# rosielab/emojivoice

Hardware: AMD Instinct MI355X
Metric: audio_seconds_per_second (higher is better)
Workload: dtype f32 (deep layers: operand = two block-scaled fp16 pieces, product = 3 fp16 products on the fp16 MFMA, f32 accumulate); 1 GPU; config2: batch 64 x 516-frame (5.99 s) utterances per GPU, 10 Euler steps + HiFi-GAN V1, 22.05 kHz; global_batch=64, frames=516, ode_steps=10, parallelism=dp1, collective=none, batch_pipeline=cfm(i+1) || hifigan(i) on two streams, 2 pipeline(s) in flight

## Files before the change

emojivoice_amd/_lib.py:

```python
from __future__ import annotations

import ctypes as C
import os
import subprocess
from typing import Dict, Optional

import numpy as np
import torch

_HERE = os.path.dirname(os.path.abspath(__file__))
LIB_PATH = os.environ.get("EV_LIB_PATH") or os.path.join(_HERE, "lib", "libemojivoice_hip.so")
CSRC = os.path.join(_HERE, "csrc")

EXPORTS = [
    "ev_abi_version", "ev_create", "ev_destroy", "ev_last_error", "ev_load_estimator", "ev_load_vocoder", "ev_load_vocoder_cfg", "ev_load_text_encoder", "ev_text_encoder",
    "ev_text_encoder_status", "ev_stft_magnitude", "ev_denoise", "ev_align", "ev_dbg_conv_bench",
    "ev_workspace_bytes", "ev_cfm_decode", "ev_estimator", "ev_hifigan", "ev_profile_enable", "ev_profile_read", "ev_profile_read_split", "ev_dbg_last_cfg", "ev_set_arithmetic", "ev_get_arithmetic",
    "ev_op_conv1d", "ev_op_groupnorm_mish", "ev_op_layernorm", "ev_op_split_pieces", "ev_op_attention", "ev_op_ln_mlp", "ev_set_mrf_streams_max",
    "ev_cfm_decode2", "ev_reserve", "ev_alloc_count", "ev_dbg_sk_stats", "ev_op_attn_out", "ev_dbg_set_amax", "ev_dbg_set_attn_h16", "ev_dbg_set_chain", "ev_dbg_sk_taken",
    "ev_load_mel_basis", "ev_mel_spectrogram",
    "ev_maximum_path", "ev_log_prior", "ev_mas_align",
    "ev_estimator_rows", "ev_cfm_loss",
    "ev_load_resampler", "ev_resample", "ev_mel_stats",
]


class EvLibraryError(RuntimeError):
    pass


class ev_tensor_index(C.Structure):
    _fields_ = [("name", C.c_char_p), ("offset", C.c_uint64), ("ndim", C.c_int32), ("shape", C.c_int64 * 4)]


class ev_model_dims(C.Structure):
    _fields_ = [("n_feats", C.c_int32), ("spk_emb_dim", C.c_int32), ("channels", C.c_int32), ("heads", C.c_int32),
                ("head_dim", C.c_int32)]


class ev_vocoder_config(C.Structure):
    _fields_ = [("resblock", C.c_int32), ("num_levels", C.c_int32), ("upsample_rates", C.c_int32 * 4), ("upsample_kernel_sizes", C.c_int32 * 4),
                ("resblock_kernel_sizes", C.c_int32 * 3), ("resblock_dilations", (C.c_int32 * 3) * 3)]


def vocoder_config(h) -> ev_vocoder_config:
    c = ev_vocoder_config()
    c.resblock = 1 if str(h["resblock"]) == "1" else 2
    c.num_levels = len(h["upsample_rates"])
    for i, (u, k) in enumerate(zip(h["upsample_rates"], h["upsample_kernel_sizes"])):
        c.upsample_rates[i], c.upsample_kernel_sizes[i] = int(u), int(k)
    for j, (k, ds) in enumerate(zip(h["resblock_kernel_sizes"], h["resblock_dilation_sizes"])):
        c.resblock_kernel_sizes[j] = int(k)
        for m, d in enumerate(ds):
            c.resblock_dilations[j][m] = int(d)
    return c


def vocoder_frame_bytes(h) -> int:
    rates, rb1 = list(h["upsample_rates"]), str(h["resblock"]) == "1"
    widest, prod, p0 = 0, 1, 4
    for i, u in enumerate(rates):
        prod *= u
        widest = max(widest, prod * (h["upsample_initial_channel"] // 2 ** (i + 1)) * 4)
        halo = 3 if i == len(rates) - 1 else 0
        for k, ds in zip(h["resblock_kernel_sizes"], h["resblock_dilation_sizes"]):
            for d in (ds if rb1 else ds[:2]):
                halo = max(halo, (k - 1) * d // 2)
        p0 = max(p0, -(-halo // prod))
    return widest, p0


def build_library(force: bool = False, verbose: bool = False) -> str:
    src = os.path.join(CSRC, "ev_engine.hip")
    deps = [src, os.path.join(CSRC, "ev_kernels.h"), os.path.join(os.path.dirname(_HERE), "include", "emojivoice.h")]
    if not force and os.path.exists(LIB_PATH) and all(os.path.getmtime(LIB_PATH) >= os.path.getmtime(d) for d in deps):
        return LIB_PATH
    os.makedirs(os.path.dirname(LIB_PATH), exist_ok=True)
    hipcc = os.environ.get("HIPCC", "/opt/rocm/bin/hipcc")
    cmd = [hipcc, "--offload-arch=gfx950", "-O3", "-std=c++17", "-fPIC", "-shared", "-Wno-unused-value", src, "-o", LIB_PATH]
    if verbose:
        print(" ".join(cmd))
    subprocess.run(cmd, check=True)
    return LIB_PATH


_lib: Optional[C.CDLL] = None


def load_library() -> C.CDLL:
    global _lib
    if _lib is not None:
        return _lib
    if not os.path.exists(LIB_PATH):
        raise EvLibraryError(
            f"{LIB_PATH} is missing: build it with `python -c 'import __graft_entry__ as g; g.build()'` "
            "(there is no CPU fallback for the EmojiVoice hot path)")
    lib = C.CDLL(LIB_PATH)
    vp, i32, f32, u64 = C.c_void_p, C.c_int, C.c_float, C.c_size_t
    lib.ev_abi_version.restype = C.c_int
    lib.ev_create.argtypes = [C.POINTER(vp), i32, C.POINTER(ev_model_dims)]
    lib.ev_destroy.argtypes = [vp]
    lib.ev_destroy.restype = None
    lib.ev_last_error.argtypes = [vp]
    lib.ev_last_error.restype = C.c_char_p
    for f in (lib.ev_load_estimator, lib.ev_load_vocoder, lib.ev_load_text_encoder):
        f.argtypes = [vp, vp, C.POINTER(ev_tensor_index), u64]
    lib.ev_load_vocoder_cfg.argtypes = [vp, vp, C.POINTER(ev_tensor_index), u64, C.POINTER(ev_vocoder_config)]
    lib.ev_set_mrf_streams_max.argtypes = [vp, i32]
    lib.ev_set_mrf_streams_max.restype = i32
    lib.ev_workspace_bytes.argtypes = [vp, i32, i32, i32]
    lib.ev_workspace_bytes.restype = u64
    lib.ev_cfm_decode.argtypes = [vp, vp, vp, vp, vp, i32, i32, i32, f32, f32, vp, vp]
    lib.ev_cfm_decode2.argtypes = [vp, vp, vp, vp, vp, i32, i32, i32, vp, f32, f32, vp, vp]
    lib.ev_reserve.argtypes = [vp, i32, i32, i32, i32, vp]
    lib.ev_alloc_count.argtypes = [vp]
    lib.ev_alloc_count.restype = C.c_int64
    lib.ev_dbg_sk_stats.argtypes = [vp, C.POINTER(C.c_uint32)]
    lib.ev_estimator.argtypes = [vp, vp, vp, vp, vp, f32, i32, i32, vp, vp]
    lib.ev_estimator_rows.argtypes = [vp, vp, vp, vp, vp, vp, i32, i32, vp, vp]
    lib.ev_cfm_loss.argtypes = [vp, vp, vp, vp, vp, vp, vp, i32, i32, f32, vp, vp, vp]
    lib.ev_hifigan.argtypes = [vp, vp, i32, i32, vp, vp]
    lib.ev_text_encoder.argtypes = [vp, vp, vp, vp, i32, i32, vp, vp, vp]
    lib.ev_text_encoder_status.argtypes = [vp, vp]
    lib.ev_dbg_conv_bench.argtypes = [vp, i32, i32, i32, i32, i32, i32, i32, i32, i32, i32, C.POINTER(C.c_float)]
    lib.ev_stft_magnitude.argtypes = [vp, vp, i32, i32, vp, vp]
    lib.ev_align.argtypes = [vp, vp, vp, vp, vp, i32, i32, i32, vp, vp, vp]
    lib.ev_denoise.argtypes = [vp, vp, i32, i32, vp, f32, vp, vp]
    lib.ev_load_mel_basis.argtypes = [vp, vp, i32, i32]
    lib.ev_mel_spectrogram.argtypes = [vp, vp, i32, i32, f32, f32, vp, vp]
    lib.ev_load_resampler.argtypes = [vp, vp, i32, i32, i32]
    lib.ev_resample.argtypes = [vp, vp, vp, i32, i32, vp, i32, vp]
    lib.ev_mel_stats.argtypes = [vp, vp, vp, i32, i32, i32, vp, vp]
    lib.ev_maximum_path.argtypes = [vp, vp, vp, vp, i32, i32, i32, vp, vp, vp]
    lib.ev_log_prior.argtypes = [vp, vp, vp, i32, i32, i32, vp, vp]
    lib.ev_mas_align.argtypes = [vp, vp, vp, vp, vp, i32, i32, i32, vp, vp, vp, vp, vp]
    lib.ev_profile_enable.argtypes = [vp, i32]
    lib.ev_profile_read.argtypes = [vp, C.POINTER(C.c_double), C.POINTER(C.c_double), C.POINTER(C.c_int64), i32]
    lib.ev_profile_read_split.argtypes = [vp, C.POINTER(C.c_double), C.POINTER(C.c_double), C.POINTER(C.c_int64)]
    lib.ev_dbg_last_cfg.argtypes = [vp]
    lib.ev_set_arithmetic.argtypes = [vp, i32]
    lib.ev_get_arithmetic.argtypes = [vp]
    lib.ev_dbg_set_amax.argtypes = [vp, i32]
    lib.ev_dbg_set_attn_h16.argtypes = [vp, i32]
    lib.ev_dbg_set_chain.argtypes = [vp, i32]
    lib.ev_dbg_sk_taken.argtypes = [vp]
    lib.ev_dbg_sk_taken.restype = C.c_int64
    lib.ev_op_conv1d.argtypes = [vp, vp, vp, vp, i32, i32, i32, i32, i32, i32, i32, i32, i32, f32, vp, vp]
    lib.ev_op_groupnorm_mish.argtypes = [vp, vp, vp, vp, vp, i32, i32, i32, i32, vp, vp]
    lib.ev_op_layernorm.argtypes = [vp, vp, vp, vp, i32, i32, vp, vp]
    lib.ev_op_split_pieces.argtypes = [vp, vp, i32, vp, vp]
    lib.ev_op_attention.argtypes = [vp, vp, vp, i32, i32, i32, vp, vp]
    lib.ev_op_attn_out.argtypes = [vp, vp, vp, i32, i32, vp, vp, vp, vp]
    lib.ev_op_ln_mlp.argtypes = [vp, vp, vp, vp, vp, vp, vp, vp, vp, vp, vp, i32, i32, i32, vp, vp]
    for n in EXPORTS:
        getattr(lib, n)
    _lib = lib
    return lib


def _stream_ptr() -> int:
    return int(torch.cuda.current_stream().cuda_stream)


class Engine:

    def __init__(self, device: int = 0, spk_emb_dim: int = 64, heads: int = 2):
        if not torch.cuda.is_available():
            raise EvLibraryError("no ROCm GPU visible: the EmojiVoice hot path has no CPU fallback")
        self.lib = load_library()
        self.device = device
        dims = ev_model_dims(80, spk_emb_dim, 256, heads, 64)
        h = C.c_void_p()
        rc = self.lib.ev_create(C.byref(h), device, C.byref(dims))
        if rc != 0:
            raise EvLibraryError(f"ev_create failed with code {rc}")
        self.h = h
        self.spk_emb_dim = spk_emb_dim
        env = os.environ.get("EV_MRF_STREAMS_MAX", "")
        if env:
            import re
            m = re.match(r"\s*([+-]?\d+)", env)
            self.mrf_streams_max = int(m.group(1)) if m else 0
        else:
            self.mrf_streams_max = 16384
        self.pipeline_owner = None
        self.voc_frame_bytes, self.voc_pad0 = 256 * 128, 4

    def set_mrf_streams_max(self, max_frames: int) -> None:
        if self.lib.ev_set_mrf_streams_max(self.h, int(max_frames)) != 0:
            raise EvLibraryError(self.lib.ev_last_error(self.h).decode())
        self.mrf_streams_max = int(max_frames)

    def close(self):
        if getattr(self, "h", None):
            self.lib.ev_destroy(self.h)
            self.h = None

    def __del__(self):
        try:
            self.close()
        except Exception:
            pass

    def _check(self, rc: int, what: str):
        if rc != 0:
            raise EvLibraryError(f"{what} failed: {self.lib.ev_last_error(self.h).decode()}")

    def _load(self, fn, tensors: Dict[str, torch.Tensor], what: str, *extra):
        names = list(tensors.keys())
        arrs = [np.ascontiguousarray(tensors[k].detach().to("cpu", torch.float32).numpy()).reshape(-1) for k in names]
        blob = np.concatenate(arrs) if arrs else np.zeros(1, np.float32)
        idx = (ev_tensor_index * len(names))()
        off = 0
        keep = []
        for i, k in enumerate(names):
            b = k.encode()
            keep.append(b)
            shp = tuple(tensors[k].shape)
            idx[i].name = b
            idx[i].offset = off
            idx[i].ndim = len(shp)
            for d, s in enumerate(shp):
                idx[i].shape[d] = s
            off += arrs[i].size
        self._check(fn(self.h, blob.ctypes.data_as(C.c_void_p), idx, len(names), *extra), what)

    def load_estimator(self, tensors: Dict[str, torch.Tensor]):
        self._load(self.lib.ev_load_estimator, tensors, "ev_load_estimator")
# ... 102 lines not shown
        return logp

    def mas_align(self, mu_x, y, x_lengths, y_lengths, want_attn: bool = True, want_dur: bool = True, want_mu_y: bool = True, want_logp: bool = False):
        mu_x, y = self._f32(mu_x), self._f32(y)
        B, F, Tx = mu_x.shape
        Ty = y.shape[2]
        assert y.shape[:2] == (B, F)
        dev = mu_x.device
        xl = x_lengths.to(dev, torch.int32).contiguous()
        yl = y_lengths.to(dev, torch.int32).contiguous()
        attn = torch.empty((B, Tx, Ty), dtype=torch.float32, device=dev) if want_attn else None
        dur = torch.empty((B, Tx), dtype=torch.int32, device=dev) if want_dur else None
        mu_y = torch.empty((B, F, Ty), dtype=torch.float32, device=dev) if want_mu_y else None
        logp = torch.empty((B, Tx, Ty), dtype=torch.float32, device=dev) if want_logp else None
        dp = lambda t: None if t is None else t.data_ptr()
        self._check(self.lib.ev_mas_align(self.h, mu_x.data_ptr(), y.data_ptr(), xl.data_ptr(), yl.data_ptr(), B, Tx, Ty,
                                          dp(attn), dp(dur), dp(mu_y), dp(logp), _stream_ptr()), "ev_mas_align")
        return {"attn": attn, "dur": dur, "mu_y": mu_y, "logp": logp}

    def load_text_encoder(self, tensors: Dict[str, torch.Tensor]):
        self._load(self.lib.ev_load_text_encoder, tensors, "ev_load_text_encoder")

    def text_encoder(self, ids, lengths, spk):
        assert ids.is_cuda and ids.dim() == 2
        ids = ids.to(torch.int64).contiguous()
        B, Tx = ids.shape
        lengths = lengths.to(ids.device, torch.int32).contiguous()
        spk_p = None
        if spk is not None:
            spk = self._f32(spk)
            spk_p = spk.data_ptr()
        mu = torch.empty((B, 80, Tx), dtype=torch.float32, device=ids.device)
        logw = torch.empty((B, 1, Tx), dtype=torch.float32, device=ids.device)
        self._check(self.lib.ev_text_encoder(self.h, ids.data_ptr(), lengths.data_ptr(), spk_p, B, Tx, mu.data_ptr(), logw.data_ptr(), _stream_ptr()),
                    "ev_text_encoder")
        return mu, logw

    def text_encoder_status(self):
        if self.lib.ev_text_encoder_status(self.h, _stream_ptr()) != 0:
            raise IndexError(self.lib.ev_last_error(self.h).decode())

    @staticmethod
    def _f32(t: torch.Tensor) -> torch.Tensor:
        assert t.is_cuda, "tensor must live on the GPU"
        return t.contiguous().float()

    def cfm_decode(self, mu, lengths, spk, z, n_steps: int, out_scale: float = 1.0, out_shift: float = 0.0):
        mu, z = self._f32(mu), self._f32(z)
        B, F, Tp = mu.shape
        assert F == 80 and z.shape == mu.shape
        lengths = lengths.to(mu.device, torch.int32).contiguous()
        spk_p = None
        if spk is not None:
            spk = self._f32(spk)
            spk_p = spk.data_ptr()
        out = torch.empty_like(mu)
        self._check(self.lib.ev_cfm_decode(self.h, mu.data_ptr(), lengths.data_ptr(), spk_p, z.data_ptr(), B, Tp, int(n_steps),
                                           float(out_scale), float(out_shift), out.data_ptr(), _stream_ptr()), "ev_cfm_decode")
        return out

    def cfm_decode2(self, mu, lengths, spk, z, n_steps: int, mel_std: float, mel_mean: float):
        mu, z = self._f32(mu), self._f32(z)
        B, F, Tp = mu.shape
        assert F == 80 and z.shape == mu.shape
        lengths = lengths.to(mu.device, torch.int32).contiguous()
        spk_p = None
        if spk is not None:
            spk = self._f32(spk)
            spk_p = spk.data_ptr()
        dec, mel = torch.empty_like(mu), torch.empty_like(mu)
        self._check(self.lib.ev_cfm_decode2(self.h, mu.data_ptr(), lengths.data_ptr(), spk_p, z.data_ptr(), B, Tp, int(n_steps),
                                            dec.data_ptr(), float(mel_std), float(mel_mean), mel.data_ptr(), _stream_ptr()), "ev_cfm_decode2")
        return dec, mel

    def reserve(self, B: int, Tx_max: int = 0, Tp_max: int = 0, T_voc_max: int = 0) -> None:
        self._check(self.lib.ev_reserve(self.h, int(B), int(Tx_max), int(Tp_max), int(T_voc_max), _stream_ptr()), "ev_reserve")

    def alloc_count(self) -> int:
        return int(self.lib.ev_alloc_count(self.h))

    def sk_taken(self) -> int:
        return int(self.lib.ev_dbg_sk_taken(self.h))

    def sk_stats(self):
        out = (C.c_uint32 * 3)()
        self._check(self.lib.ev_dbg_sk_stats(self.h, out), "ev_dbg_sk_stats")
        return tuple(int(v) for v in out)

    def estimator(self, x, mu, lengths, spk, t: float):
        x, mu = self._f32(x), self._f32(mu)
        B, F, Tp = mu.shape
        lengths = lengths.to(mu.device, torch.int32).contiguous()
        spk_p = None
        if spk is not None:
            spk = self._f32(spk)
            spk_p = spk.data_ptr()
        out = torch.empty_like(mu)
        self._check(self.lib.ev_estimator(self.h, x.data_ptr(), mu.data_ptr(), lengths.data_ptr(), spk_p, float(t), B, Tp,
                                          out.data_ptr(), _stream_ptr()), "ev_estimator")
        return out

    @staticmethod
    def _host_times(t, B: int) -> np.ndarray:
        tv = np.ascontiguousarray(torch.as_tensor(t).detach().to("cpu", torch.float32).numpy().reshape(-1))
        if tv.shape[0] != B:
            raise ValueError(f"t must hold one time per utterance: {B} expected, got {tv.shape[0]}")
        return tv

    def estimator_rows(self, x, mu, lengths, spk, t):
        x, mu = self._f32(x), self._f32(mu)
        B, F, Tp = mu.shape
        assert F == 80 and x.shape == mu.shape
        lengths = lengths.to(mu.device, torch.int32).contiguous()
        tv = self._host_times(t, B)
        spk_p = None
        if spk is not None:
            spk = self._f32(spk)
            spk_p = spk.data_ptr()
        out = torch.empty_like(mu)
        self._check(self.lib.ev_estimator_rows(self.h, x.data_ptr(), mu.data_ptr(), lengths.data_ptr(), spk_p, tv.ctypes.data_as(C.c_void_p), B, Tp,
                                               out.data_ptr(), _stream_ptr()), "ev_estimator_rows")
        return out

    def cfm_loss(self, x1, mu_y, y_lengths, spk, z, t, sigma_min: float, want_v: bool = False):
        x1, mu_y, z = self._f32(x1), self._f32(mu_y), self._f32(z)
        B, F, Ty = x1.shape
        assert F == 80 and mu_y.shape == x1.shape and z.shape == x1.shape
        yl = y_lengths.to(x1.device, torch.int32).contiguous()
        tv = self._host_times(t, B)
        spk_p = None
        if spk is not None:
            spk = self._f32(spk)
            spk_p = spk.data_ptr()
        sums = torch.empty((B, 2), dtype=torch.float64, device=x1.device)
        v = torch.empty_like(x1) if want_v else None
        self._check(self.lib.ev_cfm_loss(self.h, x1.data_ptr(), mu_y.data_ptr(), yl.data_ptr(), spk_p, z.data_ptr(), tv.ctypes.data_as(C.c_void_p), B, Ty,
                                         float(sigma_min), sums.data_ptr(), v.data_ptr() if want_v else None, _stream_ptr()), "ev_cfm_loss")
        return sums, v

    def hifigan(self, mel):
        mel = self._f32(mel)
        B, F, T = mel.shape
        assert F == 80
        wav = torch.empty((B, 1, T * 256), dtype=torch.float32, device=mel.device)
        per_utt = (T + 2 * self.voc_pad0) * self.voc_frame_bytes
        bmax = max(1, int((2**32 - 2**20) // per_utt))
        for b0 in range(0, B, bmax):
            b1 = min(B, b0 + bmax)
            self._check(self.lib.ev_hifigan(self.h, mel[b0:b1].data_ptr(), b1 - b0, T, wav[b0:b1].data_ptr(), _stream_ptr()), "ev_hifigan")
        return wav

    def workspace_bytes(self, B: int, Tp: int, Tv: int) -> int:
        return int(self.lib.ev_workspace_bytes(self.h, B, Tp, Tv))

    def profile_enable(self, on: bool):
        self._check(self.lib.ev_profile_enable(self.h, int(on)), "ev_profile_enable")

    def op_split_pieces(self, x):
        x = self._f32(x).reshape(-1)
        out = torch.empty((3, x.numel()), dtype=torch.float32, device=x.device)
        self._check(self.lib.ev_op_split_pieces(self.h, x.data_ptr(), x.numel(), out.data_ptr(), _stream_ptr()), "ev_op_split_pieces")
        return out

    def set_arithmetic(self, bf16_products: int):
        self._check(self.lib.ev_set_arithmetic(self.h, int(bf16_products)), "ev_set_arithmetic")

# ... 98 lines not shown
```

emojivoice_amd/csrc/ev_engine.hip:

```cpp
#include "ev_kernels.h"
#include "../../include/emojivoice.h"

#include <math.h>
#include <stdlib.h>
#include <stdarg.h>
#include <stdio.h>
#include <string.h>

#include <algorithm>
#include <atomic>
#include <mutex>
#include <numeric>
#include <string>
#include <unordered_map>
#include <vector>

namespace {

struct HostTensor {
    const float* p = nullptr;
    int ndim = 0;
    int64_t shape[4] = {0, 0, 0, 0};
    int64_t numel() const { int64_t n = 1; for (int i = 0; i < ndim; ++i) n *= shape[i]; return n; }
};
typedef std::unordered_map<std::string, HostTensor> TensorMap;

struct Geom { int nrows, S, P, T; };

struct ConvLayer {
    float* W = nullptr;
    unsigned short* Wh = nullptr; float wh_scale = 1.f;
    unsigned short* Wx = nullptr;
    unsigned short* Wq = nullptr;
    float* bias = nullptr;
    int2* taplist[3] = {nullptr, nullptr, nullptr};
    int* nact[3] = {nullptr, nullptr, nullptr};
    bool sparse_taps = false;
    bool tile128_exact = true;
    int kstack_mt = 0, kstack_tap = 0;
    int ntaps = 0, off[EV_MAX_TAPS] = {0};
    int halo_lo = 0, halo_hi = 0;
    bool wide = false;
    int Cin = 0, Cout = 0, Mpad = 0, Kpad = 0;
    double macs_per_row = 0;
};

struct Epi {
    int act = ACT_NONE; float act_slope = 0.f; const float* act_a = nullptr; const float* act_b = nullptr;
    int mask1 = 0; float scale = 1.f; const float* R = nullptr; int ldr = 0; int accum = 0; int div3 = 0;
    int act2_lrelu = 0; float act2_slope = 0.f; int mask2 = 0; const float* rowmask = nullptr; int mmul = 1;
    float* Y2 = nullptr; int ldy2 = 0;
    float pro_slope = -1.f;
    int dbg = 0; int force_cfg = -1; int stagger = -1; unsigned long long* stamps = nullptr;
    float* gn_part = nullptr;
    int isplit_log2 = 31, isstride = 0;
    unsigned* ymax = nullptr; int ymax_mul = 1; const unsigned* rmax = nullptr; const unsigned* yold = nullptr; const unsigned* xmax = nullptr; int xmax_n = 0;
    int osplit_log2 = 31, osstride = 0;
};

struct ResnetW { ConvLayer c1r, c2; float *g1, *b1, *g2, *b2; };
struct TransW {
    ConvLayer qkv, out, ff1, ff2; float *ln1g, *ln1b, *ln3g, *ln3b, *alpha, *binv;
    float qkv_scale[3] = {0.f, 0.f, 0.f};
};

struct EstimatorW {
    bool loaded = false;
    int in_ch = 0;
    ConvLayer t1, t2, tmlp;
    ResnetW rn[6];
    ConvLayer rn0_c1r_x, rn0_c1r_ms;
    TransW tr[6];
    ConvLayer down0, down1, up0, up1, fin_conv, fin_proj;
    float *fin_g, *fin_b;
};

struct VocoderW {
    bool loaded = false;
    int rb = 1;
    int nl = 4;
    int rates[4] = {8, 8, 2, 2};
    int P0 = 4;
    ConvLayer pre, post, ups[4];
    ConvLayer c1[12][3], c2[12][3];
    ConvLayer lo[12][2], hi[12][2];
    int ch[5];
    float* post_w = nullptr; float post_b = 0.f; int post_k = 0;
};

struct EncLayerW { ConvLayer qkv, out, ff1, ff2; float *g1, *b1, *g2, *b2; };
struct TextEncW {
    bool loaded = false;
    int nvocab = 0, nch = 0, C = 0, heads = 0, nlayers = 0, ffc = 0;
    float* emb = nullptr; float* theta = nullptr;
    ConvLayer pre[3], pre_proj; float *pre_g[3], *pre_b[3];
    std::vector<EncLayerW> layers;
    ConvLayer proj_m, dp1, dp2, dp_proj; float *dp_g1, *dp_b1, *dp_g2, *dp_b2;
};

struct DenoiserW { bool ready = false; ConvLayer fwd, inv; float* win2 = nullptr; };

struct MelBasisW { bool loaded = false; int n_mels = 0, nb = 0; int* span = nullptr; float* wts = nullptr; };
struct ResamplerW { bool loaded = false; int up = 0, down = 0, n_taps = 0, W = 0, Wp = 0, tab_floats = 0; float* table = nullptr; };

}

struct ev_handle {
    int device = 0;
    ev_model_dims dims;
    std::string err;
    std::vector<void*> owned;
    EstimatorW est;
    VocoderW voc;
    TextEncW enc;
    DenoiserW dn;
    MelBasisW melb;
    ResamplerW rs;
    struct Scratch { char* p = nullptr; size_t bytes = 0; hipStream_t last = nullptr; bool last_valid = false; };
    Scratch dn_ws, enc_ws, mas_ws;
    Scratch stat_ws;
    float* zeros = nullptr;
    int max_steps = 64;
    int* bad_ids_host = nullptr; int* bad_ids_dev = nullptr;
    char* ws = nullptr; size_t ws_bytes = 0; size_t ws_used = 0; size_t ws_bytes_last = 0;
    int ws_B = -1, ws_Tp = -1, ws_Tv = -1;
    bool prof = false;
    bool fuse_pairs = true;
    bool fuse_attn = true;
    bool attn_h16 = true;
    bool use_chain = true;
    bool fuse_mlp = true;
    int gn_stats_tiles = 0;
    int fuse_mlp_min_tiles = 96;
    std::vector<hipEvent_t> ev_pool; size_t ev_used = 0;
    hipStream_t ws_stream = nullptr; bool ws_stream_valid = false;
    float* temb_host[2] = {nullptr, nullptr}; size_t temb_cap[2] = {0, 0}; hipEvent_t temb_ev[2] = {nullptr, nullptr}; int temb_slot = 0;
    float* cap_pool = nullptr; size_t cap_stride = 0; int cap_used = 0; int cap_nt[8] = {0};
    struct TprojEntry { int nt; float* d; };
    std::vector<TprojEntry> tproj_cache;
    bool captured = false; int cap_B = 0, cap_Tp = 0;
    int64_t n_allocs = 0;
    double prof_flops = 0; int64_t prof_launches = 0;
    struct ProfRec { int kind, Cin, Cout, ntaps, nrows, cfg, lean; double flops; bool split = false; };
    std::vector<ProfRec> prof_recs;
    hipStream_t stream = nullptr;
    hipStream_t mrf_stream[2] = {nullptr, nullptr};
    hipEvent_t mrf_ev[4] = {nullptr, nullptr, nullptr, nullptr};
    int ncu = 0;
    unsigned* sk_ctrl = nullptr;
    unsigned sk_seq = 0;
    float* sk_part = nullptr;
    int split_terms = 16;
    bool use_amax = true;
    bool amax_emitted = false;
    int n_fp32_only_layers = 0;
    int last_cfg = -1;
    bool sk_balance = true;
    int sk_wgs = 2;
    int sk_spin = 3000;
    int mrf_max_frames = 16384;
    int force_cfg = -1;
    bool lean = true;
    bool small_sk = true;
    bool sk32_lean = true;
    bool gn_stats = true;
    bool qkv_h16 = true;
    bool attn_sk = true;
    int attn_tpw = 2;
    bool full_rezero = false;
    int rb2_minkeep = 4;
};

namespace {

int fail(ev_handle* h, const char* fmt, ...) {
    char buf[512];
    va_list ap; va_start(ap, fmt); vsnprintf(buf, sizeof buf, fmt, ap); va_end(ap);
    if (h) h->err = buf;
    return 1;
}
#define HIPCHK(h, x) do { hipError_t e_ = (x); if (e_ != hipSuccess) return fail(h, "%s failed: %s (%s:%d)", #x, hipGetErrorString(e_), __FILE__, __LINE__); } while (0)

template <typename T>
int dev_upload(ev_handle* h, const std::vector<T>& v, T** out) {
    void* d = nullptr;
    HIPCHK(h, hipMalloc(&d, v.size() * sizeof(T) + 16));
    HIPCHK(h, hipMemcpy(d, v.data(), v.size() * sizeof(T), hipMemcpyHostToDevice));
    h->owned.push_back(d);
    *out = (T*)d;
    return 0;
}

int round_up(int x, int m) { return (x + m - 1) / m * m; }

int scratch_acquire(ev_handle* h, ev_handle::Scratch& s, size_t need) {
    if (s.last_valid && s.last != h->stream) HIPCHK(h, hipStreamSynchronize(s.last));
    if (need > s.bytes) {
        if (s.last_valid) HIPCHK(h, hipStreamSynchronize(h->stream));
        if (s.p) HIPCHK(h, hipFree(s.p));
        const size_t want = std::max(need, s.bytes + s.bytes / 2);
        s.p = nullptr; s.bytes = 0;
        if (hipMalloc((void**)&s.p, want) == hipSuccess) s.bytes = want;
        else { (void)hipGetLastError(); HIPCHK(h, hipMalloc((void**)&s.p, need)); s.bytes = need; }
        ++h->n_allocs;
    }
    s.last = h->stream; s.last_valid = true;
    return 0;
}

int finish_layer(ev_handle* h, ConvLayer& L, const std::vector<float>& Wh, const std::vector<float>* bias) {
    int lo = 0, hi = 0;
    for (int i = 0; i < L.ntaps; ++i) { if (-L.off[i] > lo) lo = -L.off[i]; if (L.off[i] > hi) hi = L.off[i]; }
    L.halo_lo = lo; L.halo_hi = hi;
    if (lo + hi > EV_HALO && !L.wide) return fail(h, "conv halo %d exceeds EV_HALO", lo + hi);
    {
        std::vector<float> Wf(Wh.size());
        const int MT32 = L.Mpad / 32, KG8 = L.Kpad / 8;
        for (int tap = 0; tap < L.ntaps; ++tap)
            for (int mt = 0; mt < MT32; ++mt)
                for (int kg = 0; kg < KG8; ++kg)
                    for (int lane = 0; lane < 64; ++lane)
                        for (int e = 0; e < 4; ++e) {
                            const int row = mt * 32 + (lane & 31), k = kg * 8 + 4 * (lane >> 5) + e;
                            Wf[((((size_t)tap * MT32 + mt) * KG8 + kg) * 64 + lane) * 4 + e] = Wh[((size_t)tap * L.Mpad + row) * L.Kpad + k];
                        }
        if (dev_upload(h, Wf, &L.W)) return 1;
    }
    if (L.Kpad % 16 == 0) {
        float mx = 0.f;
        for (float w : Wh) if (std::isfinite(w)) mx = std::max(mx, std::fabs(w));
        int k = 0;
        if (mx > 0.f) { int ex; std::frexp(mx, &ex); k = 14 - ex; }
        k = std::max(-40, std::min(40, k));
        L.wh_scale = std::ldexp(1.0f, k);
        const int MT32 = L.Mpad / 32, KG16 = L.Kpad / 16;
        std::vector<unsigned short> Whp(Wh.size() * 2);
        auto hbits = [](_Float16 v) { unsigned short u; memcpy(&u, &v, 2); return u; };
        for (int tap = 0; tap < L.ntaps; ++tap)
            for (int mt = 0; mt < MT32; ++mt)
                for (int kg = 0; kg < KG16; ++kg)
                    for (int lane = 0; lane < 64; ++lane)
                        for (int e = 0; e < 8; ++e) {
                            const int row = mt * 32 + (lane & 31), kk = kg * 16 + 8 * (lane >> 5) + e;
                            const float w = Wh[((size_t)tap * L.Mpad + row) * L.Kpad + kk] * L.wh_scale;
                            const _Float16 h0 = (_Float16)w, h1 = (_Float16)(w - (float)h0);
                            const size_t base = ((((size_t)tap * MT32 + mt) * KG16 + kg) * 2) * 512 + (size_t)lane * 8 + e;
                            Whp[base] = hbits(h0); Whp[base + 512] = hbits(h1);
                        }
// ... 250 lines not shown
    h->prof_recs.push_back(r);
    return 0;
}
inline double valid_rows(const Geom& g) { return (double)(g.nrows / g.S) * g.T; }

inline bool over_4gib(const Geom& g, int ld) { return (double)g.nrows * ld * 4.0 >= 4294967296.0; }

template <int BM, int BN, int WM, int WN, bool PF = false>
void launch_cfg(const ConvParams& p, hipStream_t st, const LaunchOpts& lo) {
    const size_t xs = (size_t)(BN + ((lo.halo + 7) & ~7)) * 36;
    constexpr size_t es = (size_t)4 * 32 * (BM / WM + 4);
    size_t smem = (xs > es ? xs : es) * sizeof(float);
    if (lo.wgs_per_cu > 0) { size_t cap = (size_t)(160 * 1024 / lo.wgs_per_cu) & ~(size_t)255; if (cap > smem) smem = cap; }
    dispatch<1, 2, 3, 0, EPI_FULL>(epi_flavour(p, lo.lean && lean_ok(p)), [&](auto E) {
        launch<conv_gemm_kernel<BM, BN, WM, WN, PF, E == EPI_FULL, (E > 0 ? E : 0)>>(lo.device, dim3(p.mtiles * p.ntiles), dim3(256), smem, st, p);
    });
}

template <int BM, int BN, int WM, int WN, int TERMS = 6>
void launch_split(const ConvParams& p, hipStream_t st, const LaunchOpts& lo) {
    const size_t xs = (size_t)(BN + ((lo.halo + 7) & ~7)) * EVX_RSB;
    constexpr size_t es = (size_t)4 * 32 * (BM / WM + 4) * sizeof(float);
    const size_t smem = xs > es ? xs : es;
    dispatch<1, 2, 3>(epi_flavour(p, true), [&](auto E) {
        launch<conv_split_kernel<BM, BN, WM, WN, E, TERMS>>(lo.device, dim3(p.mtiles * p.ntiles), dim3(256), smem, st, p);
    });
}
template <int BM, int BN, int WM, int WN>
void launch_h16(const ConvParams& p, hipStream_t st, const LaunchOpts& lo) {
    const size_t xs = (size_t)(BN + EV_HALO) * EVH_RSB + 16;
    constexpr size_t es = (size_t)4 * 32 * (BM / WM + 4) * sizeof(float);
    const size_t smem = xs > es ? xs : es;
    const dim3 grid(p.mtiles * p.ntiles);
    if (p.Wq && p.act != ACT_SNAKE)
        dispatch<1, 3>(epi_flavour(p, true), [&](auto E) { launch<conv_h16_kernel<BM, BN, WM, WN, E, 1>>(lo.device, grid, dim3(256), smem, st, p); });
    else dispatch<1, 2, 3>(epi_flavour(p, true), [&](auto E) { launch<conv_h16_kernel<BM, BN, WM, WN, E>>(lo.device, grid, dim3(256), smem, st, p); });
}
inline bool split_ok(const ConvLayer& L, const ConvParams& p0) {
    ConvParams p = p0;
    p.dbg &= ~4;
    return L.Wx && lean_ok(p) && (p.isplit_log2 >= 31 || (p.isplit_log2 >= 6 && p.isplit_log2 < 31)) && L.Cin % EVX_KC == 0 && L.Cin == L.Kpad && L.Mpad % 128 == 0 && ((size_t)p.bias & 15) == 0;
}

template <int TW>
void launch_sk(const ConvParams& p, hipStream_t st, const LaunchOpts& lo) {
    constexpr int KS = TW == 4 ? 4 : 8, BN = TW == 4 ? 64 : 32;
    const int nchunks = p.Kpad / EV_BK, rows = BN + ((lo.halo + 7) & ~7);
    int kbs = nchunks < (TW == 4 ? 8 : 32) ? nchunks : (TW == 4 ? 8 : 32);
    while (kbs > 8 && ((size_t)rows * (32 * kbs + 4) * 4 > 150 * 1024 || rows * kbs * 8 > EV_SK_MAXF4(TW))) kbs = (kbs - 1) & ~7;
    const size_t xs = 2 * EV_MAX_TAPS + (size_t)rows * (32 * kbs + 4);
    const size_t red = (size_t)(KS - 1) * TW * 16 * 64, es = (size_t)TW * 32 * 36;
    size_t smem = std::max(xs, std::max(red, es)) * sizeof(float);
    ConvParams q = p;
    q.sk_kb = kbs;
    dispatch<1, 2, 3, 0, EPI_FULL>(epi_flavour(p, lo.lean && lean_ok(p)), [&](auto E) {
        launch<conv_gemm_sk_kernel<KS, E == EPI_FULL, (E > 0 ? E : 0), TW>>(lo.device, dim3(p.mtiles * p.ntiles), dim3(64 * TW * KS), smem, st, q);
    });
}

constexpr int EV_CAPTURE_SLOTS = 8;
constexpr int EV_SK_MAXWG = 1024;
constexpr int EV_SK_PART_FLOATS = 16384;
int ensure_sk(ev_handle* h, bool hot_path = true) {
    if (h->sk_ctrl) return 0;
    if (hot_path) ++h->n_allocs;
    const size_t words = 16 + 2 * EV_SK_MAXWG;
    HIPCHK(h, hipMalloc((void**)&h->sk_ctrl, words * sizeof(unsigned)));
    HIPCHK(h, hipMemset(h->sk_ctrl, 0, words * sizeof(unsigned)));
    HIPCHK(h, hipMalloc((void**)&h->sk_part, (size_t)EV_SK_MAXWG * 2 * EV_SK_PART_FLOATS * sizeof(float)));
    return 0;
}
int sk_setup(ev_handle* h, SkCtl& sk, long U, int G, bool claims) {
    if (ensure_sk(h)) return 1;
    sk.ctrl = h->sk_ctrl; sk.flags = h->sk_ctrl + 16; sk.part = h->sk_part; sk.part_floats = EV_SK_PART_FLOATS;
    sk.q = (int)(U / G); sk.r = (int)(U % G); sk.spin_limit = h->sk_spin;
    if (claims) { sk.claims = h->sk_ctrl + 16 + EV_SK_MAXWG; sk.seq = ++h->sk_seq; }
    return 0;
}

enum { PIPE_FP32, PIPE_BF16, PIPE_H16 };
template <int PIPE, int BM, int BN, int WM, int WN>
int launch_bal(ev_handle* h, ConvParams p, const LaunchOpts& lo, int wpc) {
    static_assert((size_t)BM * BN <= EV_SK_PART_FLOATS, "hand-off slot");
    const int G = wpc * h->ncu;
    if (sk_setup(h, p.sk, (long)p.mtiles * p.ntiles * (p.Kpad / (PIPE == PIPE_FP32 ? EV_BK : EVX_KC)), G, PIPE == PIPE_H16)) return 1;
    const size_t rsb = PIPE == PIPE_FP32 ? 36 * sizeof(float) : PIPE == PIPE_BF16 ? EVX_RSB : EVH_RSB;
    const size_t xs = (size_t)(BN + ((lo.halo + 7) & ~7)) * rsb;
    constexpr size_t es = (size_t)4 * 32 * (BM / WM + 4) * sizeof(float);
    size_t smem = xs > es ? xs : es;
    p.sk.lds_word = (int)smem;
    smem += PIPE == PIPE_H16 ? 16 + 3 * 4 * sizeof(float) + 16 : 16;
    const int lean = lean_acc(p) ? 3 : 1;
    const dim3 grid(G), block(256);
    if constexpr (PIPE == PIPE_FP32)
        dispatch<1, 3>(lean, [&](auto E) { launch<conv_gemm_bal_kernel<BM, BN, WM, WN, E>>(lo.device, grid, block, smem, h->stream, p); });
    else if constexpr (PIPE == PIPE_BF16)
        dispatch<1, 3>(lean, [&](auto E) { launch<conv_split_bal_kernel<BM, BN, WM, WN, E>>(lo.device, grid, block, smem, h->stream, p); });
    else if (BN + p.halo_lo + p.halo_hi <= 16 * 9)
        dispatch<1, 3>(lean, [&](auto E) { launch<conv_h16_bal_kernel<BM, BN, WM, WN, E, 9>>(lo.device, grid, block, smem, h->stream, p); });
    else dispatch<1, 3>(lean, [&](auto E) { launch<conv_h16_bal_kernel<BM, BN, WM, WN, E>>(lo.device, grid, block, smem, h->stream, p); });
    return 0;
}
inline bool split_bal_ok(const ev_handle* h, const ConvLayer& L, const ConvParams& p, long nwg, int wpc) {
    return h->sk_balance && h->ncu > 0 && split_ok(L, p) && p.act != ACT_SNAKE && !p.dbg && !p.stamps && !p.gn_part &&
           nwg * 2 >= h->ncu && wpc * h->ncu <= EV_SK_MAXWG && (long)nwg * (p.Kpad / EVX_KC) >= (long)wpc * h->ncu;
}
inline bool bal_ok(const ev_handle* h, const ConvLayer& L, const ConvParams& p, long nwg, int wpc) {
    if (L.sparse_taps) return false;
    return h->sk_balance && h->ncu > 0 && lean_ok(p) && p.act != ACT_SNAKE && !p.dbg && !p.stamps && !p.gn_part &&
           nwg >= h->ncu && nwg < 4L * wpc * h->ncu && wpc * h->ncu <= EV_SK_MAXWG && (long)nwg * (p.Kpad / EV_BK) >= (long)wpc * h->ncu;
}

enum : int {
    CFG_128x128 = 0, CFG_64x128 = 1, CFG_32x256 = 2, CFG_64x192 = 5, CFG_64x64 = 6,
    CFG_64x64_PF = 8,
    CFG_SK64 = 9, CFG_SK32 = 19,
    CFG_SPLIT = 40, CFG_SPLIT64 = 41, CFG_SPLIT3 = 43, CFG_SPLIT9 = 49,
    CFG_H16 = 46,
    CFG_SPLIT_BAL = 60,
    CFG_H16_64 = 47, CFG_BAL64 = 56, CFG_H16_BAL = 66,
};
struct ConvTile { int cfg, bm, bn, slots; bool split; };
constexpr ConvTile EV_TILES[] = {
    {CFG_128x128, 128, 128, 3, false}, {CFG_64x128, 64, 128, 4, false}, {CFG_32x256, 32, 256, 3, false}, {CFG_64x192, 64, 192, 4, false},
    {CFG_64x64, 64, 64, 5, false}, {CFG_64x64_PF, 64, 64, 5, false}, {CFG_SK64, 64, 64, 0, false}, {CFG_SK32, 32, 32, 0, false},
    {CFG_SPLIT, 128, 128, 0, true}, {CFG_SPLIT64, 64, 128, 0, true}, {CFG_SPLIT3, 128, 128, 0, true}, {CFG_H16, 128, 128, 0, true},
    {CFG_SPLIT9, 128, 128, 0, true}, {CFG_SPLIT_BAL, 128, 128, 0, true},
};
inline const ConvTile* conv_tile(int cfg) {
    for (const ConvTile& t : EV_TILES) if (t.cfg == cfg) return &t;
    return nullptr;
}
inline int tile_list(const ConvTile& t) { return t.bm == 128 ? 0 : t.bm == 64 ? 1 : 2; }
inline int tile_mtiles(const ConvTile& t, const ConvLayer& L) { return t.bm == 128 ? L.Mpad / 128 : (L.Cout + t.bm - 1) / t.bm; }
inline long tile_count(const ConvTile& t, const ConvLayer& L, const Geom& g) { return (long)tile_mtiles(t, L) * ((g.nrows + t.bn - 1) / t.bn); }

int pick_cfg(const ev_handle* h, const ConvLayer& L, const ConvParams& p, const Geom& g) {
    auto tiles = [&](int cfg) { return tile_count(*conv_tile(cfg), L, g); };
    int cfg;
    if (L.Cout <= 32) cfg = CFG_32x256;
    else {
        double best = 1e30;
        cfg = CFG_64x128;
        for (int c : {CFG_64x128, CFG_64x192, CFG_64x64}) {
            const ConvTile& k = *conv_tile(c);
            const long nwg = tiles(c);
            const double w = (double)(k.bm / 32) * (k.bn / 32);
            double t;
            if (nwg <= 256L * k.slots) t = (double)((nwg + 255) / 256) * w;
            else t = (double)nwg * w / 256.0 + (nwg < 256L * k.slots * 3 ? w : 0.0);
            t *= (c == CFG_64x64 ? 1.08 : 1.0);
            if (t < best - 1e-9) { best = t; cfg = c; }
        }
    }
    if (L.sparse_taps && L.Cout > 32 && tiles(CFG_64x64) <= 256L * 5 * 2) cfg = CFG_64x64;
    if (cfg == CFG_64x64 && tiles(CFG_64x64) <= 320) cfg = CFG_64x64_PF;
    if (cfg == CFG_64x128 && L.Cout % 128 == 0 && !L.sparse_taps && tiles(CFG_64x128) >= 256L * 4 * 6)
        cfg = (L.Cin > 128 && L.ntaps >= 7) ? CFG_64x192 : CFG_128x128;
    if (h->small_sk) {
        const long wg64 = tiles(CFG_64x64);
        if ((cfg == CFG_64x64 || cfg == CFG_64x64_PF) && wg64 <= 192 && (L.Kpad / EV_BK) * L.ntaps >= 8) cfg = CFG_SK64;
        if ((cfg == CFG_64x64 || cfg == CFG_64x64_PF) && wg64 <= 96 && L.Kpad == 128 && L.Cin == 128 && !L.sparse_taps) cfg = CFG_SK64;
        if (cfg == CFG_SK64 && wg64 <= 192 && L.Cout >= 32) cfg = CFG_SK32;
    }
    {
        const int split_terms = h->split_terms;
        const bool fp32_tile = cfg == CFG_128x128 || cfg == CFG_64x128 || cfg == CFG_64x192 || cfg == CFG_64x64;
        const long nwg128 = tiles(CFG_128x128);
        if (split_terms > 0 && fp32_tile && split_ok(L, p) && L.Cout % 128 == 0 && (!L.sparse_taps || (L.tile128_exact && L.kstack_mt == 0)) && nwg128 >= 2L * 2 * h->ncu && h->ncu > 0)
            cfg = split_terms == 3 ? CFG_SPLIT3 : split_terms == 9 ? CFG_SPLIT9 : split_terms == 16 ? CFG_H16 : CFG_SPLIT;
        else if ((split_terms == 6 || split_terms == 3 || split_terms == 16) && fp32_tile && split_ok(L, p) && L.Cout % 64 == 0 && L.kstack_mt == 0 && h->ncu > 0 &&
                 (L.sparse_taps || L.Cout % 128 != 0) && tiles(CFG_64x128) >= 2L * 3 * h->ncu) cfg = CFG_SPLIT64;
        else if ((split_terms == 6 || split_terms == 16) && fp32_tile && L.Cout == L.Mpad && split_bal_ok(h, L, p, nwg128, 2)) cfg = CFG_SPLIT_BAL;
    }
    return cfg;
}

constexpr int EV_GN_MAXTILES = 256;
int launch_conv(ev_handle* h, const ConvLayer& L, const float* X, int ldx, float* Y, int ldy, const Geom& g, const Epi& e) {
    ConvParams p;
    memset(&p, 0, sizeof p);
    h->gn_stats_tiles = 0;
    if (L.halo_lo + L.halo_hi > EV_HALO) return fail(h, "launch_conv: conv halo %d exceeds EV_HALO", L.halo_lo + L.halo_hi);
    p.X = X; p.ldx = ldx; p.Cin = L.Cin; p.isplit_log2 = e.isplit_log2; p.isstride = e.isstride;
    p.W = L.W; p.Wx = L.Wx; p.Wh = L.Wh; p.Wq = L.Wq; p.wh_scale = L.wh_scale; p.Mpad = L.Mpad; p.Kpad = L.Kpad; p.bias = L.bias;
    p.Y = Y; p.ldy = ldy; p.Cout = L.Cout; p.osplit_log2 = e.osplit_log2; p.osstride = e.osstride; p.mmul = e.mmul;
    p.nrows = g.nrows; p.S = g.S; p.P = g.P; p.T = g.T;
    p.ntaps = L.ntaps; for (int i = 0; i < L.ntaps; ++i) p.off[i] = L.off[i];
    if (!L.sparse_taps || L.kstack_mt > 0) {
        bool even = true;
        const int d = L.ntaps > 1 ? L.off[1] - L.off[0] : 0;
        for (int i = 2; i < L.ntaps; ++i) even = even && (L.off[i] - L.off[i - 1] == d);
        if (even) {
            p.plane_bytes = (L.Mpad / 32) * (L.Kpad / 8) * 1024; p.koff0 = L.off[0]; p.kdoff = d;
            if (!L.sparse_taps) p.ktaps_n = L.ntaps;
            else { p.kstack_mt = L.kstack_mt; p.kstack_tap = L.kstack_tap; }
        }
    }
    p.halo_lo = L.halo_lo; p.halo_hi = L.halo_hi;
    p.pro_lrelu = e.pro_slope >= 0.f; p.pro_slope = e.pro_slope;
    p.act = e.act; p.act_slope = e.act_slope; p.act_a = e.act_a; p.act_b = e.act_b;
    p.mask1 = e.mask1; p.scale = e.scale; p.R = e.R; p.ldr = e.ldr; p.accum = e.accum; p.div3 = e.div3;
    p.act2_lrelu = e.act2_lrelu; p.act2_slope = e.act2_slope; p.mask2 = e.mask2; p.rowmask = e.rowmask;
    p.Y2 = e.Y2; p.ldy2 = e.ldy2; p.dbg = e.dbg; p.stamps = e.stamps;
    p.xmax = e.xmax; p.xmax_n = e.xmax_n; p.rmax = e.rmax; p.yold = e.yold; p.ymax_mul = e.ymax_mul; h->amax_emitted = false;
    if ((ldx & 3) || (L.Cin & 3)) return fail(h, "conv input must be float4-aligned (ldx %d Cin %d)", ldx, L.Cin);
    if (over_4gib(g, ldx) || over_4gib(g, ldy) || (e.R && over_4gib(g, e.ldr)) || (e.Y2 && over_4gib(g, e.ldy2)))
        return fail(h, "tensor of %.1f GiB exceeds the 4 GiB buffer-addressing limit: split the batch", (double)g.nrows * std::max(ldx, ldy) * 4.0 / 1073741824.0);

    int cfg = pick_cfg(h, L, p, g);
    LaunchOpts lo;
    lo.device = h->device; lo.lean = h->lean; lo.halo = L.halo_lo + L.halo_hi;
    if (h->force_cfg >= 0) cfg = h->force_cfg;
    if (e.force_cfg >= 0) { cfg = e.force_cfg < 1000 ? e.force_cfg % 100 : -1; lo.wgs_per_cu = (e.force_cfg / 100) % 10; }
    if ((h->force_cfg >= 0 || e.force_cfg >= 0) && !conv_tile(cfg))
        return fail(h, "launch_conv: forced tile configuration %d is not one launch_conv selects", e.force_cfg >= 0 ? e.force_cfg : h->force_cfg);
    if (prof_begin(h)) return 1;
    {
        const ConvTile& s = *conv_tile(cfg == CFG_SK64 ? CFG_32x256 : cfg);
        p.stagger_slots = tile_count(s, L, g) >= 256L * s.slots * 3 ? s.slots : 0;
        if (e.stagger >= 0) p.stagger_slots = e.stagger;
    }
    if (conv_tile(cfg)->split && !split_ok(L, p)) cfg = CFG_128x128;
    if (cfg == CFG_H16 && !L.Wh) cfg = CFG_SPLIT;
    const bool fp16 = h->split_terms == 16 && L.Wh;
    {
        const bool lean1or3 = lean_ok(p) && p.act != ACT_SNAKE && h->lean;
        const bool h16 = cfg == CFG_H16 || (cfg == CFG_SPLIT64 && fp16);
        const bool gemm = (cfg == CFG_128x128 || cfg == CFG_64x128 || cfg == CFG_64x192 || cfg == CFG_64x64) && lean1or3;
        const bool no_amax = !h->use_amax;
        if (!no_amax && e.ymax && lean1or3 && (h16 || gemm) && (!e.R || e.rmax) && (!e.accum || e.yold)) { p.ymax = e.ymax; h->amax_emitted = true; }
        if (no_amax) p.xmax = nullptr;
    }
    const ConvTile& t = *conv_tile(cfg);
    p.mtiles = tile_mtiles(t, L); p.ntiles = (g.nrows + t.bn - 1) / t.bn;
    p.taplist = L.taplist[tile_list(t)]; p.nact_tab = L.nact[tile_list(t)]; p.tl_stride = L.sparse_taps ? EV_MAX_TAPS : 0;
    switch (cfg) {
    case CFG_H16: launch_h16<128, 128, 2, 2>(p, h->stream, lo); break;
    case CFG_SPLIT64:
        if (fp16) { launch_h16<64, 128, 2, 2>(p, h->stream, lo); cfg = CFG_H16_64; }
        else if (h->split_terms == 3) launch_split<64, 128, 2, 2, 3>(p, h->stream, lo);
        else launch_split<64, 128, 2, 2, 6>(p, h->stream, lo);
        break;
    case CFG_SPLIT_BAL:
        if (fp16) { if (launch_bal<PIPE_H16, 128, 128, 2, 2>(h, p, lo, 2)) return 1; cfg = CFG_H16_BAL; }
        else if (launch_bal<PIPE_BF16, 128, 128, 2, 2>(h, p, lo, 2)) return 1;
        break;
    case CFG_SPLIT: launch_split<128, 128, 2, 2, 6>(p, h->stream, lo); break;
    case CFG_SPLIT3: launch_split<128, 128, 2, 2, 3>(p, h->stream, lo); break;
    case CFG_SPLIT9: launch_split<128, 128, 2, 2, 9>(p, h->stream, lo); break;
    case CFG_128x128: launch_cfg<128, 128, 2, 2>(p, h->stream, lo); break;
    case CFG_64x128: launch_cfg<64, 128, 2, 2>(p, h->stream, lo); break;
    case CFG_64x192: launch_cfg<64, 192, 2, 2>(p, h->stream, lo); break;
    case CFG_64x64_PF: launch_cfg<64, 64, 2, 2, true>(p, h->stream, lo); break;
    case CFG_SK64: launch_sk<4>(p, h->stream, lo); break;
    case CFG_SK32: {
        const int xr = 32 + p.halo_lo + p.halo_hi;
        const bool fast = h->sk32_lean && h->lean && lean_ok(p) && (p.ktaps_n > 0 || p.kstack_mt > 0) && p.isplit_log2 >= 31 && !p.pro_lrelu && p.Cin == p.Kpad &&
                          (p.Kpad == 128 || p.Kpad == 256 || p.Kpad == 512 || p.Kpad == 1024) && (ldx % 4) == 0 && xr <= 16 * (512 / (p.Kpad / 4)) && (size_t)g.nrows * ldx * 4 < ((size_t)1 << 31) &&
                          (size_t)xr * (p.Kpad + 4) * 4 <= 150 * 1024;
        if (!fast) { launch_sk<1>(p, h->stream, lo); break; }
        if (h->gn_stats && e.gn_part && g.nrows == g.S && p.ntiles <= EV_GN_MAXTILES && p.act == ACT_NONE && !p.R && !lean_acc(p) && !p.mask1 && !p.mask2 &&
            (p.kstack_mt == 8 || (p.kstack_mt == 0 && L.Cout == 256))) {
            p.gn_part = e.gn_part;
            h->gn_stats_tiles = p.ntiles;
        }
        const size_t smem = std::max((size_t)xr * (p.Kpad + 4), (size_t)7 * 16 * 64) * sizeof(float);
        dispatch<1, 2, 3>(epi_flavour(p, true), [&](auto E) { launch<conv_sk32_kernel<E>>(h->device, dim3(p.mtiles, p.ntiles), dim3(512), smem, h->stream, p); });
        break;
    }
    case CFG_64x64:
        if (bal_ok(h, L, p, (long)p.mtiles * p.ntiles, 4)) {
            p.ymax = nullptr; h->amax_emitted = false;
            if (launch_bal<PIPE_FP32, 64, 64, 2, 2>(h, p, lo, 4)) return 1;
            cfg = CFG_BAL64;
        }
        else launch_cfg<64, 64, 2, 2>(p, h->stream, lo);
        break;
    default: launch_cfg<32, 256, 1, 4>(p, h->stream, lo);
    }
    HIPCHK(h, hipGetLastError());
    h->last_cfg = cfg;
    return h->prof ? prof_end(h, {0, L.Cin, L.Cout, L.ntaps, g.nrows, cfg, (int)lean_ok(p), 2.0 * L.macs_per_row * valid_rows(g), t.split}) : 0;
}

void resblock_params(ev_handle* h, ConvParams& p, const ConvLayer& Lc, const float* X, float* Y, int C, const Geom& g, const Epi& e, int out_rows) {
    p.X = X; p.ldx = C; p.Cin = C; p.isplit_log2 = 31;
    p.Mpad = Lc.Mpad; p.Kpad = Lc.Kpad;
    p.Y = Y; p.ldy = C; p.Cout = C; p.osplit_log2 = 31; p.mmul = 1;
    p.nrows = g.nrows; p.S = g.S; p.P = g.P; p.T = g.T;
    p.pro_lrelu = 1; p.pro_slope = 0.1f;
    p.scale = 1.f; p.ldr = C; p.accum = e.accum; p.div3 = e.div3; p.act2_lrelu = e.act2_lrelu; p.act2_slope = e.act2_slope;
    p.yold = e.yold; p.ymax_mul = 1; h->amax_emitted = false;
    p.mtiles = 1; p.ntiles = (g.nrows + out_rows - 1) / out_rows;
}
inline void resblock_bounds(ev_handle* h, ConvParams& p, const Epi& e) {
    if (e.ymax && (!e.accum || e.yold) && h->use_amax) { p.ymax = e.ymax; h->amax_emitted = true; }
}

int launch_pair(ev_handle* h, const ConvLayer& L1, const ConvLayer& L2, const float* X, float* Y, int C, const Geom& g, const Epi& e) {
    if (over_4gib(g, C)) return fail(h, "tensor exceeds the 4 GiB buffer-addressing limit: split the batch");
    if (L1.sparse_taps || L2.sparse_taps || L1.Kpad != C || L2.Kpad != C || L1.Kpad != L2.Kpad || L1.Mpad != L2.Mpad || L1.halo_lo != L1.halo_hi ||
        L2.halo_lo != L2.halo_hi || 2 * L2.halo_lo > 16 || !L1.bias || !L2.bias)
        return fail(h, "launch_pair: unsupported layer pair");
    if (C != 32 && C != 64 && C != 128) return fail(h, "launch_pair: C must be 32, 64 or 128");
    PairParams pp;
    memset(&pp, 0, sizeof pp);
    ConvParams& p = pp.c2;
    const int NT = 8192 / C;
    pp.h1 = L1.halo_lo; pp.h2 = L2.halo_lo; pp.mid_slope = 0.1f; pp.out_rows = NT - 2 * pp.h2;
    resblock_params(h, p, L2, X, Y, C, g, e, pp.out_rows);
    p.W = L2.W; p.bias = L2.bias; p.ntaps = L2.ntaps; p.taplist = L2.taplist[0];
    p.R = X;
    pp.W1 = L1.W; pp.W1x = L1.Wx; p.Wx = L2.Wx; pp.W1h = L1.Wh; pp.w1h_scale = L1.wh_scale; p.Wh = L2.Wh; p.wh_scale = L2.wh_scale; pp.b1 = L1.bias; pp.taplist1 = L1.taplist[0]; pp.ntaps1 = L1.ntaps;
    if (prof_begin(h)) return 1;
    const int lean = epi_flavour(p, h->lean);
    const int split_terms = h->split_terms;
    const bool split = split_terms > 0 && lean != 0 && L1.Wx && L2.Wx && !(e.force_cfg == 0);
    const bool h16 = split && split_terms == 16 && L1.Wh && L2.Wh;
    const dim3 grid(p.ntiles), block(256);
    dispatch<32, 64, 128>(C, [&](auto CC) {
        constexpr int WM = CC / 32, WN = 4 / WM;
        if (h16) {
            resblock_bounds(h, p, e);
            const size_t smem = std::max((size_t)(NT + EV_HALO) * (4 * C + 16) + 64, (size_t)4 * 32 * 36 * sizeof(float));
            dispatch<1, 3>(lean, [&](auto E) { launch<resblock_pair_h16_kernel<WM, WN, E>>(h->device, grid, block, smem, h->stream, pp); });
        } else if (split) {
            const size_t rsb = 6 * C + 16;
// ... 37 lines not shown
    for (int m = 0; m < 3; ++m) {
        cp.W1h[m] = L1[m].Wh; cp.W2h[m] = L2[m].Wh; cp.w1_scale[m] = L1[m].wh_scale; cp.w2_scale[m] = L2[m].wh_scale;
        cp.b1[m] = L1[m].bias; cp.b2[m] = L2[m].bias; cp.tl1[m] = L1[m].taplist[0]; cp.tl2[m] = L2[m].taplist[0];
        hb = std::max(hb, std::max(L1[m].halo_lo, L2[m].halo_lo));
        macs += L1[m].macs_per_row + L2[m].macs_per_row;
    }
    cp.ntaps1 = L1[0].ntaps; cp.ntaps2 = L2[0].ntaps; cp.hb = hb; cp.halo = chain_halo(L1, L2); cp.mid_slope = 0.1f;
    const int NT = 8192 / C;
    cp.out_rows = NT - 2 * cp.halo;
    resblock_params(h, p, L2[2], X, Y, C, g, e, cp.out_rows);
    resblock_bounds(h, p, e);
    if (prof_begin(h)) return 1;
    const int lean = epi_flavour(p, true);
    const size_t smem = std::max((size_t)(NT + EV_HALO) * (4 * C + 16) + 64, (size_t)4 * 32 * 36 * sizeof(float));
    dispatch<32, 64>(C, [&](auto CC) {
        constexpr int WM = CC / 32, WN = 4 / WM;
        dispatch<1, 3>(lean, [&](auto E) { launch<resblock_chain_h16_kernel<WM, WN, E>>(h->device, dim3(p.ntiles), dim3(256), smem, h->stream, cp); });
    });
    HIPCHK(h, hipGetLastError());
    h->last_cfg = 180 + L2[0].ntaps;
    return h->prof ? prof_end(h, {1, C, C, L1[0].ntaps, g.nrows, 180 + L2[0].ntaps, lean, 2.0 * macs * valid_rows(g), true}) : 0;
}

inline int rb2_halo(const ConvLayer* L) { return L[0].halo_lo + L[1].halo_lo; }
inline bool rb2_ok(const ev_handle* h, const ConvLayer* L, int C) {
    if (!h->use_chain || h->split_terms != 16 || (C != 32 && C != 64 && C != 128)) return false;
    for (int m = 0; m < 2; ++m) {
        const ConvLayer& a = L[m];
        if (!a.Wh || !a.bias || a.sparse_taps || a.Kpad != C || a.Mpad != L[0].Mpad || a.halo_lo != a.halo_hi || a.ntaps != L[0].ntaps || a.ntaps > 64) return false;
    }
    const int NT = C == 32 ? 256 : C == 64 ? 128 : 64;
    return 8 * (NT - 2 * rb2_halo(L)) >= h->rb2_minkeep * NT && NT - 2 * rb2_halo(L) > 0;
}
int launch_rb2(ev_handle* h, const ConvLayer* L, const float* X, float* Y, int C, const Geom& g, const Epi& e) {
    if (over_4gib(g, C)) return fail(h, "tensor exceeds the 4 GiB buffer-addressing limit: split the batch");
    Rb2Params cp;
    memset(&cp, 0, sizeof cp);
    ConvParams& p = cp.c2;
    int hb = 0;
    for (int m = 0; m < 2; ++m) {
        cp.Wh[m] = L[m].Wh; cp.w_scale[m] = L[m].wh_scale; cp.b[m] = L[m].bias; cp.tl[m] = L[m].taplist[0];
        hb = std::max(hb, L[m].halo_lo);
    }
    cp.ntaps = L[0].ntaps; cp.hb = hb; cp.halo = rb2_halo(L);
    const int NT = 8192 / C;
    cp.out_rows = NT - 2 * cp.halo;
    if (cp.out_rows <= 0) return fail(h, "launch_rb2: halo %d leaves no row of a %d-frame tile", cp.halo, NT);
    resblock_params(h, p, L[1], X, Y, C, g, e, cp.out_rows);
    resblock_bounds(h, p, e);
    if (prof_begin(h)) return 1;
    const int lean = epi_flavour(p, true);
    const size_t smem = std::max((size_t)(NT + 2 * hb) * (4 * C + 16) + 64, (size_t)4 * 32 * 36 * sizeof(float));
    dispatch<32, 64, 128>(C, [&](auto CC) {
        constexpr int WM = CC / 32, WN = 4 / WM;
        dispatch<1, 3>(lean, [&](auto E) { launch<resblock2_h16_kernel<WM, WN, E>>(h->device, dim3(p.ntiles), dim3(256), smem, h->stream, cp); });
    });
    HIPCHK(h, hipGetLastError());
    h->last_cfg = 200 + L[0].ntaps;
    return h->prof ? prof_end(h, {1, C, C, L[0].ntaps, g.nrows, 200 + L[0].ntaps, lean, 2.0 * (L[0].macs_per_row + L[1].macs_per_row) * valid_rows(g), true}) : 0;
}

int launch_gn(ev_handle* h, const float* X, int ldx, float* Y, int ldy, const float* gamma, const float* beta, const float* rowmask,
              const float* temb, const float* R, int ldr, const Geom& g, int C, int mode, const float* part = nullptr, int temb_stride = 0) {
    GNParams p;
    p.X = X; p.ldx = ldx; p.Y = Y; p.ldy = ldy; p.gamma = gamma; p.beta = beta; p.rowmask = rowmask; p.temb = temb; p.R = R; p.ldr = ldr;
    p.S = g.S; p.P = g.P; p.T = g.T; p.CG = C / 8; p.mode = mode; p.eps = 1e-5f; p.temb_stride = temb_stride;
    if (p.CG != 32) return fail(h, "groupnorm kernel expects 32 channels per group, got %d", p.CG);
    if (part && h->gn_stats_tiles > 0 && g.nrows == g.S && h->gn_stats_tiles == (g.nrows + 31) / 32)
        hipLaunchKernelGGL(groupnorm_apply_kernel, dim3(h->gn_stats_tiles, 8), dim3(256), 0, h->stream, p, part, h->gn_stats_tiles);
    else if (g.nrows / g.S < 32) hipLaunchKernelGGL(groupnorm_mish_kernel<1024>, dim3(g.nrows / g.S, 8), dim3(1024), 0, h->stream, p);
    else hipLaunchKernelGGL(groupnorm_mish_kernel<512>, dim3(g.nrows / g.S, 8), dim3(512), 0, h->stream, p);
    HIPCHK(h, hipGetLastError());
    return 0;
}

int launch_ln(ev_handle* h, const float* X, int ldx, float* Y, int ldy, const float* gamma, const float* beta, const Geom& g) {
    LNParams p;
    p.X = X; p.ldx = ldx; p.Y = Y; p.ldy = ldy; p.gamma = gamma; p.beta = beta; p.nrows = g.nrows; p.S = g.S; p.P = g.P; p.T = g.T; p.eps = 1e-5f;
    hipLaunchKernelGGL(layernorm256_kernel, dim3((g.nrows + 3) / 4), dim3(256), 0, h->stream, p);
    HIPCHK(h, hipGetLastError());
    return 0;
}

int launch_mlp(ev_handle* h, int mode, const float* X, const float* ln_g, const float* ln_b, const ConvLayer& L1, const ConvLayer* L2,
               const float* alpha, const float* binv, const float* R, const float* rowmask, float* Y, int ldy, const Geom& g,
               const float* qkv_scale = nullptr, int* qkv_packed = nullptr) {
    if (qkv_packed) *qkv_packed = 0;
    MlpParams mp;
    memset(&mp, 0, sizeof mp);
    ConvParams& p = mp.ep;
    const ConvLayer& Lout = mode == 0 ? *L2 : L1;
    p.Y = Y; p.ldy = ldy; p.Cout = Lout.Cout; p.bias = mode == 0 ? Lout.bias : nullptr; p.osplit_log2 = 31; p.isplit_log2 = 31; p.mmul = 1;
    p.nrows = g.nrows; p.S = g.S; p.P = g.P; p.T = g.T; p.scale = 1.f;
    p.R = R; p.ldr = 256; p.rowmask = rowmask; p.mask2 = (mode == 0 && rowmask) ? 1 : 0;
    mp.X = X; mp.ldx = 256; mp.ln_g = ln_g; mp.ln_b = ln_b; mp.ln_eps = 1e-5f;
    if (!L1.bias && !h->zeros) {
        HIPCHK(h, hipMalloc((void**)&h->zeros, 4096 * sizeof(float)));
        HIPCHK(h, hipMemsetAsync(h->zeros, 0, 4096 * sizeof(float), h->stream));
        h->owned.push_back(h->zeros);
    }
    if (L1.Mpad > 4096) return fail(h, "launch_mlp: hidden width %d > 4096", L1.Mpad);
    mp.W1 = L1.W; mp.b1 = L1.bias ? L1.bias : h->zeros; mp.M1 = L1.Mpad; mp.alpha = alpha; mp.binv = binv; mp.W2 = L2 ? L2->W : nullptr;
    if (L1.Cin != 256 || L1.Kpad != 256 || L1.ntaps != 1 || (L1.Mpad % 128) || L1.Cout != L1.Mpad || (ldy & 3))
        return fail(h, "launch_mlp: first linear must be 256 -> multiple of 128 (got %d -> %d)", L1.Cin, L1.Cout);
    if (mode == 0 && (!L2 || L2->Cout != 256 || L2->Mpad != 256 || L2->Cin != L1.Cout || L2->Kpad != L1.Mpad || L2->ntaps != 1 || !L2->bias || !alpha || !binv))
        return fail(h, "launch_mlp: second linear must be %d -> 256 with bias", L1.Cout);
    if (over_4gib(g, std::max(ldy, 256))) return fail(h, "tensor exceeds the 4 GiB buffer-addressing limit: split the batch");
    if (g.S < 4 && g.nrows > 1) return fail(h, "launch_mlp: utterance stride %d < 4 rows is not supported by the lean row walk", g.S);
    const int nchunk = L1.Mpad / 128;
    const double flops = 2.0 * (L1.macs_per_row + (L2 ? L2->macs_per_row : 0.0)) * valid_rows(g);
    {
        const int split_terms = h->split_terms;
        const int nt64 = (g.nrows + 63) / 64;
        if (mode == 0 && (split_terms == 6 || split_terms == 16) && L1.Wx && L2->Wx && h->sk_balance && h->ncu > 0 && h->ncu <= EV_SK_MAXWG && nt64 >= h->ncu) {
            const int grid = h->ncu;
            const bool h16 = split_terms == 16 && L1.Wh && L2->Wh;
            mp.W1x = L1.Wx; mp.W2x = L2->Wx; mp.ntiles = nt64;
            mp.W1h = L1.Wh; mp.W2h = L2->Wh; mp.w1_scale = L1.wh_scale; mp.w2_scale = L2->wh_scale;
            if (sk_setup(h, mp.sk, (long)nt64 * nchunk, grid, h16)) return 1;
            if (L1.Mpad > 1024) return fail(h, "launch_mlp: hidden width %d > 1024 (LDS table of the SnakeBeta vectors)", L1.Mpad);
            const size_t smem = h16 ? (size_t)64 * (4 * 256 + 16) + (size_t)64 * (4 * 128 + 16) + 16 + (size_t)2 * L1.Mpad * sizeof(float) + 64
                                    : (size_t)64 * (6 * 256 + 16) + (size_t)64 * (6 * 128 + 16) + 16 + (size_t)2 * L1.Mpad * sizeof(float);
            if (prof_begin(h)) return 1;
            if (h16) launch<ln_mlp_h16_kernel<0>>(h->device, dim3(grid), dim3(256), smem, h->stream, mp);
            else launch<ln_mlp_split_kernel<6>>(h->device, dim3(grid), dim3(256), smem, h->stream, mp);
            HIPCHK(h, hipGetLastError());
            return h->prof ? prof_end(h, {2, 256, Lout.Cout, 1, g.nrows, h16 ? 121 : 120, 1, flops, true}) : 0;
        }
    }
    {
        const int nt64 = (g.nrows + 63) / 64;
        if (mode == 1 && h->split_terms == 16 && h->qkv_h16 && L1.Wh && L1.Mpad == 384 && !R && !rowmask && h->ncu > 0 && nt64 >= h->ncu) {
            mp.W1h = L1.Wh; mp.w1_scale = L1.wh_scale; mp.ntiles = nt64;
            if (qkv_scale && qkv_packed && qkv_scale[0] > 0.f && qkv_scale[1] > 0.f && qkv_scale[2] > 0.f) {
                mp.qkv_pack = 1; *qkv_packed = 1;
                for (int i = 0; i < 3; ++i) mp.qkv_scale[i] = qkv_scale[i];
            }
            const size_t smem = (size_t)64 * (4 * 256 + 16) + 32;
            if (prof_begin(h)) return 1;
            launch<ln_qkv_h16_kernel<0>>(h->device, dim3(nt64), dim3(256), smem, h->stream, mp);
            HIPCHK(h, hipGetLastError());
            h->last_cfg = 122;
            return h->prof ? prof_end(h, {3, 256, Lout.Cout, 1, g.nrows, 122, 1, flops, true}) : 0;
        }
    }
    const int ntiles = (g.nrows + 31) / 32;
    size_t smem = (size_t)(32 * 260 + 4 * 32 * 36 + 4) * sizeof(float);
    int grid = ntiles;
    mp.ntiles = ntiles;
    mp.sk.q = nchunk; mp.sk.r = 0; mp.sk.spin_limit = h->sk_spin;
    const int wpc = h->sk_wgs;
    const bool big = ntiles >= h->ncu && (long)ntiles * nchunk >= (long)wpc * h->ncu;
    if (h->sk_balance && h->ncu > 0 && wpc * h->ncu <= EV_SK_MAXWG && big) {
        const long U = (long)ntiles * nchunk;
        grid = (int)std::min<long>((long)wpc * h->ncu, U);
        if (sk_setup(h, mp.sk, U, grid, false)) return 1;
        if (wpc != 2) smem = std::max(smem, (size_t)((160 * 1024 / wpc) & ~255));
    }
    if (prof_begin(h)) return 1;
    const bool two = (mp.sk.ctrl != nullptr && wpc == 2) || (mp.sk.ctrl == nullptr && h->ncu > 0 && ntiles <= 2 * h->ncu);
    dispatch<0, 1>(mode != 0, [&](auto M) {
        if (two) launch<ln_mlp_kernel<M, 2>>(h->device, dim3(grid), dim3(256), smem, h->stream, mp);
        else launch<ln_mlp_kernel<M, 3>>(h->device, dim3(grid), dim3(256), smem, h->stream, mp);
    });
    HIPCHK(h, hipGetLastError());
    return h->prof ? prof_end(h, {2 + mode, 256, Lout.Cout, 1, g.nrows, 20 + mode, 1, flops}) : 0;
}

constexpr int EV_ATTN_MAXPARTS = 16;
constexpr int EV_ATTN_MAXROWS = 8192;
int launch_attn(ev_handle* h, const float* QKV, int ld, float* O, int ldo, const float* rowmask, const Geom& g, int H, float* part = nullptr) {
    AttnParams p;
    p.QKV = QKV; p.ld = ld; p.O = O; p.ldo = ldo; p.rowmask = rowmask; p.S = g.S; p.P = g.P; p.T = g.T; p.H = H; p.scale = 0.125f;
    const int nwg = ((g.T + 127) / 128) * H * (g.nrows / g.S), nkt = (g.T + 31) / 32;
    if (h->attn_sk && part && nwg <= 64 && nkt >= 4 && g.nrows <= EV_ATTN_MAXROWS) {
        AttnPartParams pp;
        pp.a = p; pp.rows = g.nrows;
        pp.KS = std::min(EV_ATTN_MAXPARTS, (nkt + h->attn_tpw - 1) / h->attn_tpw);
        pp.PO = part; pp.PML = part + (size_t)EV_ATTN_MAXPARTS * g.nrows * H * 64;
        hipLaunchKernelGGL(attention_part_kernel, dim3((g.T + 127) / 128, H, (g.nrows / g.S) * pp.KS), dim3(256), 0, h->stream, pp);
        const long tot = (long)g.nrows * H * 16;
        hipLaunchKernelGGL(attention_merge_kernel, dim3((unsigned)((tot + 255) / 256)), dim3(256), 0, h->stream, pp);
    } else {
        hipLaunchKernelGGL(attention_kernel, dim3((g.T + 127) / 128, H, g.nrows / g.S), dim3(256), 0, h->stream, p);
    }
    HIPCHK(h, hipGetLastError());
    return 0;
}

bool attn_mask_split(const float* qkv_scale, float* mask_a, float* mask_b) {
    int eq = 0, ek = 0;
    if (!(qkv_scale[0] > 0.f) || !(qkv_scale[1] > 0.f) || std::frexp(qkv_scale[0], &eq) != 0.5f || std::frexp(qkv_scale[1], &ek) != 0.5f) return false;
    const int e = 3 + (eq - 1) + (ek - 1);
    const int ea = std::min(15, std::max(-14, e / 2)), eb = e - ea;
    if (eb < -14 || eb > 15) return false;
    *mask_a = (float)std::ldexp(1.0, ea); *mask_b = (float)std::ldexp(1.0, eb);
    return true;
}

void qkv_pack_scales(const HostTensor* g, const HostTensor* b, std::initializer_list<const HostTensor*> ws, float* out) {
    out[0] = out[1] = out[2] = 0.f;
    if (!g || !b) return;
    float tmp[3]; int t = 0;
    for (const HostTensor* W : ws) {
        if (!W || W->ndim != 2 || t >= 3) return;
        const int M = (int)W->shape[0], C = (int)W->shape[1];
        if ((int)g->shape[0] != C || (int)b->shape[0] != C) return;
        const double rc = std::sqrt((double)(C - 1));
        double worst = 0.0;
        for (int j = 0; j < M; ++j) {
            double acc = 0.0;
            for (int c = 0; c < C; ++c) acc += std::fabs((double)W->p[(size_t)j * C + c]) * (rc * std::fabs((double)g->p[c]) + std::fabs((double)b->p[c]));
            worst = std::max(worst, acc);
        }
        if (!(worst > 0.0) || !std::isfinite(worst)) return;
        int e = (int)std::floor(std::log2(32768.0 / worst));
        e = std::min(40, std::max(-40, e));
        tmp[t++] = (float)std::ldexp(1.0, e);
    }
    float ma, mb;
    if (t == 3 && attn_mask_split(tmp, &ma, &mb)) for (int i = 0; i < 3; ++i) out[i] = tmp[i];
}

inline bool attn_out_ok(const ev_handle* h, const ConvLayer& Lo, const Geom& g, int H) {
    const long wgs = (long)((g.T + 31) / 32) * (g.nrows / g.S);
    return h->fuse_attn && H == 2 && Lo.Cin == 128 && Lo.Kpad == 128 && Lo.Cout == 256 && Lo.Mpad == 256 && Lo.ntaps == 1 && !Lo.sparse_taps && Lo.bias &&
           g.S >= 4 && h->ncu > 0 && wgs >= h->ncu / 2;
}
int launch_attn_out(ev_handle* h, const float* QKV, int ld, const ConvLayer& Lo, float* Hid, int ldh, const float* rowmask, const Geom& g, int H,
                    const float* qkv_scale = nullptr) {
    AttnOutParams p;
    memset(&p, 0, sizeof p);
    const bool h16 = qkv_scale != nullptr;
    if (h16) {
        p.inv_sq = 1.0f / qkv_scale[0]; p.inv_sk = 1.0f / qkv_scale[1]; p.inv_sv = 1.0f / qkv_scale[2]; p.Wouth = Lo.Wh; p.wo_scale = Lo.wh_scale;
        if (!attn_mask_split(qkv_scale, &p.mask_a, &p.mask_b) || !Lo.Wh) return fail(h, "launch_attn_out: q / k scales %g, %g outside the fp16 form's range", qkv_scale[0], qkv_scale[1]);
    }
    const int B = g.nrows / g.S;
    p.QKV = QKV; p.ld = ld; p.rowmask = rowmask; p.Wout = Lo.W; p.S = g.S; p.P = g.P; p.T = g.T; p.B = B; p.nq = (g.T + 31) / 32; p.scale = 0.125f;
    p.xcd_map = (B % 8 == 0) ? 1 : 0;
    {
        const int last = g.T - 32 * (p.nq - 1);
        if (p.nq >= 2 && last <= AO_TAILQ) { p.ntail = last; p.nq -= 1; }
    }
    ConvParams& e = p.ep;
    e.Y = Hid; e.ldy = ldh; e.Cout = Lo.Cout; e.bias = Lo.bias; e.R = Hid; e.ldr = ldh; e.osplit_log2 = 31; e.isplit_log2 = 31; e.mmul = 1; e.scale = 1.f;
    e.nrows = g.nrows; e.S = g.S; e.P = g.P; e.T = g.T;
    if ((ldh & 3) || (ld & 3) || ((size_t)Lo.bias & 15)) return fail(h, "launch_attn_out: unaligned operand");
    if (over_4gib(g, std::max(ld, ldh))) return fail(h, "tensor exceeds the 4 GiB buffer-addressing limit: split the batch");
    const size_t smem = h16 ? (size_t)4 * AOH_WB : (size_t)4 * 2 * 32 * AO_LDK * sizeof(float);
    if (prof_begin(h)) return 1;
    const dim3 grid((unsigned)(p.nq * B + (p.ntail > 0 ? B : 0)));
    if (h16) launch<attn_out_h16_kernel>(h->device, grid, dim3(256), smem, h->stream, p);
    else launch<attn_out_kernel>(h->device, grid, dim3(256), smem, h->stream, p);
    HIPCHK(h, hipGetLastError());
    const double fl = (double)B * ((double)H * 4.0 * g.T * (double)g.T * 64.0 + 2.0 * Lo.macs_per_row * g.T);
    return h->prof ? prof_end(h, {4, 128, 256, 1, g.nrows, h16 ? 31 : 30, 1, fl, h16}) : 0;
}

struct Bump {
    char* base; size_t off = 0; size_t cap;
    float* take(size_t nfloats) {
        size_t bytes = (nfloats * sizeof(float) + 255) & ~(size_t)255;
        float* p = (float*)(base ? base + off : nullptr);
        off += bytes;
        return p;
    }
};

struct EstBufs {
    Geom g0, g1, gt;
    float *rm0, *rm1, *X0, *state, *A0, *B0, *R0, *H0, *LN0, *QKV0, *ATT0, *FF0, *CAT1, *U1, *F0, *G0, *V0;
    float *A1, *B1, *R1, *H1, *LN1, *QKV1, *ATT1, *FF1, *CAT0, *D1, *D2, *M1, *UU;
    float *tv, *temb_in, *temb_a, *temb_b, *tproj;
    float *LOSSP; int32_t* elen;
    float *GNP;
    float *ATTP;
    float *C1RMS;
    float *AR0, *AR1;
};

void plan_est(Bump& b, int B, int Tp, int in_ch, int nsteps, EstBufs& e) {
    e.g0 = {B * (Tp + 4), Tp + 4, 2, Tp};
    e.g1 = {B * (Tp / 2 + 2), Tp / 2 + 2, 1, Tp / 2};
    e.gt = {nsteps, nsteps, 0, nsteps};
    const size_t n0 = e.g0.nrows, n1 = e.g1.nrows;
    e.rm0 = b.take(n0); e.rm1 = b.take(n1);
    e.X0 = b.take(n0 * in_ch); e.state = b.take(n0 * 80);
    e.A0 = b.take(n0 * 256); e.B0 = b.take(n0 * 256); e.R0 = b.take(n0 * 256); e.H0 = b.take(n0 * 256); e.LN0 = b.take(n0 * 256);
    e.QKV0 = b.take(n0 * 384); e.ATT0 = b.take(n0 * 128); e.FF0 = b.take(n0 * 1024); e.CAT1 = b.take(n0 * 512);
    e.U1 = b.take(n0 * 256); e.F0 = b.take(n0 * 256); e.G0 = b.take(n0 * 256); e.V0 = b.take(n0 * 80);
    e.A1 = b.take(n1 * 256); e.B1 = b.take(n1 * 256); e.R1 = b.take(n1 * 256); e.H1 = b.take(n1 * 256); e.LN1 = b.take(n1 * 256);
    e.QKV1 = b.take(n1 * 384); e.ATT1 = b.take(n1 * 128); e.FF1 = b.take(n1 * 1024); e.CAT0 = b.take(n1 * 512);
    e.D1 = b.take(n1 * 256); e.D2 = b.take(n1 * 256); e.M1 = b.take(n1 * 256); e.UU = b.take(n1 * 256);
    const size_t ns = nsteps;
    e.C1RMS = b.take(n0 * 512); e.AR0 = b.take(n0 * 512); e.AR1 = b.take(n1 * 512);
    e.ATTP = b.take(std::min<size_t>(n0, EV_ATTN_MAXROWS) * EV_ATTN_MAXPARTS * (128 + 4));
    e.GNP = b.take((size_t)EV_GN_MAXTILES * 8 * 4);
    e.tv = b.take(ns); e.temb_in = b.take(ns * in_ch); e.temb_a = b.take(ns * 1024); e.temb_b = b.take(ns * 1024); e.tproj = b.take(ns * 1536);
    e.LOSSP = b.take((size_t)B * (Tp / 32 + 1) * 4); e.elen = (int32_t*)b.take(B);
}

struct VocBufs {
    Geom g[5] = {};
    float *M0 = nullptr, *C0 = nullptr;
    float *U[5] = {}, *XS[5] = {}, *T1[5] = {}, *Pa[5] = {}, *Pb[5] = {};
    float *T1x[2][5] = {}, *Pax[2][5] = {}, *Pbx[2][5] = {};
    struct { float* p; int C, l; unsigned* amax[2]; int amax_n; } zl[64]; int nz = 0;
    unsigned* slots = nullptr; size_t slot_words = 0;
    int index_of(const float* q) const { for (int k = 0; k < nz; ++k) if (zl[k].p == q) return k; return -1; }
};

void plan_voc(Bump& b, int B, int T, const int* ch, const int* rates, int nl, int P0, VocBufs& v, bool mrf_streams = false) {
    int Tl = T, Pl = P0;
    v.g[0] = {B * (Tl + 2 * Pl), Tl + 2 * Pl, Pl, Tl};
    for (int l = 1; l <= nl; ++l) {
        Tl *= rates[l - 1]; Pl *= rates[l - 1];
        v.g[l] = {B * (Tl + 2 * Pl), Tl + 2 * Pl, Pl, Tl};
    }
    v.nz = 0;
    auto take = [&](size_t n, int C, int l) { float* q = b.take(n); v.zl[v.nz].p = q; v.zl[v.nz].C = C; v.zl[v.nz].l = l; ++v.nz; return q; };
    v.M0 = take((size_t)v.g[0].nrows * 80, 80, 0);
    v.C0 = take((size_t)v.g[0].nrows * ch[0], ch[0], 0);
    for (int l = 1; l <= nl; ++l) {
        const size_t n = (size_t)v.g[l].nrows * ch[l];
        v.U[l] = take(n, ch[l], l); v.XS[l] = take(n, ch[l], l); v.T1[l] = take(n, ch[l], l); v.Pa[l] = take(n, ch[l], l); v.Pb[l] = take(n, ch[l], l);
        for (int c = 0; c < 2; ++c) {
            v.T1x[c][l] = mrf_streams ? take(n, ch[l], l) : nullptr; v.Pax[c][l] = mrf_streams ? take(n, ch[l], l) : nullptr;
            v.Pbx[c][l] = mrf_streams ? take(n, ch[l], l) : nullptr;
        }
    }
    v.slot_words = 0;
    for (int k = 0; k < v.nz; ++k) { v.zl[k].amax_n = (v.g[v.zl[k].l].nrows >> 7) + 2; v.slot_words += 2 * (size_t)v.zl[k].amax_n; }
    v.slots = (unsigned*)b.take(v.slot_words);
    size_t off = 0;
    for (int k = 0; k < v.nz; ++k)
        for (int c = 0; c < 2; ++c) { v.zl[k].amax[c] = v.slots ? v.slots + off : nullptr; off += (size_t)v.zl[k].amax_n; }
}
inline bool mrf_streams_for(const ev_handle* h, int B, int Tv) { return h->mrf_max_frames > 0 && (long)B * Tv <= h->mrf_max_frames; }


size_t plan_all(ev_handle* h, char* base, int B, int Tp, int Tv, EstBufs* eb, VocBufs* vb, size_t* voc_off = nullptr) {
    Bump b{base, 0, 0};
    EstBufs e; VocBufs v;
    if (Tp > 0) plan_est(b, B, Tp, h->est.loaded ? h->est.in_ch : 2 * h->dims.n_feats + h->dims.spk_emb_dim, h->max_steps, e);
    if (voc_off) *voc_off = b.off;
    if (Tv > 0) {
        const int ch[5] = {512, 256, 128, 64, 32}, rates[4] = {8, 8, 2, 2};
        const VocoderW& w = h->voc;
        plan_voc(b, B, Tv, w.loaded ? w.ch : ch, w.loaded ? w.rates : rates, w.loaded ? w.nl : 4, w.loaded ? w.P0 : 4, v, mrf_streams_for(h, B, Tv));
    }
    if (eb) *eb = e;
    if (vb) *vb = v;
    return b.off;
}

int grow_ws(ev_handle* h, size_t need, bool geometric) {
    if (h->ws_stream_valid) HIPCHK(h, hipStreamSynchronize(h->ws_stream));
    if (h->stream && (!h->ws_stream_valid || h->stream != h->ws_stream)) HIPCHK(h, hipStreamSynchronize(h->stream));
    if (h->ws) HIPCHK(h, hipFree(h->ws));
    h->ws = nullptr; h->ws_bytes = 0; h->ws_B = -1;
    const size_t want = geometric ? std::max(need, h->ws_bytes_last + h->ws_bytes_last / 2) : need;
    if (want > need && hipMalloc((void**)&h->ws, want) == hipSuccess) h->ws_bytes = want;
    else { (void)hipGetLastError(); HIPCHK(h, hipMalloc((void**)&h->ws, need)); h->ws_bytes = need; }
    h->ws_bytes_last = h->ws_bytes;
    ++h->n_allocs;
    return 0;
}

int ensure_ws(ev_handle* h, int B, int Tp, int Tv, EstBufs* eb, VocBufs* vb) {
    if (!h->captured) {
        if (Tp <= 0) Tp = h->ws_Tp > 0 && h->ws_B == B ? h->ws_Tp : 0;
        if (Tv <= 0) Tv = h->ws_Tv > 0 && h->ws_B == B ? h->ws_Tv : 0;
    }
    if (h->ws_stream_valid && h->ws_stream != h->stream) HIPCHK(h, hipStreamSynchronize(h->ws_stream));
    h->ws_stream = h->stream; h->ws_stream_valid = true;
    const size_t need = plan_all(h, nullptr, B, Tp, Tv, nullptr, nullptr);
    bool rezero = h->captured || B != h->ws_B || Tp != h->ws_Tp || Tv != h->ws_Tv;
    if (need > h->ws_bytes) {
        if (h->captured) return fail(h, "this handle holds a captured ev_cfm_decode: its workspace cannot be replaced (needs %zu bytes, has %zu); "
                                        "use ev_reserve before capturing, or another handle", need, h->ws_bytes);
        if (grow_ws(h, need, true)) return 1;
        rezero = true;
    }
    size_t voc_off = 0;
    VocBufs vplan;
    plan_all(h, h->ws, B, Tp, Tv, eb, &vplan, &voc_off);
    if (vb) *vb = vplan;
    if (rezero) {
        const size_t zbytes = (h->full_rezero || Tv <= 0) ? need : voc_off;
        if (zbytes) {
            hipStreamCaptureStatus cst = hipStreamCaptureStatusNone;
            const bool capturing = h->stream && hipStreamIsCapturing(h->stream, &cst) == hipSuccess && cst == hipStreamCaptureStatusActive;
            if (capturing || h->captured) {
                const size_t n16 = (zbytes + 15) / 16;
                hipLaunchKernelGGL(zero_fill_kernel, dim3((unsigned)std::min<size_t>((n16 + 255) / 256, 2048)), dim3(256), 0, h->stream, (f32x4*)h->ws, n16);
                HIPCHK(h, hipGetLastError());
            } else HIPCHK(h, hipMemsetAsync(h->ws, 0, zbytes, h->stream));
        }
        if (!h->full_rezero && Tv > 0 && vplan.nz > 0) {
            ZeroPadParams zp;
            memset(&zp, 0, sizeof zp);
            zp.B = B; zp.n = vplan.nz;
            for (int k = 0; k < vplan.nz; ++k) { zp.p[k] = vplan.zl[k].p; zp.C[k] = vplan.zl[k].C; zp.lvl[k] = vplan.zl[k].l; }
            long most = 0;
            for (int l = 0; l < 5; ++l) {
                zp.S[l] = vplan.g[l].S; zp.P[l] = vplan.g[l].P; zp.T[l] = vplan.g[l].T;
            }
            for (int k = 0; k < vplan.nz; ++k) most = std::max(most, (long)B * (zp.S[zp.lvl[k]] - zp.T[zp.lvl[k]]) * (zp.C[k] / 4));
            const unsigned gx = (unsigned)std::min<long>((most + 255) / 256, 512);
            hipLaunchKernelGGL(zero_pads_kernel, dim3(gx ? gx : 1, vplan.nz), dim3(256), 0, h->stream, zp);
            HIPCHK(h, hipGetLastError());
        }
        h->ws_B = B; h->ws_Tp = Tp; h->ws_Tv = Tv;
    }
    return 0;
}

struct LevelBufs { float *A, *Bf, *R, *H, *LN, *QKV, *ATT, *FF; const float* rm; Geom g; float* AR; float* ATTP; float* GNP; };
inline int g_rows32(const Geom& g) { return (g.nrows + 31) / 32; }

int run_resnet(ev_handle* h, const ResnetW& w, const float* X, int ldx, const LevelBufs& L, const float* temb, int tstride) {
    Epi e; e.gn_part = L.GNP;
    if (launch_conv(h, w.c1r, X, ldx, L.AR, 512, L.g, e)) return 1;
    if (launch_gn(h, L.AR, 512, L.Bf, 256, w.g1, w.b1, L.rm, temb, nullptr, 0, L.g, 256, 1, L.GNP, tstride)) return 1;
    if (launch_conv(h, w.c2, L.Bf, 256, L.A, 256, L.g, e)) return 1;
    return launch_gn(h, L.A, 256, L.H, 256, w.g2, w.b2, L.rm, nullptr, L.AR + 256, 512, L.g, 256, 2, L.GNP);
}

int run_resnet0(ev_handle* h, const EstimatorW& W, const float* X, int ldx, const LevelBufs& L, const float* temb, int tstride, const float* C1RMS) {
    const ResnetW& w = W.rn[0];
    Epi e;
    { Epi e1; e1.R = C1RMS; e1.ldr = 512; if (launch_conv(h, W.rn0_c1r_x, X, ldx, L.AR, 512, L.g, e1)) return 1; }
    if (launch_gn(h, L.AR, 512, L.Bf, 256, w.g1, w.b1, L.rm, temb, nullptr, 0, L.g, 256, 1, nullptr, tstride)) return 1;
    e.gn_part = L.GNP;
    if (launch_conv(h, w.c2, L.Bf, 256, L.A, 256, L.g, e)) return 1;
    return launch_gn(h, L.A, 256, L.H, 256, w.g2, w.b2, L.rm, nullptr, L.AR + 256, 512, L.g, 256, 2, L.GNP);
}

int run_transformer(ev_handle* h, const TransW& w, const LevelBufs& L, float* Z, int ldz, int heads) {
    Epi e;
    const bool fuse = h->fuse_mlp && g_rows32(L.g) >= h->fuse_mlp_min_tiles;
    const bool aok = attn_out_ok(h, w.out, L.g, heads);
    int packed = 0;
    if (fuse) {
        if (launch_mlp(h, 1, L.H, w.ln1g, w.ln1b, w.qkv, nullptr, nullptr, nullptr, nullptr, nullptr, L.QKV, 384, L.g,
                       (aok && h->attn_h16 && w.out.Wh) ? w.qkv_scale : nullptr, &packed)) return 1;
    } else {
        if (launch_ln(h, L.H, 256, L.LN, 256, w.ln1g, w.ln1b, L.g)) return 1;
        if (launch_conv(h, w.qkv, L.LN, 256, L.QKV, 384, L.g, e)) return 1;
    }
    if (aok) {
        if (launch_attn_out(h, L.QKV, 384, w.out, L.H, 256, L.rm, L.g, heads, packed ? w.qkv_scale : nullptr)) return 1;
    } else {
        if (launch_attn(h, L.QKV, 384, L.ATT, 128, L.rm, L.g, heads, L.ATTP)) return 1;
        Epi eo; eo.R = L.H; eo.ldr = 256;
        if (launch_conv(h, w.out, L.ATT, 128, L.H, 256, L.g, eo)) return 1;
    }
    if (fuse) return launch_mlp(h, 0, L.H, w.ln3g, w.ln3b, w.ff1, &w.ff2, w.alpha, w.binv, L.H, L.rm, Z, ldz, L.g);
    if (launch_ln(h, L.H, 256, L.LN, 256, w.ln3g, w.ln3b, L.g)) return 1;
    Epi e1; e1.act = ACT_SNAKE; e1.act_a = w.alpha; e1.act_b = w.binv;
    if (launch_conv(h, w.ff1, L.LN, 256, L.FF, 1024, L.g, e1)) return 1;
    Epi e2; e2.R = L.H; e2.ldr = 256; e2.mask2 = 1; e2.rowmask = L.rm;
    return launch_conv(h, w.ff2, L.FF, 1024, Z, ldz, L.g, e2);
}

int run_estimator(ev_handle* h, EstBufs& b, int step, float dt, bool euler, const float* tproj = nullptr, int tstride = 0) {
    const EstimatorW& w = h->est;
    const int heads = h->dims.heads;
    LevelBufs L0{b.A0, b.B0, b.R0, b.H0, b.LN0, b.QKV0, b.ATT0, b.FF0, b.rm0, b.g0, b.AR0, b.ATTP, b.GNP};
    LevelBufs L1{b.A1, b.B1, b.R1, b.H1, b.LN1, b.QKV1, b.ATT1, b.FF1, b.rm1, b.g1, b.AR1, b.ATTP, b.GNP};
    const float* tp = (tproj ? tproj : b.tproj) + (size_t)step * 1536;
    if (run_resnet0(h, w, b.X0, w.in_ch, L0, tp + 0 * 256, tstride, b.C1RMS)) return 1;
    if (run_transformer(h, w.tr[0], L0, b.CAT1 + 256, 512, heads)) return 1;
    {
        Epi e; e.isplit_log2 = 8; e.isstride = 512; e.mask1 = 1; e.rowmask = b.rm1;
        if (launch_conv(h, w.down0, b.CAT1 + 256, 1024, b.D1, 256, b.g1, e)) return 1;
    }
    if (run_resnet(h, w.rn[1], b.D1, 256, L1, tp + 1 * 256, tstride)) return 1;
    if (run_transformer(h, w.tr[1], L1, b.CAT0 + 256, 512, heads)) return 1;
    { Epi e; e.mask1 = 1; e.rowmask = b.rm1; if (launch_conv(h, w.down1, b.CAT0 + 256, 512, b.D2, 256, b.g1, e)) return 1; }
    if (run_resnet(h, w.rn[2], b.D2, 256, L1, tp + 2 * 256, tstride)) return 1;
    if (run_transformer(h, w.tr[2], L1, b.M1, 256, heads)) return 1;
    if (run_resnet(h, w.rn[3], b.M1, 256, L1, tp + 3 * 256, tstride)) return 1;
    if (run_transformer(h, w.tr[3], L1, b.CAT0, 512, heads)) return 1;
    if (run_resnet(h, w.rn[4], b.CAT0, 512, L1, tp + 4 * 256, tstride)) return 1;
    if (run_transformer(h, w.tr[4], L1, b.UU, 256, heads)) return 1;
    {
        Epi e; e.osplit_log2 = 8; e.osstride = 512; e.mask1 = 1; e.rowmask = b.rm0; e.mmul = 2;
        if (launch_conv(h, w.up0, b.UU, 256, b.CAT1, 1024, b.g1, e)) return 1;
    }
    if (run_resnet(h, w.rn[5], b.CAT1, 512, L0, tp + 5 * 256, tstride)) return 1;
    if (run_transformer(h, w.tr[5], L0, b.U1, 256, heads)) return 1;
    { Epi e; e.mask1 = 1; e.rowmask = b.rm0; if (launch_conv(h, w.up1, b.U1, 256, b.F0, 256, b.g0, e)) return 1; }
    { Epi e; if (launch_conv(h, w.fin_conv, b.F0, 256, b.A0, 256, b.g0, e)) return 1; }
    if (launch_gn(h, b.A0, 256, b.G0, 256, w.fin_g, w.fin_b, b.rm0, nullptr, nullptr, 0, b.g0, 256, 0)) return 1;
    if (euler) {
        Epi e; e.mask1 = 1; e.rowmask = b.rm0; e.scale = dt; e.R = b.state; e.ldr = 80; e.Y2 = b.X0; e.ldy2 = w.in_ch;
        return launch_conv(h, w.fin_proj, b.G0, 256, b.state, 80, b.g0, e);
    }
    Epi e; e.mask1 = 1; e.rowmask = b.rm0;
    return launch_conv(h, w.fin_proj, b.G0, 256, b.V0, 80, b.g0, e);
}

int run_time_mlp(ev_handle* h, EstBufs& b, const std::vector<float>& ts) {
    const EstimatorW& w = h->est;
    const int nt = (int)ts.size(), dim = w.in_ch, half = dim / 2;
    std::vector<float> emb((size_t)nt * dim);
    const float ne = -(float)(log(10000.0) / (double)(half - 1));
    for (int i = 0; i < nt; ++i) {
        const float st = 1000.0f * ts[i];
        for (int k = 0; k < half; ++k) {
            const float f = expf((float)k * ne);
            const float a = st * f;
            emb[(size_t)i * dim + k] = sinf(a);
            emb[(size_t)i * dim + half + k] = cosf(a);
        }
    }
    {
        const size_t bytes = emb.size() * sizeof(float);
        hipStreamCaptureStatus cst = hipStreamCaptureStatusNone;
        const bool capturing = h->stream && hipStreamIsCapturing(h->stream, &cst) == hipSuccess && cst == hipStreamCaptureStatusActive;
        const float* src = nullptr;
        if (capturing) {
            if (!h->cap_pool || bytes > h->cap_stride) return fail(h, "ev_cfm_decode under stream capture: %d Euler steps exceed the capture staging (%zu bytes per call)", nt, h->cap_stride);
            int slot = -1;
            for (int k = 0; k < h->cap_used; ++k) if (h->cap_nt[k] == nt) slot = k;
            if (slot < 0) {
                if (h->cap_used >= EV_CAPTURE_SLOTS) return fail(h, "ev_cfm_decode under stream capture: this handle has already captured calls with %d different step counts (their staging is never recycled)", EV_CAPTURE_SLOTS);
                slot = h->cap_used++;
                h->cap_nt[slot] = nt;
                memcpy((char*)h->cap_pool + (size_t)slot * h->cap_stride, emb.data(), bytes);
            }
            src = (const float*)((const char*)h->cap_pool + (size_t)slot * h->cap_stride);
        } else {
            const int slot = (h->temb_slot ^= 1);
            if (h->temb_cap[slot] < bytes) {
                if (h->temb_host[slot]) { HIPCHK(h, hipEventSynchronize(h->temb_ev[slot])); HIPCHK(h, hipHostFree(h->temb_host[slot])); h->temb_host[slot] = nullptr; h->temb_cap[slot] = 0; }
                const size_t want = std::max(bytes, (size_t)64 * dim * sizeof(float));
                HIPCHK(h, hipHostMalloc((void**)&h->temb_host[slot], want, hipHostMallocDefault));
                h->temb_cap[slot] = want;
                ++h->n_allocs;
                if (!h->temb_ev[slot]) HIPCHK(h, hipEventCreateWithFlags(&h->temb_ev[slot], hipEventDisableTiming));
            } else {
                HIPCHK(h, hipEventSynchronize(h->temb_ev[slot]));
            }
            memcpy(h->temb_host[slot], emb.data(), bytes);
            src = h->temb_host[slot];
        }
        HIPCHK(h, hipMemcpyAsync(b.temb_in, src, bytes, hipMemcpyHostToDevice, h->stream));
        if (!capturing) HIPCHK(h, hipEventRecord(h->temb_ev[h->temb_slot], h->stream));
    }
    Geom gt{nt, nt, 0, nt};
    Epi e1; e1.act = ACT_SILU;
    if (launch_conv(h, w.t1, b.temb_in, dim, b.temb_a, 1024, gt, e1)) return 1;
    Epi e2; e2.act = ACT_MISH;
    if (launch_conv(h, w.t2, b.temb_a, 1024, b.temb_b, 1024, gt, e2)) return 1;
    Epi e3;
    return launch_conv(h, w.tmlp, b.temb_b, 1024, b.tproj, 1536, gt, e3);
}

void prep_masks(ev_handle* h, EstBufs& b, const int32_t* d_len) {
    hipStream_t st = h->stream;
    hipLaunchKernelGGL(rowmask_kernel, dim3((b.g0.nrows + 255) / 256), dim3(256), 0, st, b.rm0, d_len, b.g0.nrows, b.g0.S, b.g0.P, b.g0.T, 1);
    hipLaunchKernelGGL(rowmask_kernel, dim3((b.g1.nrows + 255) / 256), dim3(256), 0, st, b.rm1, d_len, b.g1.nrows, b.g1.S, b.g1.P, b.g1.T, 2);
}

int prep_rest(ev_handle* h, EstBufs& b, const float* d_spk) {
    const EstimatorW& w = h->est;
    hipStream_t st = h->stream;
    if (w.in_ch > 160) {
        const int C = w.in_ch - 160;
        const long tot = (long)b.g0.nrows * C;
        hipLaunchKernelGGL(bcast_rows_kernel, dim3((unsigned)((tot + 255) / 256)), dim3(256), 0, st, d_spk, b.X0, w.in_ch, 160, C, b.g0.nrows, b.g0.S, b.g0.P, b.g0.T, (const float*)b.rm0);
    }
    HIPCHK(h, hipGetLastError());
// ... 205 lines not shown
        hipLaunchKernelGGL(mel_project_kernel, dim3((T + 31) / 32, B), dim3(256), smem, st, (const float*)SPEC, (const int*)mb.span, (const float*)mb.wts, d_mel,
                           mb.n_mels, mb.nb, T, S, P, out_scale, out_shift);
    }
    HIPCHK(h, hipGetLastError());
    return 0;
}

int run_mas(ev_handle* h, bool fused, const float* d_value, const float* d_mu_x, const float* d_y, const int32_t* d_xlen, const int32_t* d_ylen,
            int B, int Tx, int Ty, float* d_attn, int32_t* d_dur, float* d_mu_y, float* d_logp) {
    constexpr size_t LDS_MAX = 160 * 1024;
    const int C = h->dims.n_feats;
    if (B <= 0 || B > 65535 || Tx <= 0 || Ty <= 0 || Tx > 4096 || !d_xlen || !d_ylen || (fused ? (!d_mu_x || !d_y || C <= 0) : !d_value))
        return fail(h, "bad arguments B=%d Tx=%d Ty=%d (1 <= B <= 65535, 1 <= Tx <= 4096, 1 <= Ty)", B, Tx, Ty);
    MasParams p{};
    p.value = d_value; p.mu_x = d_mu_x; p.y = d_y; p.xlen = d_xlen; p.ylen = d_ylen; p.logp = fused ? d_logp : nullptr; p.dur = d_dur;
    p.C = C; p.Tx = Tx; p.Ty = Ty; p.TxP = round_up(Tx, 2) + 1; p.nxw = (Tx + 63) / 64;
    p.cst = (float)(-0.5 * log(2.0 * 3.14159265358979323846) * C);
    int W = 16;
    auto plan = [&](int w) {
        p.off_col = fused ? round_up(C * w, 4) : 0;
        p.off_tile = p.off_col + round_up(2 * p.TxP, 4);
        p.off_bits = p.off_tile + round_up(w * p.TxP, 4);
        return (size_t)p.off_bits * sizeof(float);
    };
    if (plan(16) > LDS_MAX) W = 4;
    size_t smem = plan(W);
    if (smem > LDS_MAX) return fail(h, "alignment search: Tx=%d does not fit the LDS plan", Tx);
    const size_t bit_bytes = (size_t)Ty * p.nxw * sizeof(unsigned long long);
    const bool bits_in_lds = smem + bit_bytes <= LDS_MAX;
    if (bits_in_lds) smem += bit_bytes;
    const size_t idx_bytes = ((size_t)B * Ty * sizeof(int32_t) + 255) / 256 * 256;
    if (scratch_acquire(h, h->mas_ws, idx_bytes + (bits_in_lds ? 0 : (size_t)B * bit_bytes))) return 1;
    p.idx = (int32_t*)h->mas_ws.p;
    p.gbits = bits_in_lds ? nullptr : (unsigned long long*)(h->mas_ws.p + idx_bytes);
    const int NT = std::min(1024, std::max(256, round_up(Tx, 64)));
    hipStream_t st = h->stream;
    auto go = [&](auto kernel_tag) {
        constexpr int w = decltype(kernel_tag)::value;
        if (fused) launch<mas_search_kernel<w, true>>(h->device, dim3(B), dim3(NT), smem, st, p);
        else launch<mas_search_kernel<w, false>>(h->device, dim3(B), dim3(NT), smem, st, p);
    };
    dispatch<16, 4>(W, go);
    HIPCHK(h, hipGetLastError());
    if (d_attn || d_mu_y) {
        hipLaunchKernelGGL(mas_fill_kernel, dim3((Ty + 255) / 256, B, d_attn ? (Tx + 63) / 64 : 1), dim3(256), 0, st, (const int32_t*)p.idx, d_mu_x, d_attn, d_mu_y, C, Tx, Ty);
        HIPCHK(h, hipGetLastError());
    }
    return 0;
}

}

extern "C" {

int ev_abi_version(void) { return EV_ABI_VERSION; }

int ev_create(ev_handle** out, int device, const ev_model_dims* dims) {
    if (!out || !dims) return 1;
    *out = nullptr;
    int ndev = 0;
    if (hipGetDeviceCount(&ndev) != hipSuccess || device < 0 || device >= ndev) return 2;
    if (hipSetDevice(device) != hipSuccess) return 3;
    ev_handle* h = new ev_handle();
    h->device = device;
    h->dims = *dims;
    { const char* fp = getenv("EV_FUSE_PAIRS"); if (fp && *fp == '0') h->fuse_pairs = false; }
    { const char* fp = getenv("EV_FUSE_MLP"); if (fp && *fp == '0') h->fuse_mlp = false; }
    { const char* fp = getenv("EV_FUSE_ATTN"); if (fp && *fp == '0') h->fuse_attn = false; }
    if (getenv("EV_NO_ATTN_H16")) h->attn_h16 = false;
    if (getenv("EV_NO_CHAIN")) h->use_chain = false;
    { const char* fp = getenv("EV_FUSE_MLP_MIN"); if (fp && *fp) h->fuse_mlp_min_tiles = atoi(fp); }
    { const char* fp = getenv("EV_MRF_STREAMS_MAX"); if (fp && *fp) h->mrf_max_frames = atoi(fp); }
    if (getenv("EV_NO_AMAX")) h->use_amax = false;
    { const char* sp = getenv("EV_SPLIT"); if (sp && *sp) { const int t = atoi(sp); h->split_terms = (t == 0 || t == 3 || t == 6 || t == 9 || t == 16) ? t : 16; } }
    { const char* fp = getenv("EV_NO_SK_BALANCE"); if (fp && *fp && *fp != '0') h->sk_balance = false; }
    { const char* fp = getenv("EV_SK_SPIN"); if (fp && *fp) h->sk_spin = atoi(fp); }
    { const char* fp = getenv("EV_SK_WGS"); if (fp && *fp) h->sk_wgs = std::min(3, std::max(1, atoi(fp))); }
    { const char* fp = getenv("EV_FORCE_CFG"); if (fp && *fp) h->force_cfg = atoi(fp); }
    if (getenv("EV_NO_LEAN")) h->lean = false;
    if (getenv("EV_NO_SK")) h->small_sk = false;
    if (getenv("EV_NO_SK32_LEAN")) h->sk32_lean = false;
    if (getenv("EV_NO_GN_STATS")) h->gn_stats = false;
    if (getenv("EV_NO_QKV_H16")) h->qkv_h16 = false;
    if (getenv("EV_NO_ATTN_SK")) h->attn_sk = false;
    { const char* fp = getenv("EV_ATTN_TPW"); if (fp) h->attn_tpw = std::max(1, atoi(fp)); }
    if (getenv("EV_FULL_REZERO")) h->full_rezero = true;
    { const char* fp = getenv("EV_RB2_MINKEEP"); if (fp) h->rb2_minkeep = atoi(fp); }
    if (hipDeviceGetAttribute(&h->ncu, hipDeviceAttributeMultiprocessorCount, device) != hipSuccess) h->ncu = 0;
    if (dims->n_feats != 80 || dims->channels != 256 || dims->head_dim != 64 || dims->heads != 2) {
        delete h;
        return 4;
    }
    *out = h;
    return 0;
}

void ev_destroy(ev_handle* h) {
    if (!h) return;
    hipSetDevice(h->device);
    hipDeviceSynchronize();
    for (void* p : h->owned) hipFree(p);
    if (h->ws) hipFree(h->ws);
    if (h->cap_pool) hipHostFree(h->cap_pool);
    for (auto& c : h->tproj_cache) hipFree(c.d);
    h->tproj_cache.clear();
    if (h->sk_ctrl) hipFree(h->sk_ctrl);
    if (h->sk_part) hipFree(h->sk_part);
    for (hipEvent_t e : h->ev_pool) hipEventDestroy(e);
    if (h->enc_ws.p) hipFree(h->enc_ws.p);
    if (h->mas_ws.p) hipFree(h->mas_ws.p);
    if (h->stat_ws.p) hipFree(h->stat_ws.p);
    if (h->dn_ws.p) hipFree(h->dn_ws.p);
    if (h->bad_ids_host) hipHostFree(h->bad_ids_host);
    for (int i = 0; i < 2; ++i) { if (h->temb_ev[i]) hipEventDestroy(h->temb_ev[i]); if (h->temb_host[i]) hipHostFree(h->temb_host[i]); }
    for (int i = 0; i < 2; ++i) if (h->mrf_stream[i]) hipStreamDestroy(h->mrf_stream[i]);
    for (int i = 0; i < 4; ++i) if (h->mrf_ev[i]) hipEventDestroy(h->mrf_ev[i]);
    delete h;
}

const char* ev_last_error(ev_handle* h) { return h ? h->err.c_str() : "null handle"; }

static int build_map(ev_handle* h, const float* blob, const ev_tensor_index* index, size_t n, TensorMap& m) {
    if (!blob || !index) return fail(h, "null blob/index");
    for (size_t i = 0; i < n; ++i) {
        HostTensor t;
        t.p = blob + index[i].offset;
        t.ndim = index[i].ndim;
        if (t.ndim < 0 || t.ndim > 4) return fail(h, "bad ndim for %s", index[i].name);
        for (int d = 0; d < t.ndim; ++d) t.shape[d] = index[i].shape[d];
        m[index[i].name] = t;
    }
    return 0;
}

int ev_load_estimator(ev_handle* h, const float* blob, const ev_tensor_index* index, size_t n) {
    if (!h) return 1;
    HIPCHK(h, hipSetDevice(h->device));
    TensorMap m;
    if (build_map(h, blob, index, n, m)) return 1;
    if (ensure_sk(h, false)) return 1;
    if (!h->tproj_cache.empty()) {
        HIPCHK(h, hipDeviceSynchronize());
        for (auto& c : h->tproj_cache) hipFree(c.d);
        h->tproj_cache.clear();
    }
    EstimatorW& w = h->est;
    w.loaded = false;
#define T_(k) find(h, m, k)
#define REQ(x) do { if (x) return 1; } while (0)
    const HostTensor* l1 = T_("time_mlp.linear_1.weight");
    if (!l1) return 1;
    w.in_ch = (int)l1->shape[1];
    if (w.in_ch != 2 * h->dims.n_feats + h->dims.spk_emb_dim) return fail(h, "estimator in_channels %d != 2*n_feats + spk_emb_dim", w.in_ch);
    {
        const HostTensor *b1 = T_("time_mlp.linear_1.bias"), *l2 = T_("time_mlp.linear_2.weight"), *b2 = T_("time_mlp.linear_2.bias");
        if (!b1 || !l2 || !b2) return 1;
        REQ(pack_linear_stack(h, w.t1, {l1}, {b1}));
        REQ(pack_linear_stack(h, w.t2, {l2}, {b2}));
    }
    const char* rn_names[6] = {"down_blocks.0.0", "down_blocks.1.0", "mid_blocks.0.0", "mid_blocks.1.0", "up_blocks.0.0", "up_blocks.1.0"};
    const char* tr_names[6] = {"down_blocks.0.1.0", "down_blocks.1.1.0", "mid_blocks.0.1.0", "mid_blocks.1.1.0", "up_blocks.0.1.0", "up_blocks.1.1.0"};
    std::vector<const HostTensor*> mw, mb;
    for (int i = 0; i < 6; ++i) {
        const std::string p = rn_names[i];
        const HostTensor *c1w = T_(p + ".block1.block.0.weight"), *c1b = T_(p + ".block1.block.0.bias");
        const HostTensor *c2w = T_(p + ".block2.block.0.weight"), *c2b = T_(p + ".block2.block.0.bias");
// ... 393 lines not shown
            if (hipMalloc((void**)&d, bytes) == hipSuccess) {
                ++h->n_allocs;
                HIPCHK(h, hipMemcpyAsync(d, b.tproj, bytes, hipMemcpyDeviceToDevice, h->stream));
                h->tproj_cache.push_back({n_steps, d});
            } else (void)hipGetLastError();
        }
    }
    for (int s = 0; s < n_steps; ++s)
        if (run_estimator(h, b, s, dts[s], true, tproj)) return 1;
    dim3 grid((Tp + 31) / 32, (80 + 31) / 32, B);
    if (d_dec) hipLaunchKernelGGL(fm_to_cm_kernel, grid, dim3(256), 0, h->stream, (const float*)b.state, 80, 0, d_dec, 80, Tp, b.g0.S, b.g0.P, 1.0f, 0.0f);
    if (d_out) hipLaunchKernelGGL(fm_to_cm_kernel, grid, dim3(256), 0, h->stream, (const float*)b.state, 80, 0, d_out, 80, Tp, b.g0.S, b.g0.P, out_scale, out_shift);
    HIPCHK(h, hipGetLastError());
    return 0;
}

int ev_cfm_decode(ev_handle* h, const float* d_mu, const int32_t* d_lengths, const float* d_spk, const float* d_z,
                  int B, int Tp, int n_steps, float out_scale, float out_shift, float* d_out, void* stream) {
    if (h && !d_out) return fail(h, "null tensor argument");
    return cfm_decode_impl(h, d_mu, d_lengths, d_spk, d_z, B, Tp, n_steps, nullptr, out_scale, out_shift, d_out, stream);
}

int ev_cfm_decode2(ev_handle* h, const float* d_mu, const int32_t* d_lengths, const float* d_spk, const float* d_z,
                   int B, int Tp, int n_steps, float* d_dec, float mel_std, float mel_mean, float* d_mel, void* stream) {
    return cfm_decode_impl(h, d_mu, d_lengths, d_spk, d_z, B, Tp, n_steps, d_dec, mel_std, mel_mean, d_mel, stream);
}

int ev_reserve(ev_handle* h, int B, int Tx_max, int Tp_max, int T_voc_max, void* stream) {
    if (!h) return 1;
    HIPCHK(h, hipSetDevice(h->device));
    if (B <= 0 || Tx_max < 0 || Tp_max < 0 || T_voc_max < 0 || (Tp_max & 3)) return fail(h, "ev_reserve: bad shape B=%d Tx=%d Tp=%d (multiple of 4) T_voc=%d", B, Tx_max, Tp_max, T_voc_max);
    h->stream = (hipStream_t)stream;
    if (ensure_sk(h, false)) return 1;
    if (Tp_max > 0 || T_voc_max > 0) {
        size_t need = plan_all(h, nullptr, B, Tp_max, T_voc_max, nullptr, nullptr);
        if (T_voc_max > 0 && h->mrf_max_frames > 0) {
            const int tv_ms = (int)std::min<long>(T_voc_max, h->mrf_max_frames / B);
            if (tv_ms > 0) need = std::max(need, plan_all(h, nullptr, B, Tp_max, tv_ms, nullptr, nullptr));
        }
        if (need > h->ws_bytes) {
            if (h->captured) return fail(h, "ev_reserve: this handle holds a captured ev_cfm_decode, its workspace cannot be replaced");
            if (grow_ws(h, need, false)) return 1;
        }
    }
    if (Tx_max > 0 && h->enc.loaded) {
        const size_t n = (size_t)B * (Tx_max + 4);
        const TextEncW& w = h->enc;
        const size_t need = (n * (1 + 3 * w.nch + 3 * w.C + 2 * w.dp1.Cout + 3 * w.C + w.C + w.ffc + 80 + 4) + 1024) * sizeof(float);
        if (scratch_acquire(h, h->enc_ws, need)) return 1;
    }
    if (T_voc_max > 0) {
        const size_t n = (size_t)B * (T_voc_max + 4 + 8);
        const size_t need = (n * (256 + 1032 + 256) + 1024) * sizeof(float);
        if (scratch_acquire(h, h->dn_ws, need)) return 1;
        if (denoiser_init(h)) return 1;
    }
    if (h->est.loaded) {
        const size_t bytes = (size_t)std::max(64, h->max_steps) * h->est.in_ch * sizeof(float);
        for (int slot = 0; slot < 2; ++slot) {
            if (h->temb_cap[slot] >= bytes) continue;
            if (h->temb_host[slot]) { HIPCHK(h, hipEventSynchronize(h->temb_ev[slot])); HIPCHK(h, hipHostFree(h->temb_host[slot])); h->temb_host[slot] = nullptr; h->temb_cap[slot] = 0; }
            HIPCHK(h, hipHostMalloc((void**)&h->temb_host[slot], bytes, hipHostMallocDefault));
            h->temb_cap[slot] = bytes;
            if (!h->temb_ev[slot]) HIPCHK(h, hipEventCreateWithFlags(&h->temb_ev[slot], hipEventDisableTiming));
            HIPCHK(h, hipEventRecord(h->temb_ev[slot], h->stream));
        }
    }
    if (h->voc.loaded && h->mrf_max_frames > 0 && !h->mrf_stream[0]) {
        for (int c = 0; c < 2; ++c) HIPCHK(h, hipStreamCreateWithFlags(&h->mrf_stream[c], hipStreamNonBlocking));
        for (int c = 0; c < 4; ++c) HIPCHK(h, hipEventCreateWithFlags(&h->mrf_ev[c], hipEventDisableTiming));
    }
    return 0;
}

int64_t ev_alloc_count(ev_handle* h) { return h ? h->n_allocs : -1; }

int ev_dbg_sk_stats(ev_handle* h, uint32_t* out3) {
    if (!h || !out3) return 1;
    out3[0] = out3[1] = out3[2] = 0;
    if (!h->sk_ctrl) return 0;
    HIPCHK(h, hipSetDevice(h->device));
    HIPCHK(h, hipDeviceSynchronize());
    HIPCHK(h, hipMemcpy(out3, h->sk_ctrl, 3 * sizeof(uint32_t), hipMemcpyDeviceToHost));
    return 0;
}

int64_t ev_dbg_sk_taken(ev_handle* h) {
    if (!h) return -1;
    if (!h->sk_ctrl) return 0;
    uint32_t v = 0;
    if (hipSetDevice(h->device) != hipSuccess || hipDeviceSynchronize() != hipSuccess || hipMemcpy(&v, h->sk_ctrl + 3, sizeof v, hipMemcpyDeviceToHost) != hipSuccess) { (void)hipGetLastError(); return -1; }
    return (int64_t)v;
}

int ev_estimator(ev_handle* h, const float* d_x, const float* d_mu, const int32_t* d_lengths, const float* d_spk, float t,
                 int B, int Tp, float* d_v, void* stream) {
    if (!h) return 1;
    HIPCHK(h, hipSetDevice(h->device));
    if (check_cfm_args(h, B, Tp)) return 1;
    h->stream = (hipStream_t)stream;
    EstBufs b;
    if (ensure_ws(h, B, Tp, 0, &b, nullptr)) return 1;
    if (prep_inputs(h, b, d_x, d_mu, d_lengths, d_spk, B, Tp)) return 1;
    if (run_time_mlp(h, b, std::vector<float>(1, t))) return 1;
    if (run_estimator(h, b, 0, 0.f, false)) return 1;
    dim3 grid((Tp + 31) / 32, (80 + 31) / 32, B);
    hipLaunchKernelGGL(fm_to_cm_kernel, grid, dim3(256), 0, h->stream, (const float*)b.V0, 80, 0, d_v, 80, Tp, b.g0.S, b.g0.P, 1.0f, 0.0f);
    HIPCHK(h, hipGetLastError());
    return 0;
}

static int rows_begin(ev_handle* h, const char* who, int B, int Tp, void* stream, EstBufs* b) {
    if (check_cfm_args(h, B, Tp)) return 1;
    h->stream = (hipStream_t)stream;
    hipStreamCaptureStatus cst = hipStreamCaptureStatusNone;
    if (h->stream && hipStreamIsCapturing(h->stream, &cst) == hipSuccess && cst == hipStreamCaptureStatusActive)
        return fail(h, "%s is eager-only: under stream capture its host-to-device copy of the B times would replay from recycled staging "
                       "(see run_time_mlp); call it outside the capture", who);
    const int64_t before = h->n_allocs;
    if (B > h->max_steps) {
        if (h->captured) return fail(h, "%s: %d rows exceed the %d time slots the workspace is planned for and the handle holds a captured call: "
                                        "its workspace cannot be re-planned", who, B, h->max_steps);
        while (B > h->max_steps) h->max_steps *= 2;
        h->ws_B = -1;
    }
    bool ring_grew = false;
    const size_t bytes = (size_t)std::max(64, h->max_steps) * h->est.in_ch * sizeof(float);
    for (int slot = 0; slot < 2; ++slot) {
        if (h->temb_cap[slot] >= (size_t)B * h->est.in_ch * sizeof(float)) continue;
        if (h->temb_host[slot]) { HIPCHK(h, hipEventSynchronize(h->temb_ev[slot])); HIPCHK(h, hipHostFree(h->temb_host[slot])); h->temb_host[slot] = nullptr; h->temb_cap[slot] = 0; }
        HIPCHK(h, hipHostMalloc((void**)&h->temb_host[slot], bytes, hipHostMallocDefault));
        h->temb_cap[slot] = bytes;
        if (!h->temb_ev[slot]) HIPCHK(h, hipEventCreateWithFlags(&h->temb_ev[slot], hipEventDisableTiming));
        HIPCHK(h, hipEventRecord(h->temb_ev[slot], h->stream));
        ring_grew = true;
    }
    if (ensure_ws(h, B, Tp, 0, b, nullptr)) return 1;
    if (ring_grew && h->n_allocs == before) ++h->n_allocs;
    return 0;
}

int ev_estimator_rows(ev_handle* h, const float* d_x, const float* d_mu, const int32_t* d_lengths, const float* d_spk, const float* t,
                      int B, int Tp, float* d_v, void* stream) {
    if (!h) return 1;
    HIPCHK(h, hipSetDevice(h->device));
    EstBufs b;
    if (rows_begin(h, "ev_estimator_rows", B, Tp, stream, &b)) return 1;
    if (!d_x || !d_mu || !t || !d_v || (h->dims.spk_emb_dim > 0 && !d_spk)) return fail(h, "null tensor argument");
    if (prep_inputs(h, b, d_x, d_mu, d_lengths, d_spk, B, Tp)) return 1;
    if (run_time_mlp(h, b, std::vector<float>(t, t + B))) return 1;
    if (run_estimator(h, b, 0, 0.f, false, nullptr, 1536)) return 1;
    dim3 grid((Tp + 31) / 32, (80 + 31) / 32, B);
    hipLaunchKernelGGL(fm_to_cm_kernel, grid, dim3(256), 0, h->stream, (const float*)b.V0, 80, 0, d_v, 80, Tp, b.g0.S, b.g0.P, 1.0f, 0.0f);
    HIPCHK(h, hipGetLastError());
    return 0;
}

int ev_cfm_loss(ev_handle* h, const float* d_x1, const float* d_mu_y, const int32_t* d_ylen, const float* d_spk, const float* d_z, const float* t,
                int B, int Ty, float sigma_min, double* d_row_sums, float* d_v, void* stream) {
    if (!h) return 1;
    HIPCHK(h, hipSetDevice(h->device));
    if (Ty < 1 || Ty > (1 << 30)) return fail(h, "ev_cfm_loss: bad shape B=%d Ty=%d", B, Ty);
    const int Tp = (Ty + 3) / 4 * 4;
    EstBufs b;
    if (rows_begin(h, "ev_cfm_loss", B, Tp, stream, &b)) return 1;
    if (!d_x1 || !d_mu_y || !d_ylen || !d_z || !t || !d_row_sums || (h->dims.spk_emb_dim > 0 && !d_spk)) return fail(h, "null tensor argument");
// ... 723 lines not shown
```

emojivoice_amd/csrc/ev_kernels.h:

```cpp
#pragma once
#include <hip/hip_runtime.h>
#include <stdint.h>
#include <type_traits>

typedef float f32x16 __attribute__((ext_vector_type(16)));
typedef float f32x4 __attribute__((ext_vector_type(4)));
typedef int i32x4 __attribute__((ext_vector_type(4)));

#define EV_MAX_TAPS 16
#define EV_BK 32
#define EV_LDK 36
#define EV_WROWS 128
#define EV_SK_MAXF4(TW) ((TW) == 4 ? (64 + 64) * 8 * 8 : 16 * 512)
#define EV_HALO 64

enum { ACT_NONE = 0, ACT_LRELU = 1, ACT_TANH = 2, ACT_SILU = 3, ACT_MISH = 4, ACT_SNAKE = 5 };

struct SkCtl {
    unsigned* ctrl;
    unsigned* flags;
    float* part;
    int part_floats;
    int q, r;
    int spin_limit;
    unsigned* claims;
    unsigned seq;
    int lds_word;
};

struct ConvParams {
    const float* X; int ldx; int Cin;
    int isplit_log2, isstride;
    const float* W; int Mpad; int Kpad;
    const void* Wh; float wh_scale;
    const void* Wq;
    const void* Wx;
    const float* bias;
    float* Y; int ldy; int Cout;
    int osplit_log2, osstride;
    int mmul;
    int nrows;
    int S, P, T;
    int ntaps; int off[EV_MAX_TAPS];
    int halo_lo, halo_hi;
    const int2* taplist; int tl_stride;
    const int* nact_tab;
    int mtiles, ntiles;
    float pro_slope; int pro_lrelu;
    int act; float act_slope; const float* act_a; const float* act_b;
    int mask1; float scale; const float* R; int ldr; int accum; int div3;
    int act2_lrelu; float act2_slope; int mask2;
    const float* rowmask;
    float* Y2; int ldy2;
    int ktaps_n, plane_bytes, koff0, kdoff;
    float* gn_part;
    int kstack_mt, kstack_tap;
    int sk_kb;
    unsigned* ymax; int ymax_mul;
    const unsigned* rmax;
    const unsigned* yold;
    const unsigned* xmax; int xmax_n;
    int stagger_slots;
    unsigned long long* stamps;
    int dbg;
    SkCtl sk;
};


__device__ __forceinline__ __amdgpu_buffer_rsrc_t ev_rsrc(const void* p) {
    return __builtin_amdgcn_make_buffer_rsrc((void*)p, 0, 0xffffffff, 0x00020000);
}
__device__ __forceinline__ f32x4 ev_bload4(__amdgpu_buffer_rsrc_t r, unsigned voff_bytes, unsigned soff_bytes) {
    return __builtin_bit_cast(f32x4, __builtin_amdgcn_raw_buffer_load_b128(r, (int)voff_bytes, (int)soff_bytes, 0));
}
__device__ __forceinline__ float ev_bload1(__amdgpu_buffer_rsrc_t r, unsigned voff_bytes, unsigned soff_bytes) {
    return __builtin_bit_cast(float, __builtin_amdgcn_raw_buffer_load_b32(r, (int)voff_bytes, (int)soff_bytes, 0));
}
__device__ __forceinline__ void ev_bstore4(__amdgpu_buffer_rsrc_t r, unsigned voff_bytes, f32x4 v) {
    __builtin_amdgcn_raw_buffer_store_b128(__builtin_bit_cast(i32x4, v), r, (int)voff_bytes, 0, 0);
}
__device__ __forceinline__ void ev_bstore1(__amdgpu_buffer_rsrc_t r, unsigned voff_bytes, float v) {
    __builtin_amdgcn_raw_buffer_store_b32(__builtin_bit_cast(int, v), r, (int)voff_bytes, 0, 0);
}

__device__ __forceinline__ int2 ev_uniform(int2 v) {
    return make_int2(__builtin_amdgcn_readfirstlane(v.x), __builtin_amdgcn_readfirstlane(v.y));
}
__device__ __forceinline__ int2 ev_tap_at(int2 tlv, int i) {
    return make_int2(__builtin_amdgcn_readlane(tlv.x, i), __builtin_amdgcn_readlane(tlv.y, i));
}

__device__ __forceinline__ float ev_lrelu(float v, float s) {
    float r;
    asm("v_max_f32 %0, %1, %2" : "=v"(r) : "v"(v), "v"(v * s));
    return r;
}
__device__ __forceinline__ float ev_mish(float x) {
    const float w = expf(fminf(x, 20.f));
    const float n = w * (w + 2.f);
    return x > 20.f ? x : x * __fdividef(n, n + 2.f);
}
__device__ __forceinline__ float ev_silu(float x) { return x / (1.f + expf(-x)); }

__device__ __forceinline__ float ev_sin2(float u) {
#ifdef EV_SIN2_HW
    const float kk = rintf(u * 0.318309886183790672f);
    float rr = fmaf(kk, -3.1415927410125732421875f, u);
    rr = fmaf(kk, 8.742277657347586e-8f, rr);
    return fmaf(__builtin_amdgcn_cosf(rr * 0.318309886183790672f), -0.5f, 0.5f);
#endif
    const float k = rintf(u * 0.63661977236758134f);
    float r = fmaf(k, -1.57079637050628662109375f, u);
    r = fmaf(k, 4.371138828673793e-8f, r);
    r = fmaf(k, 1.7763568394002505e-15f, r);
    const float z = r * r;
    const float q = fmaf(fmaf(-1.9515295891e-4f, z, 8.3321608736e-3f), z, -1.6666654611e-1f);
    const float sn = fmaf(q * z, r, r);
    const float s2 = sn * sn;
    return ((int)k & 1) ? 1.f - s2 : s2;
}

__device__ __forceinline__ float ev_act(float v, int act, float slope, const float* a, const float* b, int co) {
    switch (act) {
        case ACT_LRELU: return ev_lrelu(v, slope);
        case ACT_TANH: return tanhf(v);
        case ACT_SILU: return ev_silu(v);
        case ACT_MISH: return ev_mish(v);
        case ACT_SNAKE: return fmaf(b[co], ev_sin2(v * a[co]), v);
        default: return v;
    }
}

__device__ __forceinline__ int ev_xcd_remap(int id, int nwg) {
    int q = nwg >> 3, r = nwg & 7, xcd = id & 7, within = id >> 3;
    int base = (xcd < r) ? xcd * (q + 1) : r * (q + 1) + (xcd - r) * q;
    return base + within;
}

// ... 33 lines not shown
            bool ok[NB];
#pragma unroll
            for (int q = 0; q < NB; ++q) {
                const int n = nw0 + j * 32 + (pb + q) * RPP + er;
                const int t = (n % p.S) - p.P;
                ok[q] = co_ok && n < p.nrows && t >= 0 && t < p.T && n >= win_lo && n < win_hi;
                f32x4 z = {0.f, 0.f, 0.f, 0.f};
                rr[q] = z; yo[q] = z;
                if (ok[q]) {
                    if (full) {
                        if (p.R) rr[q] = ev_bload4(rR, ((unsigned)n * p.ldr + col) * 4u, 0);
                        if (p.accum) yo[q] = ev_bload4(rY, ((unsigned)n * p.ldy + col) * 4u, 0);
                    } else {
#pragma unroll
                        for (int e = 0; e < 4; ++e) {
                            if (co + e < p.Cout) {
                                if (p.R) rr[q][e] = ev_bload1(rR, ((unsigned)n * p.ldr + col + e) * 4u, 0);
                                if (p.accum) yo[q][e] = ev_bload1(rY, ((unsigned)n * p.ldy + col + e) * 4u, 0);
                            }
                        }
                    }
                }
            }
            if (pb == 0) {
                ev_lds_barrier();
#pragma unroll
                for (int i = 0; i < TM; ++i)
#pragma unroll
                    for (int g = 0; g < 4; ++g) {
                        f32x4 q4 = {acc[i][j][4 * g], acc[i][j][4 * g + 1], acc[i][j][4 * g + 2], acc[i][j][4 * g + 3]};
                        *(f32x4*)(Es + li * ELD + i * 32 + 8 * g + 4 * lh) = q4;
                    }
                ev_lds_barrier();
            }
#pragma unroll
            for (int q = 0; q < NB; ++q) {
                if (!ok[q]) continue;
                const int rl = (pb + q) * RPP + er;
                const int n = nw0 + j * 32 + rl;
                const f32x4 a = *(const f32x4*)(Es + rl * ELD + ec);
                float v[4] = {a[0], a[1], a[2], a[3]};
                const float rm = p.rowmask ? p.rowmask[(size_t)n * p.mmul + sp] : 1.f;
#pragma unroll
                for (int e = 0; e < 4; ++e) {
                    const int c = (co + e < p.Cout) ? co + e : p.Cout - 1;
                    float x = v[e] + bs[e];
                    if constexpr (FULL_ACT) { if (p.act) x = ev_act(x, p.act, p.act_slope, p.act_a, p.act_b, c); }
                    else { if (p.act == ACT_LRELU) x = ev_lrelu(x, p.act_slope); }
                    if (p.mask1) x *= rm;
                    x *= p.scale;
                    if (p.R) x += rr[q][e];
                    if (p.accum) x += yo[q][e];
                    if (p.div3) x = x / 3.0f;
                    if (p.act2_lrelu) x = ev_lrelu(x, p.act2_slope);
                    if (p.mask2) x *= rm;
                    v[e] = x;
                }
                if (full) {
                    f32x4 o = {v[0], v[1], v[2], v[3]};
                    ev_bstore4(rY, ((unsigned)n * p.ldy + col) * 4u, o);
                    if (p.Y2) { f32x4 o2 = {v[0] * rm, v[1] * rm, v[2] * rm, v[3] * rm}; ev_bstore4(rY2, ((unsigned)n * p.ldy2 + col) * 4u, o2); }
                } else {
#pragma unroll
                    for (int e = 0; e < 4; ++e) {
                        if (co + e < p.Cout) {
                            ev_bstore1(rY, ((unsigned)n * p.ldy + col + e) * 4u, v[e]);
                            if (p.Y2) ev_bstore1(rY2, ((unsigned)n * p.ldy2 + col + e) * 4u, v[e] * rm);
                        }
                    }
                }
            }
        }
    }
}

#ifndef EV_CONV_MIN_WAVES
#define EV_CONV_MIN_WAVES 1
#endif
__device__ __forceinline__ float ev_div3(float x) {
    const float q = x * 0.333333343267440796f;
    return fmaf(fmaf(-3.f, q, x), 0.333333343267440796f, q);
}
struct EvNoHook { __device__ __forceinline__ void operator()() const {} };
template <int TM, int TN, int MODE, class Hook, class PutSlab>
__device__ __forceinline__ void conv_epilogue_lean_impl(const ConvParams& p, PutSlab put_slab, float* Es, int mw0, int nw0, int lane,
                                                        int win_lo, int win_hi, Hook after_issue) {
    constexpr int EC = TM * 32, ELD = EC + 4, C4 = EC / 4, RPP = 64 / C4, NP = 32 / RPP;
    asm volatile("" : "+v"(lane));
    const int er = lane / C4, ec = (lane % C4) * 4;
    const int co = mw0 + ec;
    const bool co_ok = co < p.Cout;
    const __amdgpu_buffer_rsrc_t rY = ev_rsrc(p.Y), rR = ev_rsrc(p.R);
    const bool has_r = p.R != nullptr;
    const bool do_act = p.act == ACT_LRELU;
    constexpr bool SNAKE = MODE == 2, ACC = MODE == 3;
    f32x4 sa = {0.f, 0.f, 0.f, 0.f}, sb = sa;
    if constexpr (SNAKE) {
        if (co_ok) { sa = *(const f32x4*)(p.act_a + co); sb = *(const f32x4*)(p.act_b + co); }
    }
    const int n0l = nw0 + er;
    int t = n0l % p.S;
    if (t < 0) t += p.S;
    t -= p.P;
    const int sp = (p.osplit_log2 >= 31) ? 0 : (co >> p.osplit_log2);
    const unsigned col = (p.osplit_log2 >= 31) ? (unsigned)co : (unsigned)sp * (unsigned)p.osstride + (unsigned)(co & ((1 << p.osplit_log2) - 1));
    unsigned yoff = ((unsigned)n0l * p.ldy + col) * 4u, roff = ((unsigned)n0l * p.ldr + col) * 4u;
    const unsigned ystep = (unsigned)(RPP * p.ldy) * 4u, rstep = (unsigned)(RPP * p.ldr) * 4u;
    f32x4 rr[NP], ra[ACC ? NP : 1];
    float rmk[NP];
    const bool mk = p.mask1 || p.mask2;
    const __amdgpu_buffer_rsrc_t rM = ev_rsrc(p.rowmask);
    const __amdgpu_buffer_rsrc_t rRe = has_r ? rR : rY, rMe = mk ? rM : rY;
    const bool use_acc = ACC && p.accum;
    int nn = n0l;
    unsigned ro = roff, ao = yoff;
    auto issue_one = [&](int q) {
        const bool inr = co_ok && nn >= 0 && nn < p.nrows;
        rr[q] = ev_bload4(rRe, (has_r && inr) ? ro : 0u, 0);
        rmk[q] = ev_bload1(rMe, (mk && inr) ? ((unsigned)nn * (unsigned)p.mmul + (unsigned)sp) * 4u : 0u, 0);
        if constexpr (ACC) {
            ra[q] = ev_bload4(rY, (use_acc && inr) ? ao : 0u, 0);
            ao += ystep;
        }
        nn += RPP;
        ro += rstep;
    };
    const int lim = p.S - p.P;
#pragma unroll
    for (int q = 0; q < NP; ++q) issue_one(q);
    after_issue();
    ev_lds_barrier();
#pragma unroll
    for (int j = 0; j < TN; ++j) {
        put_slab(j);
        asm volatile("s_waitcnt lgkmcnt(0)" ::: "memory");
#pragma unroll
        for (int q = 0; q < NP; ++q) {
            const int rl = q * RPP + er;
            const int n = n0l + (j * NP + q) * RPP;
            f32x4 v = *(const f32x4*)(Es + rl * ELD + ec);
            const bool ok = co_ok && t >= 0 && t < p.T && n < p.nrows && n >= win_lo && n < win_hi;
            if constexpr (SNAKE) {
#pragma unroll
                for (int e = 0; e < 4; ++e) v[e] = fmaf(sb[e], ev_sin2(v[e] * sa[e]), v[e]);
            } else if (do_act) {
                v[0] = fmaxf(v[0], v[0] * p.act_slope); v[1] = fmaxf(v[1], v[1] * p.act_slope);
                v[2] = fmaxf(v[2], v[2] * p.act_slope); v[3] = fmaxf(v[3], v[3] * p.act_slope);
            }
            if (p.mask1) v *= rmk[q];
            if (has_r) v += rr[q];
            if (p.mask2) v *= rmk[q];
            if constexpr (ACC) {
                if (use_acc) v += ra[q];
                if (p.div3) { v[0] = ev_div3(v[0]); v[1] = ev_div3(v[1]); v[2] = ev_div3(v[2]); v[3] = ev_div3(v[3]); }
                if (p.act2_lrelu) {
                    v[0] = fmaxf(v[0], v[0] * p.act2_slope); v[1] = fmaxf(v[1], v[1] * p.act2_slope);
                    v[2] = fmaxf(v[2], v[2] * p.act2_slope); v[3] = fmaxf(v[3], v[3] * p.act2_slope);
                }
            }
            if (ok) ev_bstore4(rY, yoff, v);
            if (j + 1 < TN) issue_one(q);
            t += RPP; t -= (t >= lim) ? p.S : 0; t -= (t >= lim) ? p.S : 0;
            yoff += ystep;
        }
        asm volatile("s_waitcnt lgkmcnt(0)" ::: "memory");
    }
}
template <int TM, int TN, int MODE = 1, class Hook = EvNoHook>
__device__ __forceinline__ void conv_epilogue_lean(const ConvParams& p, f32x16 (&acc)[TM][TN], float* Es, int mw0, int nw0, int lane,
                                                   int win_lo = -0x7fffffff, int win_hi = 0x7fffffff, Hook after_issue = Hook()) {
    auto put = [&](int j) {
        constexpr int ELD = TM * 32 + 4;
        const int li = lane & 31, lh = lane >> 5;
#pragma unroll
        for (int i = 0; i < TM; ++i)
#pragma unroll
            for (int g = 0; g < 4; ++g) {
                f32x4 q4 = {acc[i][j][4 * g], acc[i][j][4 * g + 1], acc[i][j][4 * g + 2], acc[i][j][4 * g + 3]};
                *(f32x4*)(Es + li * ELD + i * 32 + 8 * g + 4 * lh) = q4;
            }
    };
    conv_epilogue_lean_impl<TM, TN, MODE>(p, put, Es, mw0, nw0, lane, win_lo, win_hi, after_issue);
}
template <int TM, int TN, int MODE = 1>
__device__ __forceinline__ void conv_epilogue_lean_q(const ConvParams& p, f32x4 (&acc)[2 * TM][2 * TN], float* Es, int mw0, int nw0, int lane,
                                                     int win_lo = -0x7fffffff, int win_hi = 0x7fffffff) {
    auto put = [&](int j) {
        constexpr int ELD = TM * 32 + 4;
        const int f = lane & 15, kg = lane >> 4;
#pragma unroll
        for (int b2 = 0; b2 < 2; ++b2)
#pragma unroll
            for (int a = 0; a < 2 * TM; ++a) *(f32x4*)(Es + (b2 * 16 + f) * ELD + a * 16 + 4 * kg) = acc[a][2 * j + b2];
    };
    conv_epilogue_lean_impl<TM, TN, MODE>(p, put, Es, mw0, nw0, lane, win_lo, win_hi, EvNoHook());
}

typedef __attribute__((address_space(1))) unsigned ev_gu32;
__device__ __forceinline__ int sk_start(const SkCtl& c, int x) {
    return x * c.q + (x < c.r ? x : c.r);
}
__device__ __forceinline__ unsigned sk_tag(const SkCtl& c) {
    return c.ctrl ? (unsigned)__builtin_amdgcn_readfirstlane((int)__hip_atomic_load((ev_gu32*)c.ctrl, __ATOMIC_RELAXED, __HIP_MEMORY_SCOPE_AGENT)) + 1u : 0u;
}
__device__ __forceinline__ f32x4 ev_bload4_sc1(__amdgpu_buffer_rsrc_t r, unsigned voff_bytes) {
    return __builtin_bit_cast(f32x4, __builtin_amdgcn_raw_buffer_load_b128(r, (int)voff_bytes, 0, 16));
}
__device__ __forceinline__ void ev_bstore4_sc1(__amdgpu_buffer_rsrc_t r, unsigned voff_bytes, f32x4 v) {
    __builtin_amdgcn_raw_buffer_store_b128(__builtin_bit_cast(i32x4, v), r, (int)voff_bytes, 0, 16);
}
__device__ __forceinline__ f32x4 ev_bload4_sc1(__amdgpu_buffer_rsrc_t r, unsigned voff_bytes, unsigned soff_bytes) {
    return __builtin_bit_cast(f32x4, __builtin_amdgcn_raw_buffer_load_b128(r, (int)voff_bytes, (int)soff_bytes, 16));
}
__device__ __forceinline__ void ev_bstore4_sc1(__amdgpu_buffer_rsrc_t r, unsigned voff_bytes, unsigned soff_bytes, f32x4 v) {
    __builtin_amdgcn_raw_buffer_store_b128(__builtin_bit_cast(i32x4, v), r, (int)voff_bytes, (int)soff_bytes, 16);
}
__device__ __forceinline__ void sk_publish(const SkCtl& c, int g, unsigned tag, int tid) {
    asm volatile("s_waitcnt vmcnt(0) lgkmcnt(0)\n\ts_barrier" ::: "memory");
    asm volatile("" : "+s"(tag));
    if (tid == 0) __hip_atomic_store((ev_gu32*)(c.flags + g), tag, __ATOMIC_RELAXED, __HIP_MEMORY_SCOPE_AGENT);
}
__device__ __forceinline__ bool sk_wait(const SkCtl& c, int gi, unsigned tag, int tid, int* word) {
    if (tid == 0) {
        int ok = 0;
        for (int spins = 0; spins < c.spin_limit; ++spins) {
            if (__hip_atomic_load((ev_gu32*)(c.flags + gi), __ATOMIC_RELAXED, __HIP_MEMORY_SCOPE_AGENT) == tag) { ok = 1; break; }
            __builtin_amdgcn_s_sleep(16);
        }
        __builtin_amdgcn_fence(__ATOMIC_ACQUIRE, "agent");
        if (!ok) atomicAdd(c.ctrl + 2, 1u);
        *word = ok;
    }
    asm volatile("s_waitcnt vmcnt(0) lgkmcnt(0)\n\ts_barrier" ::: "memory");
    const bool ok = __builtin_amdgcn_readfirstlane(*word) != 0;
    asm volatile("s_waitcnt lgkmcnt(0)\n\ts_barrier" ::: "memory");
    return ok;
}
__device__ __forceinline__ unsigned sk_claim_start(const SkCtl& c, int g, int tid) {
    unsigned prev = 0;
    if (c.claims && tid == 0) prev = __hip_atomic_fetch_max((ev_gu32*)(c.claims + g), 2u * c.seq, __ATOMIC_RELAXED, __HIP_MEMORY_SCOPE_AGENT);
    return prev;
}
__device__ __forceinline__ bool sk_claim_taken(const SkCtl& c, unsigned prev, int tid, int* word) {
    if (!c.claims) return false;
    if (tid == 0) *word = (prev == 2u * c.seq + 1u) ? 1 : 0;
    asm volatile("s_waitcnt vmcnt(0) lgkmcnt(0)\n\ts_barrier" ::: "memory");
    const bool taken = __builtin_amdgcn_readfirstlane(*word) != 0;
    asm volatile("s_waitcnt lgkmcnt(0)\n\ts_barrier" ::: "memory");
    return taken;
}
__device__ __forceinline__ int sk_wait_many(const SkCtl& c, int gi, int n, unsigned tag, int tid, int* word) {
    if (tid < 64) {
        unsigned long long up = 0, taken = 0;
        const unsigned long long want = n >= 64 ? ~0ull : ((1ull << n) - 1ull);
        if (c.claims) {
            bool mine = false;
            if (tid < n) {
                ev_gu32* w = (ev_gu32*)(c.claims + gi + tid);
                const unsigned started = 2u * c.seq, stolen = started + 1u;
                unsigned v = __hip_atomic_load(w, __ATOMIC_RELAXED, __HIP_MEMORY_SCOPE_AGENT);
                if (v == stolen) mine = true;
                else if (v != started) {
                    unsigned expect = v;
                    mine = __hip_atomic_compare_exchange_strong(w, &expect, stolen, __ATOMIC_RELAXED, __ATOMIC_RELAXED, __HIP_MEMORY_SCOPE_AGENT) || expect == stolen;
                }
            }
            taken = __ballot(mine);
        }
        for (int spins = 0; spins < c.spin_limit; ++spins) {
            const unsigned v = tid < n ? __hip_atomic_load((ev_gu32*)(c.flags + gi + tid), __ATOMIC_RELAXED, __HIP_MEMORY_SCOPE_AGENT) : tag;
            up = __ballot(v == tag) & ~taken;
            const unsigned long long miss = ~up & want;
            if (!miss || ((taken >> __builtin_ctzll(miss)) & 1ull)) break;
            __builtin_amdgcn_s_sleep(16);
        }
        __builtin_amdgcn_fence(__ATOMIC_ACQUIRE, "agent");
        const unsigned long long miss = ~up & want;
        const int ready = miss ? __builtin_ctzll(miss) : n;
// ... 1474 lines not shown
                ldB(B0, brow, 0);
                for (int ti = 0; ti < nact; ++ti) {
                    const bool last_tap = (ti + 1 == nact);
                    const int2 ntv = last_tap ? tv_first : ev_tap_at(tlv, ti + 1);
                    const char* nbrow = bbase + ntv.y * EVH_RSB;
                    const bool have_next = !(last_tap && ch + 1 == cB);
                    const unsigned nap = have_next ? a_off(ntv.x, last_tap ? ch * 4 + 4 : ch * 4) : a_off(tv_first.x, cA * 4);
                    ldB(B1, brow, 1);
                    __builtin_amdgcn_sched_barrier(0);
                    evh_mma<TM, TN>(acc, A0, B0);
                    __builtin_amdgcn_sched_barrier(0);
                    ldAp(A0, nap);
                    ldB(B0, brow, 2);
                    __builtin_amdgcn_sched_barrier(0);
                    evh_mma<TM, TN>(acc, A1, B1);
                    __builtin_amdgcn_sched_barrier(0);
                    ldAp(A1, nap + 2048u);
                    ldB(B1, brow, 3);
                    __builtin_amdgcn_sched_barrier(0);
                    evh_mma<TM, TN>(acc, A2, B0);
                    __builtin_amdgcn_sched_barrier(0);
                    ldAp(A2, nap + 4096u);
                    ldB(B0, nbrow, 0);
                    __builtin_amdgcn_sched_barrier(0);
                    evh_mma<TM, TN>(acc, A3, B1);
                    __builtin_amdgcn_sched_barrier(0);
                    ldAp(A3, nap + 6144u);
                    brow = nbrow;
                }
            }
            const float acc_out = 1.0f / (p.wh_scale * xs);
#pragma unroll
            for (int a = 0; a < TM; ++a)
#pragma unroll
                for (int b = 0; b < TN; ++b)
#pragma unroll
                    for (int r = 0; r < 16; ++r) acc[a][b][r] *= acc_out;
            auto acc_io = [&](unsigned base, int mode) {
#pragma unroll
                for (int a = 0; a < TM; ++a)
#pragma unroll
                    for (int b = 0; b < TN; ++b)
#pragma unroll
                        for (int q = 0; q < 4; ++q) {
                            const unsigned soff = base + (unsigned)((a * TN + b) * 4 + q) * 1024u;
                            if (mode == 0) {
                                const f32x4 v = {acc[a][b][4 * q], acc[a][b][4 * q + 1], acc[a][b][4 * q + 2], acc[a][b][4 * q + 3]};
                                ev_bstore4_sc1(rPart, pelem, soff, v);
                            } else {
                                const f32x4 v = ev_bload4_sc1(rPart, pelem, soff);
#pragma unroll
                                for (int e = 0; e < 4; ++e) acc[a][b][4 * q + e] += v[e];
                            }
                        }
            };
            if (spilled) { acc_io((unsigned)g * pslot + pslot / 2, 1); spilled = false; }
            if (c0 != 0) {
                acc_io((unsigned)g * pslot, 0);
                pend_pub = true;
                break;
            }
            bool again = false;
            while (c1 < nchunks) {
                int n = 0;
                while (n < 64 && gi + n < (int)gridDim.x && sk_start(p.sk, gi + n) < tile_end) ++n;
                if (n == 0) break;
                const int ready = sk_wait_many(p.sk, gi, n, get_tag(), tid, skw);
                for (int k = 0; k < ready; ++k) acc_io((unsigned)(gi + k) * pslot, 1);
                gi += ready;
                if (ready < n) {
                    const int sgi = sk_start(p.sk, gi);
                    int egi = sk_start(p.sk, gi + 1);
                    egi = egi < tile_end ? egi : tile_end;
                    acc_io((unsigned)g * pslot + pslot / 2, 0);
                    asm volatile("s_waitcnt vmcnt(0)" ::: "memory");
                    cA = sgi - t * nchunks; cB = egi - t * nchunks;
                    spilled = true; again = true;
                    ++gi;
                    break;
                }
            }
            if (again) continue;
            __builtin_amdgcn_s_setprio(3);
            conv_epilogue_lean<TM, TN, LEAN>(p, acc, smem + wave * (32 * (TM * 32 + 4)), m0 + wm * (TM * 32), n0 + wn * (TN * 32), lane);
            __builtin_amdgcn_s_setprio(0);
            break;
        }
    }
    if (pend_pub) sk_publish(p.sk, g, get_tag(), tid);
    sk_arrive(p.sk, get_tag(), tid);
}


template <int KS, bool FULL_ACT, int LEAN, int TW = 4>
__global__ __launch_bounds__(64 * TW * KS) void conv_gemm_sk_kernel(const ConvParams pk) {
    static_assert(TW == 4 || TW == 1, "tile waves");
    constexpr int BM = TW == 4 ? 64 : 32, BN = BM, NTHR = 64 * TW * KS;
    constexpr int MAXPASS = EV_SK_MAXF4(TW) / NTHR;
    constexpr int NPRE = TW == 1 ? 4 : 1;
    extern __shared__ __attribute__((aligned(16))) float smem[];
    int2* taps = (int2*)smem;
    float* Xs = smem + 2 * EV_MAX_TAPS;
    ConvParams p = pk;
    asm volatile("" : "+s"(p.X), "+s"(p.ldx), "+s"(p.Cin), "+s"(p.isplit_log2), "+s"(p.isstride), "+s"(p.W), "+s"(p.Kpad), "+s"(p.bias),
                      "+s"(p.Y), "+s"(p.ldy), "+s"(p.Cout), "+s"(p.nrows), "+s"(p.S), "+s"(p.P), "+s"(p.T));
    asm volatile("" : "+s"(p.ntaps), "+s"(p.halo_lo), "+s"(p.halo_hi), "+s"(p.taplist), "+s"(p.tl_stride), "+s"(p.nact_tab), "+s"(p.mtiles),
                      "+s"(p.pro_slope), "+s"(p.pro_lrelu), "+s"(p.act), "+s"(p.act_slope), "+s"(p.act_a), "+s"(p.act_b), "+s"(p.mask1), "+s"(p.R));
    asm volatile("" : "+s"(p.ldr), "+s"(p.accum), "+s"(p.div3), "+s"(p.act2_lrelu), "+s"(p.act2_slope), "+s"(p.mask2), "+s"(p.rowmask),
                      "+s"(p.ktaps_n), "+s"(p.plane_bytes), "+s"(p.koff0), "+s"(p.kdoff), "+s"(p.sk_kb), "+s"(p.stamps), "+s"(p.dbg));

    const int tid = threadIdx.x, lane = tid & 63;
    const int wave = __builtin_amdgcn_readfirstlane(tid >> 6);
    const int tw = wave % TW, ks = wave / TW;
    const int wm = TW == 4 ? (tw >> 1) : 0, wn = TW == 4 ? (tw & 1) : 0;
    const int li = lane & 31, lh = lane >> 5;
    const int work = blockIdx.x;
    const int mt = work % p.mtiles, nt = work / p.mtiles;
    const int m0 = mt * BM, n0 = nt * BN;
    {
        int t_first = (n0 % p.S) - p.P;
        int dist;
        if (t_first >= 0 && t_first < p.T) dist = 0;
        else if (t_first < 0) dist = -t_first;
        else dist = p.S - (n0 % p.S) + p.P;
        if (dist >= BN || n0 + dist >= p.nrows) return;
    }
    if ((p.dbg & 16) && tid == 0) p.stamps[4 * blockIdx.x + 0] = __builtin_amdgcn_s_memrealtime();
#ifdef EV_NOPSLED
    asm volatile(".rept 1024\n s_nop 0\n .endr" ::: "memory");
#endif
    const bool ktp = p.ktaps_n > 0;
    const int2* tl = p.taplist + (size_t)mt * p.tl_stride;
    int nact = p.ntaps;
    if (!ktp && p.nact_tab) nact = __builtin_amdgcn_readfirstlane(p.nact_tab[mt]);
    if (!ktp && tid < nact) taps[tid] = tl[tid];
    const int nchunks = p.Kpad / EV_BK;
    const int KBs = p.sk_kb;
    const int LDKs = 32 * KBs + 4;
    const int xrows = BN + p.halo_lo + p.halo_hi;

    const int mt32 = (m0 + wm * 32) >> 5;
    const int KG8 = p.Kpad >> 3;
    const __amdgpu_buffer_rsrc_t rW = ev_rsrc(p.W), rX = ev_rsrc(p.X);
    const unsigned wlane = (unsigned)lane * 16u;
    const unsigned wbase = (unsigned)(mt32 * KG8) * 1024u;
    const int f4row = KBs * 8;
    const int nf4 = xrows * f4row;

    f32x4 A[NPRE][4];
    int2 tvs[NPRE];
    int cs[NPRE];
    int ti0 = 0, cn0 = ks;
    const int kb0 = nchunks < KBs ? nchunks : KBs;
    const int npre = __builtin_amdgcn_readfirstlane(ktp && kb0 > ks ? (((kb0 - ks + KS - 1) / KS) * nact < NPRE ? ((kb0 - ks + KS - 1) / KS) * nact : NPRE) : 0);
#pragma unroll
    for (int s = 0; s < NPRE; ++s) {
        tvs[s] = make_int2(0, 0); cs[s] = 0;
        if (s < npre) {
            const int2 tv = make_int2(ti0 * p.plane_bytes, p.koff0 + ti0 * p.kdoff);
            tvs[s] = tv; cs[s] = cn0;
            const unsigned ap = (unsigned)tv.x + wbase + (unsigned)(cn0 * 4) * 1024u;
            A[s][0] = ev_bload4(rW, wlane, ap); A[s][1] = ev_bload4(rW, wlane, ap + 1024u);
            A[s][2] = ev_bload4(rW, wlane, ap + 2048u); A[s][3] = ev_bload4(rW, wlane, ap + 3072u);
            if (++ti0 == nact) { ti0 = 0; cn0 += KS; }
        }
    }

// ... 1345 lines not shown
    const int g = blockIdx.y, tid = threadIdx.x, lane = tid & 63;
    const int t = blockIdx.x * 32 + (tid >> 3) - p.P, c4 = (tid & 7) * 4;
    const int cbase = g * 32 + c4;
    const bool live = t >= 0 && t < p.T;
    const size_t n = (size_t)p.P + (live ? t : 0);
    const f32x4 v = *(const f32x4*)(p.X + n * p.ldx + cbase);
    const f32x4 ga = *(const f32x4*)(p.gamma + cbase), be = *(const f32x4*)(p.beta + cbase);
    f32x4 te = {0.f, 0.f, 0.f, 0.f}, rr = te;
    if (p.mode == 1) te = *(const f32x4*)(p.temb + cbase);
    if (p.mode == 2) rr = *(const f32x4*)(p.R + n * p.ldr + cbase);
    const float m = p.rowmask[n];
    float na = 0.f, mean = 0.f, m2 = 0.f;
    for (int j0 = 0; j0 < ntiles; j0 += 64) {
        int pn = 0, pm = 0, pq = 0;
        if (j0 + lane < ntiles) {
            const int* pp = (const int*)(part + ((size_t)(j0 + lane) * 8 + g) * 4);
            pn = pp[0]; pm = pp[1]; pq = pp[2];
        }
        const int nj = ntiles - j0 < 64 ? ntiles - j0 : 64;
        for (int j = 0; j < nj; ++j) {
            const float nb = __int_as_float(__builtin_amdgcn_readlane(pn, j));
            const float mb = __int_as_float(__builtin_amdgcn_readlane(pm, j));
            const float qb = __int_as_float(__builtin_amdgcn_readlane(pq, j));
            if (nb > 0.f) {
                const float nn = na + nb, d = mb - mean, w = nb / nn;
                mean += d * w;
                m2 += qb + d * d * na * w;
                na = nn;
            }
        }
    }
    if (!live) return;
    const float rstd = 1.0f / sqrtf(m2 / na + p.eps);
    f32x4 o;
#pragma unroll
    for (int e = 0; e < 4; ++e) {
        float y = (v[e] - mean) * rstd * ga[e] + be[e];
        y = ev_mish(y) * m;
        if (p.mode == 1) y = (y + te[e]) * m;
        o[e] = y;
    }
    if (p.mode == 2) { o[0] += rr[0]; o[1] += rr[1]; o[2] += rr[2]; o[3] += rr[3]; }
    *(f32x4*)(p.Y + n * p.ldy + cbase) = o;
}

struct LNParams {
    const float* X; int ldx; float* Y; int ldy; const float* gamma; const float* beta;
    int nrows, S, P, T; float eps;
};

__device__ __forceinline__ f32x4 ev_ln256_row(f32x4 v, f32x4 g, f32x4 be, float eps) {
    float mean = wave_sum((v[0] + v[1]) + (v[2] + v[3])) * (1.0f / 256.0f);
    float d0 = v[0] - mean, d1 = v[1] - mean, d2 = v[2] - mean, d3 = v[3] - mean;
    float var = wave_sum((d0 * d0 + d1 * d1) + (d2 * d2 + d3 * d3)) * (1.0f / 256.0f);
    float rstd = 1.0f / sqrtf(var + eps);
    f32x4 o = {d0 * rstd * g[0] + be[0], d1 * rstd * g[1] + be[1], d2 * rstd * g[2] + be[2], d3 * rstd * g[3] + be[3]};
    return o;
}

__global__ __launch_bounds__(256) void layernorm256_kernel(const LNParams p) {
    const int lane = threadIdx.x & 63;
    const int n = blockIdx.x * 4 + (threadIdx.x >> 6);
    if (n >= p.nrows) return;
    const int t = (n % p.S) - p.P;
    if (t < 0 || t >= p.T) return;
    f32x4 v = *(const f32x4*)(p.X + (size_t)n * p.ldx + lane * 4);
    f32x4 g = *(const f32x4*)(p.gamma + lane * 4);
    f32x4 be = *(const f32x4*)(p.beta + lane * 4);
    *(f32x4*)(p.Y + (size_t)n * p.ldy + lane * 4) = ev_ln256_row(v, g, be, p.eps);
}

struct MlpParams {
    ConvParams ep;
    const float* X; int ldx;
    const float* ln_g; const float* ln_b; float ln_eps;
    const float* W1; const float* b1; int M1;
    const float* alpha; const float* binv;
    const float* W2;
    const void* W1h; const void* W2h; float w1_scale, w2_scale;
    const void* W1x; const void* W2x;
    int ntiles;
    SkCtl sk;
    int qkv_pack; float qkv_scale[3];
};

template <int MODE, int WPC>
__global__ __launch_bounds__(256, WPC) void ln_mlp_kernel(const MlpParams mp) {
    constexpr int NT = 32, C = 256, XLD = C + 4, HC = 128, HLD = HC + 4;
    const ConvParams& p = mp.ep;
    extern __shared__ __attribute__((aligned(16))) float smem[];
    float* Xs = smem;
    float* Hs = smem + NT * XLD;
    int* skw = (int*)(smem + NT * XLD + 4 * 32 * 36);
    const int tid = threadIdx.x, lane = tid & 63;
    const int wave = __builtin_amdgcn_readfirstlane(tid >> 6);
    const int li = lane & 31, lh = lane >> 5;
    const __amdgpu_buffer_rsrc_t rX = ev_rsrc(mp.X), rW1 = ev_rsrc(mp.W1), rW2 = ev_rsrc(MODE == 0 ? mp.W2 : mp.W1);
    const unsigned wlane = (unsigned)lane * 16u;
    const int nchunk = mp.M1 / HC;
    const int KG2 = mp.M1 / 8;
    const int g = blockIdx.x;
    const unsigned tag = MODE == 0 ? sk_tag(mp.sk) : 0u;
    int u = sk_start(mp.sk, g);
    const int ue = sk_start(mp.sk, g + 1);
    f32x4 F0, F1, F2, F3, F4, F5, F6, F7;
    auto ldP = [&](int ht, int kg) { return ev_bload4(rW1, wlane, (unsigned)(ht * (C / 8) + kg) * 1024u); };
    auto ldQ = [&](int hc, int kg, int a) { return ev_bload4(rW2, wlane, (unsigned)((wave * 2 + a) * KG2 + hc * (HC / 8) + kg) * 1024u); };
    const __amdgpu_buffer_rsrc_t rB1 = ev_rsrc(mp.b1), rSa = ev_rsrc(MODE == 0 ? mp.alpha : mp.b1), rSb = ev_rsrc(MODE == 0 ? mp.binv : mp.b1);
    const unsigned coff = (unsigned)(4 * lh) * 4u;
    const float* xrow = Xs + li * XLD + 4 * lh;
    const float* hrow = Hs + li * HLD + 4 * lh;
    const __amdgpu_buffer_rsrc_t rPart = ev_rsrc(mp.sk.part);
    const unsigned pslot = (unsigned)mp.sk.part_floats * 8u;
    const unsigned pelem = (unsigned)(wave * 8) * 1024u + wlane;
    bool pend_pub = false;

    while (u < ue) {
        const int t = u / nchunk, c0 = u - t * nchunk;
        const int c1 = (ue - u < nchunk - c0) ? c0 + (ue - u) : nchunk;
        u += c1 - c0;
        const int n0 = t * NT;
        {
            int t_first = (n0 % p.S) - p.P;
            int dist;
            if (t_first >= 0 && t_first < p.T) dist = 0;
            else if (t_first < 0) dist = -t_first;
            else dist = p.S - (n0 % p.S) + p.P;
            if (dist >= NT || n0 + dist >= p.nrows) continue;
        }
        F0 = ldP(c0 * 4 + wave, 0); F1 = ldP(c0 * 4 + wave, 1); F2 = ldP(c0 * 4 + wave, 2); F3 = ldP(c0 * 4 + wave, 3);
        F4 = ldP(c0 * 4 + wave, 4); F5 = ldP(c0 * 4 + wave, 5); F6 = ldP(c0 * 4 + wave, 6); F7 = ldP(c0 * 4 + wave, 7);
        ev_lds_barrier();
        {
            f32x4 xv[8];
#pragma unroll
            for (int q = 0; q < 8; ++q) {
                const int i = q * 256 + tid, r = i >> 6, c4 = (i & 63) * 4, gr = n0 + r;
                xv[q] = ev_bload4(rX, ((unsigned)(gr < p.nrows ? gr : 0) * mp.ldx + c4) * 4u, 0);
            }
#pragma unroll
            for (int q = 0; q < 8; ++q) {
                const int i = q * 256 + tid, r = i >> 6, c4 = (i & 63) * 4;
                *(f32x4*)(Xs + r * XLD + c4) = xv[q];
            }
        }
        if (pend_pub) {
            sk_publish(mp.sk, g, tag, tid);
            pend_pub = false;
        } else ev_lds_barrier();
        {
            const f32x4 gm = *(const f32x4*)(mp.ln_g + lane * 4), be = *(const f32x4*)(mp.ln_b + lane * 4);
#pragma unroll
            for (int r = 0; r < 8; ++r) {
                float* row = Xs + (wave * 8 + r) * XLD + lane * 4;
                *(f32x4*)row = ev_ln256_row(*(const f32x4*)row, gm, be, mp.ln_eps);
            }
        }
        ev_lds_barrier();

        int cA = c0, cB = c1;
        bool spilled = false;
        int gi = g + 1;
        const int tile_end = (t + 1) * nchunk;
        for (;;) {
            f32x16 acc2[2][1];
            if constexpr (MODE == 0) {
// ... 800 lines not shown
#pragma unroll
                        for (int o = 32; o > 0; o >>= 1) m2 = fmaxf(m2, __shfl_xor(m2, o, 64));
                        if (lane == 0) red[12 + wave] = m2;
                        ev_lds_barrier();
                        hm = fmaxf(fmaxf(red[12], red[13]), fmaxf(red[14], red[15]));
                    }
                    sh_lds = evh_scale_for(hm);
#pragma unroll
                    for (int jq = 0; jq < 8; ++jq) {
                        uint2 q0v, q1v;
                        evh_split4(hvs[jq] * sh_lds, q0v, q1v);
                        char* dst = Hb + ((jq >> 2) * 32 + li) * HRS + (wave * 32 + 8 * (jq & 3) + 4 * lh) * 2;
                        *(uint2*)(dst) = q0v; *(uint2*)(dst + 2 * HC) = q1v;
                    }
                    ev_lds_barrier();
                }
            }
            {
                const float f = 1.0f / cur_unit;
#pragma unroll
                for (int a = 0; a < 2; ++a)
#pragma unroll
                    for (int j = 0; j < 2; ++j)
#pragma unroll
                        for (int r = 0; r < 16; ++r) acc2[a][j][r] *= f;
            }
            auto acc_io = [&](unsigned base, int mode) {
#pragma unroll
                for (int a = 0; a < 2; ++a)
#pragma unroll
                    for (int j = 0; j < 2; ++j)
#pragma unroll
                        for (int q = 0; q < 4; ++q) {
                            const unsigned soff = base + (unsigned)((a * 2 + j) * 4 + q) * 1024u;
                            if (mode == 0) {
                                const f32x4 v = {acc2[a][j][4 * q], acc2[a][j][4 * q + 1], acc2[a][j][4 * q + 2], acc2[a][j][4 * q + 3]};
                                ev_bstore4_sc1(rPart, pelem, soff, v);
                            } else {
                                const f32x4 v = ev_bload4_sc1(rPart, pelem, soff);
#pragma unroll
                                for (int e = 0; e < 4; ++e) acc2[a][j][4 * q + e] += v[e];
                            }
                        }
            };
            if (spilled) { acc_io((unsigned)g * pslot + pslot / 2, 1); spilled = false; }
            if (c0 != 0) {
                acc_io((unsigned)g * pslot, 0);
                pend_pub = true;
                break;
            }
            bool again = false;
            while (c1 < nchunk) {
                int n = 0;
                while (n < 64 && gi + n < (int)gridDim.x && sk_start(mp.sk, gi + n) < tile_end) ++n;
                if (n == 0) break;
                const int ready = sk_wait_many(mp.sk, gi, n, tag, tid, skw);
                for (int k = 0; k < ready; ++k) acc_io((unsigned)(gi + k) * pslot, 1);
                gi += ready;
                if (ready < n) {
                    const int sgi = sk_start(mp.sk, gi);
                    int egi = sk_start(mp.sk, gi + 1);
                    egi = egi < tile_end ? egi : tile_end;
                    acc_io((unsigned)g * pslot + pslot / 2, 0);
                    asm volatile("s_waitcnt vmcnt(0)" ::: "memory");
                    cA = sgi - t * nchunk; cB = egi - t * nchunk;
                    spilled = true; again = true;
                    ++gi;
                    break;
                }
            }
            if (again) {
                const int ht0 = cA * 4 + wave;
                ldP(R0, ht0, 0); ldP(R1, ht0, 1); ldP(R2, ht0, 2); ldP(R3, ht0, 3); ldP(R4, ht0, 4); ldP(R5, ht0, 5); ldP(R6, ht0, 6); ldP(R7, ht0, 7);
                continue;
            }
            conv_epilogue_lean<2, 2, 1>(p, acc2, smem + wave * (32 * 68), wave * 64, n0, lane);
            break;
        }
    }
    if (pend_pub) sk_publish(mp.sk, g, tag, tid);
    sk_arrive(mp.sk, tag, tid);
}

template <int UNUSED = 0>
__global__ __launch_bounds__(256, 2) void ln_qkv_h16_kernel(const MlpParams mp) {
    constexpr int NT = 64, C = 256, TM = 3;
    constexpr int XRS = 4 * C + 16;
    const ConvParams& p = mp.ep;
    extern __shared__ __attribute__((aligned(16))) float smem[];
    char* Xb = (char*)smem;
    float* red = (float*)(Xb + NT * XRS);
    const int tid = threadIdx.x, lane = tid & 63;
    const int wave = __builtin_amdgcn_readfirstlane(tid >> 6);
    const int li = lane & 31, lh = lane >> 5;
    const __amdgpu_buffer_rsrc_t rX = ev_rsrc(mp.X), rW1 = ev_rsrc(mp.W1h), rB1 = ev_rsrc(mp.b1);
    const unsigned wlane = (unsigned)lane * 16u;
    const int n0 = blockIdx.x * NT;
    {
        int t_first = (n0 % p.S) - p.P;
        int dist;
        if (t_first >= 0 && t_first < p.T) dist = 0;
        else if (t_first < 0) dist = -t_first;
        else dist = p.S - (n0 % p.S) + p.P;
        if (dist >= NT || n0 + dist >= p.nrows) return;
    }
    f32x4 A[4][TM][2];
    auto ldA = [&](f32x4 (&dst)[TM][2], int sl) {
#pragma unroll
        for (int i = 0; i < TM; ++i)
#pragma unroll
            for (int pc = 0; pc < 2; ++pc) dst[i][pc] = ev_bload4(rW1, wlane, (unsigned)((((wave * TM + i) * (C / 16) + sl) * 2 + pc) * 1024));
    };
    ldA(A[0], 0); ldA(A[1], 1); ldA(A[2], 2);
    f32x4 bq[TM][4];
    const unsigned coff = (unsigned)(4 * lh) * 4u;
#pragma unroll
    for (int i = 0; i < TM; ++i)
#pragma unroll
        for (int q = 0; q < 4; ++q) bq[i][q] = ev_bload4(rB1, coff + (unsigned)((wave * TM + i) * 32 + 8 * q) * 4u, 0);
    float sx;
    {
        const f32x4 gm = *(const f32x4*)(mp.ln_g + lane * 4), be = *(const f32x4*)(mp.ln_b + lane * 4);
        f32x4 xv[16];
#pragma unroll
        for (int r = 0; r < 16; ++r) {
            const int gr = n0 + wave * 16 + r;
            xv[r] = ev_bload4(rX, ((unsigned)(gr < p.nrows ? gr : 0) * mp.ldx + lane * 4) * 4u, 0);
        }
        float mx = 0.f;
#pragma unroll
        for (int r = 0; r < 16; ++r) {
            xv[r] = ev_ln256_row(xv[r], gm, be, mp.ln_eps);
            mx = fmaxf(fmaxf(mx, fmaxf(fabsf(xv[r][0]), fabsf(xv[r][1]))), fmaxf(fabsf(xv[r][2]), fabsf(xv[r][3])));
        }
#pragma unroll
        for (int o = 32; o > 0; o >>= 1) mx = fmaxf(mx, __shfl_xor(mx, o, 64));
        if (lane == 0) red[wave] = mx;
        ev_lds_barrier();
        float tmx = fmaxf(fmaxf(red[0], red[1]), fmaxf(red[2], red[3]));
        if (!evh_is_finite(tmx)) {
            mx = 0.f;
#pragma unroll
            for (int r = 0; r < 16; ++r) mx = fmaxf(mx, evh_absmax4_finite(xv[r]));
#pragma unroll
            for (int o = 32; o > 0; o >>= 1) mx = fmaxf(mx, __shfl_xor(mx, o, 64));
            if (lane == 0) red[4 + wave] = mx;
            ev_lds_barrier();
            tmx = fmaxf(fmaxf(red[4], red[5]), fmaxf(red[6], red[7]));
        }
        sx = evh_scale_for(tmx);
#pragma unroll
        for (int r = 0; r < 16; ++r) {
            uint2 q0v, q1v;
            evh_split4(xv[r] * sx, q0v, q1v);
            char* dst = Xb + (wave * 16 + r) * XRS + lane * 8;
            *(uint2*)(dst) = q0v; *(uint2*)(dst + 2 * C) = q1v;
        }
    }
    ev_lds_barrier();
    const float u1 = mp.w1_scale * sx, inv1 = 1.0f / u1;
    f32x16 acc[TM][2];
#pragma unroll
    for (int i = 0; i < TM; ++i)
#pragma unroll
        for (int j = 0; j < 2; ++j)
#pragma unroll
            for (int q = 0; q < 4; ++q)
#pragma unroll
                for (int e = 0; e < 4; ++e) acc[i][j][4 * q + e] = bq[i][q][e] * u1;
    const char* xrow = Xb + li * XRS + 16 * lh;
    f32x4 B[2][2][2];
    auto ldB = [&](f32x4 (&dst)[2][2], int sl) {
#pragma unroll
        for (int pc = 0; pc < 2; ++pc)
#pragma unroll
            for (int j = 0; j < 2; ++j) dst[pc][j] = *(const f32x4*)(xrow + j * 32 * XRS + pc * (2 * C) + sl * 32);
    };
    constexpr int PA[3] = {0, 1, 0}, PB[3] = {1, 0, 0};
    ldB(B[0], 0);
#pragma unroll
    for (int sl = 0; sl < 16; ++sl) {
        if (sl + 1 < 16) ldB(B[(sl + 1) & 1], sl + 1);
        if (sl + 3 < 16) ldA(A[(sl + 3) & 3], sl + 3);
#pragma unroll
        for (int tt = 0; tt < 3; ++tt)
#pragma unroll
            for (int i = 0; i < TM; ++i)
#pragma unroll
                for (int j = 0; j < 2; ++j)
                    acc[i][j] = __builtin_amdgcn_mfma_f32_32x32x16_f16(__builtin_bit_cast(f16x8, A[sl & 3][i][PA[tt]]), __builtin_bit_cast(f16x8, B[sl & 1][PB[tt]][j]), acc[i][j], 0, 0, 0);
        __builtin_amdgcn_sched_barrier(0);
    }
    if (!mp.qkv_pack) {
#pragma unroll
        for (int i = 0; i < TM; ++i)
#pragma unroll
            for (int j = 0; j < 2; ++j)
#pragma unroll
                for (int r = 0; r < 16; ++r) acc[i][j][r] *= inv1;
    } else {
#pragma unroll
        for (int i = 0; i < TM; ++i) {
            const float f = inv1 * mp.qkv_scale[(wave * TM + i) >> 2];
#pragma unroll
            for (int j = 0; j < 2; ++j)
#pragma unroll
                for (int u = 0; u < 8; ++u) {
                    const float c0 = acc[i][j][2 * u] * f, c1 = acc[i][j][2 * u + 1] * f;
                    const _Float16 h0 = (_Float16)c0, h1 = (_Float16)c1;
                    const _Float16 l0 = (_Float16)(c0 - (float)h0), l1 = (_Float16)(c1 - (float)h1);
                    const f16x2 hh = {h0, h1}, ll = {l0, l1};
                    acc[i][j][2 * u] = __builtin_bit_cast(float, hh);
                    acc[i][j][2 * u + 1] = __builtin_bit_cast(float, ll);
                }
        }
    }
    {
        f32x16 a2[2][2];
#pragma unroll
        for (int i = 0; i < 2; ++i)
#pragma unroll
            for (int j = 0; j < 2; ++j) a2[i][j] = acc[i][j];
        conv_epilogue_lean<2, 2, 1>(p, a2, smem + wave * (32 * 68), wave * 96, n0, lane);
    }
    {
        f32x16 a1[1][2];
#pragma unroll
        for (int j = 0; j < 2; ++j) a1[0][j] = acc[2][j];
        conv_epilogue_lean<1, 2, 1>(p, a1, smem + wave * (32 * 68), wave * 96 + 64, n0, lane);
    }
}

struct AttnParams {
    const float* QKV; int ld;
    float* O; int ldo;
    const float* rowmask;
    int S, P, T, H; float scale;
};

#define ATT_LDK 68
__global__ __launch_bounds__(256) void attention_kernel(const AttnParams p) {
// ... 1537 lines not shown
```

include/emojivoice.h:

```cpp
#ifndef EMOJIVOICE_H
#define EMOJIVOICE_H

#include <stddef.h>
#include <stdint.h>

#ifdef __cplusplus
extern "C" {
#endif

#define EV_ABI_VERSION 4

typedef struct ev_handle ev_handle;

typedef struct ev_tensor_index {
    const char *name;
    uint64_t offset;
    int32_t ndim;
    int64_t shape[4];
} ev_tensor_index;

typedef struct ev_model_dims {
    int32_t n_feats;
    int32_t spk_emb_dim;
    int32_t channels;
// ... 5 lines not shown
int ev_create(ev_handle **out, int device, const ev_model_dims *dims);
void ev_destroy(ev_handle *h);
const char *ev_last_error(ev_handle *h);

int ev_load_estimator(ev_handle *h, const float *blob, const ev_tensor_index *index, size_t n);
int ev_load_vocoder(ev_handle *h, const float *blob, const ev_tensor_index *index, size_t n);

typedef struct ev_vocoder_config {
    int32_t resblock;
    int32_t num_levels;
    int32_t upsample_rates[4];
    int32_t upsample_kernel_sizes[4];
    int32_t resblock_kernel_sizes[3];
    int32_t resblock_dilations[3][3];
} ev_vocoder_config;
int ev_load_vocoder_cfg(ev_handle *h, const float *blob, const ev_tensor_index *index, size_t n, const ev_vocoder_config *cfg);
int ev_load_text_encoder(ev_handle *h, const float *blob, const ev_tensor_index *index, size_t n);

size_t ev_workspace_bytes(ev_handle *h, int B, int Tp_cfm, int T_voc);

int ev_cfm_decode(ev_handle *h, const float *d_mu, const int32_t *d_lengths, const float *d_spk, const float *d_z,
                  int B, int Tp, int n_steps, float out_scale, float out_shift, float *d_out, void *stream);

int ev_cfm_decode2(ev_handle *h, const float *d_mu, const int32_t *d_lengths, const float *d_spk, const float *d_z,
                   int B, int Tp, int n_steps, float *d_dec, float mel_std, float mel_mean, float *d_mel, void *stream);

int ev_reserve(ev_handle *h, int B, int Tx_max, int Tp_max, int T_voc_max, void *stream);
int64_t ev_alloc_count(ev_handle *h);

int ev_estimator(ev_handle *h, const float *d_x, const float *d_mu, const int32_t *d_lengths, const float *d_spk,
                 float t, int B, int Tp, float *d_v, void *stream);

int ev_text_encoder(ev_handle *h, const int64_t *d_ids, const int32_t *d_lengths, const float *d_spk, int B, int Tx,
                    float *d_mu, float *d_logw, void *stream);

int ev_text_encoder_status(ev_handle *h, void *stream);

int ev_align(ev_handle *h, const float *d_wceil, const float *d_mu_x, const int32_t *d_xlen, const int64_t *d_ylen,
             int B, int Tx, int Tp, float *d_mu_y, float *d_attn, void *stream);

int ev_set_mrf_streams_max(ev_handle *h, int max_frames);

int ev_hifigan(ev_handle *h, const float *d_mel, int B, int T, float *d_wav, void *stream);

int ev_stft_magnitude(ev_handle *h, const float *d_audio, int B, int L, float *d_mag, void *stream);
int ev_denoise(ev_handle *h, const float *d_audio, int B, int L, const float *d_bias_spec, float strength, float *d_out, void *stream);

int ev_load_mel_basis(ev_handle *h, const float *basis, int n_mels, int n_freq);
int ev_mel_spectrogram(ev_handle *h, const float *d_audio, int B, int L, float out_scale, float out_shift, float *d_mel, void *stream);

int ev_maximum_path(ev_handle *h, const float *d_value, const int32_t *d_xlen, const int32_t *d_ylen, int B, int Tx, int Ty,
                    float *d_path, int32_t *d_dur, void *stream);
int ev_log_prior(ev_handle *h, const float *d_mu_x, const float *d_y, int B, int Tx, int Ty, float *d_logp, void *stream);
int ev_mas_align(ev_handle *h, const float *d_mu_x, const float *d_y, const int32_t *d_xlen, const int32_t *d_ylen, int B, int Tx, int Ty,
                 float *d_attn, int32_t *d_dur, float *d_mu_y, float *d_logp, void *stream);

int ev_estimator_rows(ev_handle *h, const float *d_x, const float *d_mu, const int32_t *d_lengths, const float *d_spk,
                      const float *t , int B, int Tp, float *d_v, void *stream);
int ev_cfm_loss(ev_handle *h, const float *d_x1, const float *d_mu_y, const int32_t *d_ylen, const float *d_spk, const float *d_z,
                const float *t , int B, int Ty, float sigma_min, double *d_row_sums, float *d_v, void *stream);

int ev_load_resampler(ev_handle *h, const float *taps , int n_taps, int up, int down);
int ev_resample(ev_handle *h, const float *d_x , const int32_t *d_len , int B, int L_in,
                float *d_y , int L_out, void *stream);
int ev_mel_stats(ev_handle *h, const float *d_mel , const int32_t *d_len , int B, int C, int T,
                 double *d_row_sums , void *stream);

int ev_profile_enable(ev_handle *h, int on);
int ev_profile_read(ev_handle *h, double *conv_ms, double *conv_flops, int64_t *conv_launches, int reset);
int ev_profile_read_split(ev_handle *h, double *ms, double *flops, int64_t *launches);
int ev_set_arithmetic(ev_handle *h, int setting);
int ev_get_arithmetic(ev_handle *h);

int ev_dbg_last_cfg(ev_handle *h);

int ev_dbg_conv_bench(ev_handle *h, int Cin, int Cout, int K, int dil, int B, int T, int P, int iters, int dbg, int cfg, float *ms_out);

int ev_dbg_set_amax(ev_handle *h, int on);
int ev_dbg_set_attn_h16(ev_handle *h, int on);
int ev_dbg_set_chain(ev_handle *h, int on);

int ev_dbg_sk_stats(ev_handle *h, uint32_t *out3);
int64_t ev_dbg_sk_taken(ev_handle *h);

int ev_op_conv1d(ev_handle *h, const float *d_x , const float *w ,
                 const float *bias , int B, int Cin, int T, int Cout, int K, int dilation,
                 int transposed, int stride, int padding, float pre_lrelu_slope , float *d_y, void *stream);
int ev_op_groupnorm_mish(ev_handle *h, const float *d_x , const float *d_gamma, const float *d_beta,
                         const int32_t *d_lengths, int B, int C, int T, int groups, float *d_y, void *stream);
int ev_op_split_pieces(ev_handle *h, const float *d_x, int n, float *d_pieces, void *stream);
int ev_op_layernorm(ev_handle *h, const float *d_x , const float *d_gamma, const float *d_beta, int rows,
                    int C, float *d_y, void *stream);
int ev_op_ln_mlp(ev_handle *h, const float *d_x, const float *d_ln_g, const float *d_ln_b, const float *w1, const float *b1,
                 const float *d_alpha_exp, const float *d_beta_inv, const float *w2, const float *b2, const float *d_rowmask,
                 int rows, int M1, int mode, float *d_y, void *stream);
int ev_op_attention(ev_handle *h, const float *d_qkv , const int32_t *d_lengths, int B, int T,
                    int heads, float *d_out , void *stream);

int ev_op_attn_out(ev_handle *h, const float *d_qkv, const int32_t *d_lengths, int B, int T, const float *w_out, const float *b_out,
                   float *d_hid, void *stream);

#ifdef __cplusplus
}
#endif
#endif
```

Before: 4791 audio_s/s.

## Fold resnet GroupNorm+Mish into the fused LayerNorm+QKV kernel via per-slab stats

```diff
diff --git a/emojivoice_amd/_lib.py b/emojivoice_amd/_lib.py
--- a/emojivoice_amd/_lib.py
+++ b/emojivoice_amd/_lib.py
@@ -22,6 +22,7 @@
     "ev_maximum_path", "ev_log_prior", "ev_mas_align",
     "ev_estimator_rows", "ev_cfm_loss",
     "ev_load_resampler", "ev_resample", "ev_mel_stats",
+    "ev_dbg_gn_fused",
 ]
 
 
@@ -144,6 +145,7 @@
     lib.ev_dbg_set_attn_h16.argtypes = [vp, i32]
     lib.ev_dbg_set_chain.argtypes = [vp, i32]
     lib.ev_dbg_sk_taken.argtypes = [vp]
+    lib.ev_dbg_gn_fused.argtypes = [vp, C.POINTER(C.c_uint32)]
     lib.ev_dbg_sk_taken.restype = C.c_int64
     lib.ev_op_conv1d.argtypes = [vp, vp, vp, vp, i32, i32, i32, i32, i32, i32, i32, i32, i32, f32, vp, vp]
     lib.ev_op_groupnorm_mish.argtypes = [vp, vp, vp, vp, vp, i32, i32, i32, i32, vp, vp]
@@ -412,6 +414,11 @@
     def sk_taken(self) -> int:
         return int(self.lib.ev_dbg_sk_taken(self.h))
 
+    def gn_fused(self):
+        out = (C.c_uint32 * 2)()
+        self._check(self.lib.ev_dbg_gn_fused(self.h, out), "ev_dbg_gn_fused")
+        return tuple(int(v) for v in out)
+
     def sk_stats(self):
         out = (C.c_uint32 * 3)()
         self._check(self.lib.ev_dbg_sk_stats(self.h, out), "ev_dbg_sk_stats")
diff --git a/emojivoice_amd/csrc/ev_engine.hip b/emojivoice_amd/csrc/ev_engine.hip
--- a/emojivoice_amd/csrc/ev_engine.hip
+++ b/emojivoice_amd/csrc/ev_engine.hip
@@ -53,6 +53,7 @@
     float pro_slope = -1.f;
     int dbg = 0; int force_cfg = -1; int stagger = -1; unsigned long long* stamps = nullptr;
     float* gn_part = nullptr;
+    float* gn_slots = nullptr;
     int isplit_log2 = 31, isstride = 0;
     unsigned* ymax = nullptr; int ymax_mul = 1; const unsigned* rmax = nullptr; const unsigned* yold = nullptr; const unsigned* xmax = nullptr; int xmax_n = 0;
     int osplit_log2 = 31, osstride = 0;
@@ -164,6 +165,10 @@
     bool small_sk = true;
     bool sk32_lean = true;
     bool gn_stats = true;
+    bool gn_fuse = true;
+    bool bal_small = false;
+    bool gn_slots_ready = false;
+    uint32_t gn_fused[2] = {0, 0};
     bool qkv_h16 = true;
     bool attn_sk = true;
     int attn_tpw = 2;
@@ -580,8 +585,9 @@
 template <int PIPE, int BM, int BN, int WM, int WN>
 int launch_bal(ev_handle* h, ConvParams p, const LaunchOpts& lo, int wpc) {
     static_assert((size_t)BM * BN <= EV_SK_PART_FLOATS, "hand-off slot");
-    const int G = wpc * h->ncu;
-    if (sk_setup(h, p.sk, (long)p.mtiles * p.ntiles * (p.Kpad / (PIPE == PIPE_FP32 ? EV_BK : EVX_KC)), G, PIPE == PIPE_H16)) return 1;
+    const long U = (long)p.mtiles * p.ntiles * (p.Kpad / (PIPE == PIPE_FP32 ? EV_BK : EVX_KC));
+    const int G = (int)std::min<long>((long)wpc * h->ncu, U);
+    if (sk_setup(h, p.sk, U, G, PIPE == PIPE_H16)) return 1;
     const size_t rsb = PIPE == PIPE_FP32 ? 36 * sizeof(float) : PIPE == PIPE_BF16 ? EVX_RSB : EVH_RSB;
     const size_t xs = (size_t)(BN + ((lo.halo + 7) & ~7)) * rsb;
     constexpr size_t es = (size_t)4 * 32 * (BM / WM + 4) * sizeof(float);
@@ -601,7 +607,7 @@
 }
 inline bool split_bal_ok(const ev_handle* h, const ConvLayer& L, const ConvParams& p, long nwg, int wpc) {
     return h->sk_balance && h->ncu > 0 && split_ok(L, p) && p.act != ACT_SNAKE && !p.dbg && !p.stamps && !p.gn_part &&
-           nwg * 2 >= h->ncu && wpc * h->ncu <= EV_SK_MAXWG && (long)nwg * (p.Kpad / EVX_KC) >= (long)wpc * h->ncu;
+           wpc * h->ncu <= EV_SK_MAXWG && (h->bal_small || (nwg * 2 >= h->ncu && (long)nwg * (p.Kpad / EVX_KC) >= (long)wpc * h->ncu));
 }
 inline bool bal_ok(const ev_handle* h, const ConvLayer& L, const ConvParams& p, long nwg, int wpc) {
     if (L.sparse_taps) return false;
@@ -663,7 +669,8 @@
     }
     {
         const int split_terms = h->split_terms;
-        const bool fp32_tile = cfg == CFG_128x128 || cfg == CFG_64x128 || cfg == CFG_64x192 || cfg == CFG_64x64;
+        const bool fp32_tile = cfg == CFG_128x128 || cfg == CFG_64x128 || cfg == CFG_64x192 || cfg == CFG_64x64 ||
+                               (h->bal_small && (cfg == CFG_64x64_PF || cfg == CFG_SK64 || cfg == CFG_SK32));
         const long nwg128 = tiles(CFG_128x128);
         if (split_terms > 0 && fp32_tile && split_ok(L, p) && L.Cout % 128 == 0 && (!L.sparse_taps || (L.tile128_exact && L.kstack_mt == 0)) && nwg128 >= 2L * 2 * h->ncu && h->ncu > 0)
             cfg = split_terms == 3 ? CFG_SPLIT3 : split_terms == 9 ? CFG_SPLIT9 : split_terms == 16 ? CFG_H16 : CFG_SPLIT;
@@ -674,11 +681,13 @@
     return cfg;
 }
 
+inline int gn_slots_len(const Geom& g) { return g.S / 32 + 2; }
+inline size_t gn_slots_floats(const Geom& g) { return (size_t)(g.nrows / g.S) * gn_slots_len(g) * 8 * 4; }
 constexpr int EV_GN_MAXTILES = 256;
 int launch_conv(ev_handle* h, const ConvLayer& L, const float* X, int ldx, float* Y, int ldy, const Geom& g, const Epi& e) {
     ConvParams p;
     memset(&p, 0, sizeof p);
-    h->gn_stats_tiles = 0;
+    h->gn_stats_tiles = 0; h->gn_slots_ready = false;
     if (L.halo_lo + L.halo_hi > EV_HALO) return fail(h, "launch_conv: conv halo %d exceeds EV_HALO", L.halo_lo + L.halo_hi);
     p.X = X; p.ldx = ldx; p.Cin = L.Cin; p.isplit_log2 = e.isplit_log2; p.isstride = e.isstride;
     p.W = L.W; p.Wx = L.Wx; p.Wh = L.Wh; p.Wq = L.Wq; p.wh_scale = L.wh_scale; p.Mpad = L.Mpad; p.Kpad = L.Kpad; p.bias = L.bias;
@@ -741,7 +750,13 @@
         else launch_split<64, 128, 2, 2, 6>(p, h->stream, lo);
         break;
     case CFG_SPLIT_BAL:
-        if (fp16) { if (launch_bal<PIPE_H16, 128, 128, 2, 2>(h, p, lo, 2)) return 1; cfg = CFG_H16_BAL; }
+        if (fp16) {
+            if (e.gn_slots && h->gn_fuse && !lean_acc(p) && g.S >= 32 && L.Cout >= 256 && p.osplit_log2 >= 31) {
+                p.gn_slots = e.gn_slots; p.gn_nslab = gn_slots_len(g); h->gn_slots_ready = true;
+            }
+            if (launch_bal<PIPE_H16, 128, 128, 2, 2>(h, p, lo, 2)) return 1;
+            cfg = CFG_H16_BAL;
+        }
         else if (launch_bal<PIPE_BF16, 128, 128, 2, 2>(h, p, lo, 2)) return 1;
         break;
     case CFG_SPLIT: launch_split<128, 128, 2, 2, 6>(p, h->stream, lo); break;
@@ -945,9 +960,14 @@
     return 0;
 }
 
+inline bool qkv_h16_ok(const ev_handle* h, const ConvLayer& L1, const Geom& g) {
+    return h->split_terms == 16 && h->qkv_h16 && L1.Wh && L1.Mpad == 384 && h->ncu > 0 && ((g.nrows + 63) / 64 >= h->ncu || h->bal_small);
+}
+struct GnFuse { const float* slots; int nslab; const float* A; const float* R; int ldr; const float* gamma; const float* beta; const float* rowmask; float* H; };
+
 int launch_mlp(ev_handle* h, int mode, const float* X, const float* ln_g, const float* ln_b, const ConvLayer& L1, const ConvLayer* L2,
                const float* alpha, const float* binv, const float* R, const float* rowmask, float* Y, int ldy, const Geom& g,
-               const float* qkv_scale = nullptr, int* qkv_packed = nullptr) {
+               const float* qkv_scale = nullptr, int* qkv_packed = nullptr, const GnFuse* gn = nullptr) {
     if (qkv_packed) *qkv_packed = 0;
     MlpParams mp;
     memset(&mp, 0, sizeof mp);
@@ -993,8 +1013,14 @@
     }
     {
         const int nt64 = (g.nrows + 63) / 64;
-        if (mode == 1 && h->split_terms == 16 && h->qkv_h16 && L1.Wh && L1.Mpad == 384 && !R && !rowmask && h->ncu > 0 && nt64 >= h->ncu) {
+        if (mode == 1 && qkv_h16_ok(h, L1, g) && !R && !rowmask) {
             mp.W1h = L1.Wh; mp.w1_scale = L1.wh_scale; mp.ntiles = nt64;
+            if (gn) {
+                if (g.S < 32 || over_4gib(g, gn->ldr)) return fail(h, "launch_mlp: the folded GroupNorm needs utterances of at least 32 rows");
+                mp.X = gn->A; mp.gn_slots = gn->slots; mp.gn_nslab = gn->nslab; mp.gn_gamma = gn->gamma; mp.gn_beta = gn->beta; mp.gn_eps = 1e-5f;
+                mp.gn_R = gn->R; mp.gn_ldr = gn->ldr; mp.gn_rowmask = gn->rowmask; mp.gn_H = gn->H;
+                ++h->gn_fused[1];
+            }
             if (qkv_scale && qkv_packed && qkv_scale[0] > 0.f && qkv_scale[1] > 0.f && qkv_scale[2] > 0.f) {
                 mp.qkv_pack = 1; *qkv_packed = 1;
                 for (int i = 0; i < 3; ++i) mp.qkv_scale[i] = qkv_scale[i];
@@ -1007,6 +1033,7 @@
             return h->prof ? prof_end(h, {3, 256, Lout.Cout, 1, g.nrows, 122, 1, flops, true}) : 0;
         }
     }
+    if (gn) return fail(h, "launch_mlp: only ln_qkv_h16_kernel applies a deferred GroupNorm, and this launch does not take it");
     const int ntiles = (g.nrows + 31) / 32;
     size_t smem = (size_t)(32 * 260 + 4 * 32 * 36 + 4) * sizeof(float);
     int grid = ntiles;
@@ -1137,6 +1164,7 @@
     float *A1, *B1, *R1, *H1, *LN1, *QKV1, *ATT1, *FF1, *CAT0, *D1, *D2, *M1, *UU;
     float *tv, *temb_in, *temb_a, *temb_b, *tproj;
     float *LOSSP; int32_t* elen;
+    float *GNS;
     float *GNP;
     float *ATTP;
     float *C1RMS;
@@ -1160,6 +1188,7 @@
     e.C1RMS = b.take(n0 * 512); e.AR0 = b.take(n0 * 512); e.AR1 = b.take(n1 * 512);
     e.ATTP = b.take(std::min<size_t>(n0, EV_ATTN_MAXROWS) * EV_ATTN_MAXPARTS * (128 + 4));
     e.GNP = b.take((size_t)EV_GN_MAXTILES * 8 * 4);
+    e.GNS = b.take(std::max(gn_slots_floats(e.g0), gn_slots_floats(e.g1)));
     e.tv = b.take(ns); e.temb_in = b.take(ns * in_ch); e.temb_a = b.take(ns * 1024); e.temb_b = b.take(ns * 1024); e.tproj = b.take(ns * 1536);
     e.LOSSP = b.take((size_t)B * (Tp / 32 + 1) * 4); e.elen = (int32_t*)b.take(B);
 }
@@ -1280,35 +1309,51 @@
     return 0;
 }
 
-struct LevelBufs { float *A, *Bf, *R, *H, *LN, *QKV, *ATT, *FF; const float* rm; Geom g; float* AR; float* ATTP; float* GNP; };
+struct LevelBufs { float *A, *Bf, *R, *H, *LN, *QKV, *ATT, *FF; const float* rm; Geom g; float* AR; float* ATTP; float* GNP; float* GNS; };
 inline int g_rows32(const Geom& g) { return (g.nrows + 31) / 32; }
 
-int run_resnet(ev_handle* h, const ResnetW& w, const float* X, int ldx, const LevelBufs& L, const float* temb, int tstride) {
+int resnet_tail(ev_handle* h, const ResnetW& w, const LevelBufs& L, bool defer, bool* deferred) {
+    *deferred = defer && h->gn_slots_ready;
+    if (*deferred) return 0;
+    return launch_gn(h, L.A, 256, L.H, 256, w.g2, w.b2, L.rm, nullptr, L.AR + 256, 512, L.g, 256, 2, L.GNP);
+}
+
+int run_resnet(ev_handle* h, const ResnetW& w, const float* X, int ldx, const LevelBufs& L, const float* temb, int tstride, bool defer, bool* deferred) {
     Epi e; e.gn_part = L.GNP;
     if (launch_conv(h, w.c1r, X, ldx, L.AR, 512, L.g, e)) return 1;
     if (launch_gn(h, L.AR, 512, L.Bf, 256, w.g1, w.b1, L.rm, temb, nullptr, 0, L.g, 256, 1, L.GNP, tstride)) return 1;
+    if (defer) e.gn_slots = L.GNS;
     if (launch_conv(h, w.c2, L.Bf, 256, L.A, 256, L.g, e)) return 1;
-    return launch_gn(h, L.A, 256, L.H, 256, w.g2, w.b2, L.rm, nullptr, L.AR + 256, 512, L.g, 256, 2, L.GNP);
-}
-
-int run_resnet0(ev_handle* h, const EstimatorW& W, const float* X, int ldx, const LevelBufs& L, const float* temb, int tstride, const float* C1RMS) {
+    return resnet_tail(h, w, L, defer, deferred);
+}
+
+int run_resnet0(ev_handle* h, const EstimatorW& W, const float* X, int ldx, const LevelBufs& L, const float* temb, int tstride, const float* C1RMS,
+                bool defer, bool* deferred) {
     const ResnetW& w = W.rn[0];
     Epi e;
     { Epi e1; e1.R = C1RMS; e1.ldr = 512; if (launch_conv(h, W.rn0_c1r_x, X, ldx, L.AR, 512, L.g, e1)) return 1; }
     if (launch_gn(h, L.AR, 512, L.Bf, 256, w.g1, w.b1, L.rm, temb, nullptr, 0, L.g, 256, 1, nullptr, tstride)) return 1;
     e.gn_part = L.GNP;
+    if (defer) e.gn_slots = L.GNS;
     if (launch_conv(h, w.c2, L.Bf, 256, L.A, 256, L.g, e)) return 1;
-    return launch_gn(h, L.A, 256, L.H, 256, w.g2, w.b2, L.rm, nullptr, L.AR + 256, 512, L.g, 256, 2, L.GNP);
-}
-
-int run_transformer(ev_handle* h, const TransW& w, const LevelBufs& L, float* Z, int ldz, int heads) {
+    return resnet_tail(h, w, L, defer, deferred);
+}
+
+inline bool transformer_fuses(const ev_handle* h, const LevelBufs& L) { return h->fuse_mlp && g_rows32(L.g) >= h->fuse_mlp_min_tiles; }
+inline bool gn_defer_ok(const ev_handle* h, const TransW& w, const LevelBufs& L) {
+    return h->gn_fuse && transformer_fuses(h, L) && qkv_h16_ok(h, w.qkv, L.g) && L.g.S >= 32;
+}
+
+int run_transformer(ev_handle* h, const TransW& w, const LevelBufs& L, float* Z, int ldz, int heads, const ResnetW* gn = nullptr) {
     Epi e;
-    const bool fuse = h->fuse_mlp && g_rows32(L.g) >= h->fuse_mlp_min_tiles;
+    const bool fuse = transformer_fuses(h, L);
+    if (gn && !fuse) return fail(h, "run_transformer: a deferred GroupNorm needs the fused LayerNorm + QKV launch");
     const bool aok = attn_out_ok(h, w.out, L.g, heads);
     int packed = 0;
     if (fuse) {
+        GnFuse gf{L.GNS, gn_slots_len(L.g), L.A, L.AR + 256, 512, gn ? gn->g2 : nullptr, gn ? gn->b2 : nullptr, L.rm, L.H};
         if (launch_mlp(h, 1, L.H, w.ln1g, w.ln1b, w.qkv, nullptr, nullptr, nullptr, nullptr, nullptr, L.QKV, 384, L.g,
-                       (aok && h->attn_h16 && w.out.Wh) ? w.qkv_scale : nullptr, &packed)) return 1;
+                       (aok && h->attn_h16 && w.out.Wh) ? w.qkv_scale : nullptr, &packed, gn ? &gf : nullptr)) return 1;
     } else {
         if (launch_ln(h, L.H, 256, L.LN, 256, w.ln1g, w.ln1b, L.g)) return 1;
         if (launch_conv(h, w.qkv, L.LN, 256, L.QKV, 384, L.g, e)) return 1;
@@ -1331,30 +1376,31 @@
 int run_estimator(ev_handle* h, EstBufs& b, int step, float dt, bool euler, const float* tproj = nullptr, int tstride = 0) {
     const EstimatorW& w = h->est;
     const int heads = h->dims.heads;
-    LevelBufs L0{b.A0, b.B0, b.R0, b.H0, b.LN0, b.QKV0, b.ATT0, b.FF0, b.rm0, b.g0, b.AR0, b.ATTP, b.GNP};
-    LevelBufs L1{b.A1, b.B1, b.R1, b.H1, b.LN1, b.QKV1, b.ATT1, b.FF1, b.rm1, b.g1, b.AR1, b.ATTP, b.GNP};
+    LevelBufs L0{b.A0, b.B0, b.R0, b.H0, b.LN0, b.QKV0, b.ATT0, b.FF0, b.rm0, b.g0, b.AR0, b.ATTP, b.GNP, b.GNS};
+    LevelBufs L1{b.A1, b.B1, b.R1, b.H1, b.LN1, b.QKV1, b.ATT1, b.FF1, b.rm1, b.g1, b.AR1, b.ATTP, b.GNP, b.GNS};
     const float* tp = (tproj ? tproj : b.tproj) + (size_t)step * 1536;
-    if (run_resnet0(h, w, b.X0, w.in_ch, L0, tp + 0 * 256, tstride, b.C1RMS)) return 1;
-    if (run_transformer(h, w.tr[0], L0, b.CAT1 + 256, 512, heads)) return 1;
+    bool gd = false;
+    if (run_resnet0(h, w, b.X0, w.in_ch, L0, tp + 0 * 256, tstride, b.C1RMS, gn_defer_ok(h, w.tr[0], L0), &gd)) return 1;
+    if (run_transformer(h, w.tr[0], L0, b.CAT1 + 256, 512, heads, gd ? &w.rn[0] : nullptr)) return 1;
     {
         Epi e; e.isplit_log2 = 8; e.isstride = 512; e.mask1 = 1; e.rowmask = b.rm1;
         if (launch_conv(h, w.down0, b.CAT1 + 256, 1024, b.D1, 256, b.g1, e)) return 1;
     }
-    if (run_resnet(h, w.rn[1], b.D1, 256, L1, tp + 1 * 256, tstride)) return 1;
-    if (run_transformer(h, w.tr[1], L1, b.CAT0 + 256, 512, heads)) return 1;
+    if (run_resnet(h, w.rn[1], b.D1, 256, L1, tp + 1 * 256, tstride, gn_defer_ok(h, w.tr[1], L1), &gd)) return 1;
+    if (run_transformer(h, w.tr[1], L1, b.CAT0 + 256, 512, heads, gd ? &w.rn[1] : nullptr)) return 1;
     { Epi e; e.mask1 = 1; e.rowmask = b.rm1; if (launch_conv(h, w.down1, b.CAT0 + 256, 512, b.D2, 256, b.g1, e)) return 1; }
-    if (run_resnet(h, w.rn[2], b.D2, 256, L1, tp + 2 * 256, tstride)) return 1;
-    if (run_transformer(h, w.tr[2], L1, b.M1, 256, heads)) return 1;
-    if (run_resnet(h, w.rn[3], b.M1, 256, L1, tp + 3 * 256, tstride)) return 1;
-    if (run_transformer(h, w.tr[3], L1, b.CAT0, 512, heads)) return 1;
-    if (run_resnet(h, w.rn[4], b.CAT0, 512, L1, tp + 4 * 256, tstride)) return 1;
-    if (run_transformer(h, w.tr[4], L1, b.UU, 256, heads)) return 1;
+    if (run_resnet(h, w.rn[2], b.D2, 256, L1, tp + 2 * 256, tstride, gn_defer_ok(h, w.tr[2], L1), &gd)) return 1;
+    if (run_transformer(h, w.tr[2], L1, b.M1, 256, heads, gd ? &w.rn[2] : nullptr)) return 1;
+    if (run_resnet(h, w.rn[3], b.M1, 256, L1, tp + 3 * 256, tstride, gn_defer_ok(h, w.tr[3], L1), &gd)) return 1;
+    if (run_transformer(h, w.tr[3], L1, b.CAT0, 512, heads, gd ? &w.rn[3] : nullptr)) return 1;
+    if (run_resnet(h, w.rn[4], b.CAT0, 512, L1, tp + 4 * 256, tstride, gn_defer_ok(h, w.tr[4], L1), &gd)) return 1;
+    if (run_transformer(h, w.tr[4], L1, b.UU, 256, heads, gd ? &w.rn[4] : nullptr)) return 1;
     {
         Epi e; e.osplit_log2 = 8; e.osstride = 512; e.mask1 = 1; e.rowmask = b.rm0; e.mmul = 2;
         if (launch_conv(h, w.up0, b.UU, 256, b.CAT1, 1024, b.g1, e)) return 1;
     }
-    if (run_resnet(h, w.rn[5], b.CAT1, 512, L0, tp + 5 * 256, tstride)) return 1;
-    if (run_transformer(h, w.tr[5], L0, b.U1, 256, heads)) return 1;
+    if (run_resnet(h, w.rn[5], b.CAT1, 512, L0, tp + 5 * 256, tstride, gn_defer_ok(h, w.tr[5], L0), &gd)) return 1;
+    if (run_transformer(h, w.tr[5], L0, b.U1, 256, heads, gd ? &w.rn[5] : nullptr)) return 1;
     { Epi e; e.mask1 = 1; e.rowmask = b.rm0; if (launch_conv(h, w.up1, b.U1, 256, b.F0, 256, b.g0, e)) return 1; }
     { Epi e; if (launch_conv(h, w.fin_conv, b.F0, 256, b.A0, 256, b.g0, e)) return 1; }
     if (launch_gn(h, b.A0, 256, b.G0, 256, w.fin_g, w.fin_b, b.rm0, nullptr, nullptr, 0, b.g0, 256, 0)) return 1;
@@ -1726,6 +1772,8 @@
     if (getenv("EV_NO_SK32_LEAN")) h->sk32_lean = false;
     if (getenv("EV_NO_GN_STATS")) h->gn_stats = false;
     if (getenv("EV_NO_QKV_H16")) h->qkv_h16 = false;
+    if (getenv("EV_NO_GN_FUSE")) h->gn_fuse = false;
+    if (getenv("EV_BAL_SMALL")) h->bal_small = true;
     if (getenv("EV_NO_ATTN_SK")) h->attn_sk = false;
     { const char* fp = getenv("EV_ATTN_TPW"); if (fp) h->attn_tpw = std::max(1, atoi(fp)); }
     if (getenv("EV_FULL_REZERO")) h->full_rezero = true;
@@ -2285,6 +2333,12 @@
     HIPCHK(h, hipSetDevice(h->device));
     HIPCHK(h, hipDeviceSynchronize());
     HIPCHK(h, hipMemcpy(out3, h->sk_ctrl, 3 * sizeof(uint32_t), hipMemcpyDeviceToHost));
+    return 0;
+}
+
+int ev_dbg_gn_fused(ev_handle* h, uint32_t* out2) {
+    if (!h || !out2) return 1;
+    out2[0] = h->gn_fused[0]; out2[1] = h->gn_fused[1];
     return 0;
 }
 
diff --git a/emojivoice_amd/csrc/ev_kernels.h b/emojivoice_amd/csrc/ev_kernels.h
--- a/emojivoice_amd/csrc/ev_kernels.h
+++ b/emojivoice_amd/csrc/ev_kernels.h
@@ -54,6 +54,7 @@
     float* Y2; int ldy2;
     int ktaps_n, plane_bytes, koff0, kdoff;
     float* gn_part;
+    float* gn_slots; int gn_nslab;
     int kstack_mt, kstack_tap;
     int sk_kb;
     unsigned* ymax; int ymax_mul;
@@ -253,7 +254,8 @@
     return fmaf(fmaf(-3.f, q, x), 0.333333343267440796f, q);
 }
 struct EvNoHook { __device__ __forceinline__ void operator()() const {} };
-template <int TM, int TN, int MODE, class Hook, class PutSlab>
+__device__ __forceinline__ float wave_sum(float v);
+template <int TM, int TN, int MODE, bool GN, class Hook, class PutSlab>
 __device__ __forceinline__ void conv_epilogue_lean_impl(const ConvParams& p, PutSlab put_slab, float* Es, int mw0, int nw0, int lane,
                                                         int win_lo, int win_hi, Hook after_issue) {
     constexpr int EC = TM * 32, ELD = EC + 4, C4 = EC / 4, RPP = 64 / C4, NP = 32 / RPP;
@@ -330,14 +332,53 @@
                 }
             }
             if (ok) ev_bstore4(rY, yoff, v);
+            if constexpr (GN) {
+                if (p.gn_slots) *(f32x4*)(Es + rl * ELD + ec) = v;
+            }
             if (j + 1 < TN) issue_one(q);
             t += RPP; t -= (t >= lim) ? p.S : 0; t -= (t >= lim) ? p.S : 0;
             yoff += ystep;
         }
+        if constexpr (GN) {
+            const int ns = nw0 + j * 32;
+            if (p.gn_slots && ns < p.nrows) {
+                const int b0 = ns / p.S, rem = ns - b0 * p.S;
+                const int sl = lane & 31, sh = lane >> 5;
+                const int nh = (rem + 31 >= p.S) ? 2 : 1;
+                const __amdgpu_buffer_rsrc_t rG = ev_rsrc(p.gn_slots);
+                for (int hh = 0; hh < nh; ++hh) {
+                    const int b = b0 + hh;
+                    if (b * p.S >= p.nrows) break;
+                    const int tt = rem + sl - hh * p.S - p.P;
+                    const bool in = tt >= 0 && tt < p.T && ns + sl < p.nrows;
+                    const float cnt = (float)(__popcll(__ballot(in)) * 16);
+                    const int slab = (ns >> 5) - ((b * p.S) >> 5);
+#pragma unroll
+                    for (int i = 0; i < TM; ++i) {
+                        const int grp = (mw0 >> 5) + i;
+                        if (grp >= 8) continue;
+                        const float* src = Es + sl * ELD + i * 32 + sh * 16;
+                        const f32x4 w0 = *(const f32x4*)(src), w1 = *(const f32x4*)(src + 4), w2 = *(const f32x4*)(src + 8), w3 = *(const f32x4*)(src + 12);
+                        float s1 = ((w0[0] + w0[1]) + (w0[2] + w0[3])) + ((w1[0] + w1[1]) + (w1[2] + w1[3]));
+                        s1 += ((w2[0] + w2[1]) + (w2[2] + w2[3])) + ((w3[0] + w3[1]) + (w3[2] + w3[3]));
+                        const float mean = cnt > 0.f ? wave_sum(in ? s1 : 0.f) / cnt : 0.f;
+                        float s2 = 0.f;
+#pragma unroll
+                        for (int e = 0; e < 4; ++e) {
+                            const float d0 = w0[e] - mean, d1 = w1[e] - mean, d2 = w2[e] - mean, d3 = w3[e] - mean;
+                            s2 += (d0 * d0 + d1 * d1) + (d2 * d2 + d3 * d3);
+                        }
+                        s2 = wave_sum(in ? s2 : 0.f);
+                        const f32x4 o = {cnt, mean, s2, 0.f};
+                        if (lane == 0) ev_bstore4(rG, (unsigned)((b * p.gn_nslab + slab) * 8 + grp) * 16u, o);
+                    }
+                }
+            }
+        }
         asm volatile("s_waitcnt lgkmcnt(0)" ::: "memory");
     }
 }
-template <int TM, int TN, int MODE = 1, class Hook = EvNoHook>
+template <int TM, int TN, int MODE = 1, class Hook = EvNoHook, bool GN = false>
 __device__ __forceinline__ void conv_epilogue_lean(const ConvParams& p, f32x16 (&acc)[TM][TN], float* Es, int mw0, int nw0, int lane,
                                                    int win_lo = -0x7fffffff, int win_hi = 0x7fffffff, Hook after_issue = Hook()) {
     auto put = [&](int j) {
@@ -351,7 +392,7 @@
                 *(f32x4*)(Es + li * ELD + i * 32 + 8 * g + 4 * lh) = q4;
             }
     };
-    conv_epilogue_lean_impl<TM, TN, MODE>(p, put, Es, mw0, nw0, lane, win_lo, win_hi, after_issue);
+    conv_epilogue_lean_impl<TM, TN, MODE, GN>(p, put, Es, mw0, nw0, lane, win_lo, win_hi, after_issue);
 }
 template <int TM, int TN, int MODE = 1>
 __device__ __forceinline__ void conv_epilogue_lean_q(const ConvParams& p, f32x4 (&acc)[2 * TM][2 * TN], float* Es, int mw0, int nw0, int lane,
@@ -364,7 +405,7 @@
 #pragma unroll
             for (int a = 0; a < 2 * TM; ++a) *(f32x4*)(Es + (b2 * 16 + f) * ELD + a * 16 + 4 * kg) = acc[a][2 * j + b2];
     };
-    conv_epilogue_lean_impl<TM, TN, MODE>(p, put, Es, mw0, nw0, lane, win_lo, win_hi, EvNoHook());
+    conv_epilogue_lean_impl<TM, TN, MODE, false>(p, put, Es, mw0, nw0, lane, win_lo, win_hi, EvNoHook());
 }
 
 typedef __attribute__((address_space(1))) unsigned ev_gu32;
@@ -2005,7 +2046,7 @@
             }
             if (again) continue;
             __builtin_amdgcn_s_setprio(3);
-            conv_epilogue_lean<TM, TN, LEAN>(p, acc, smem + wave * (32 * (TM * 32 + 4)), m0 + wm * (TM * 32), n0 + wn * (TN * 32), lane);
+            conv_epilogue_lean<TM, TN, LEAN, EvNoHook, LEAN == 1>(p, acc, smem + wave * (32 * (TM * 32 + 4)), m0 + wm * (TM * 32), n0 + wn * (TN * 32), lane);
             __builtin_amdgcn_s_setprio(0);
             break;
         }
@@ -3517,6 +3558,8 @@
     int ntiles;
     SkCtl sk;
     int qkv_pack; float qkv_scale[3];
+    const float* gn_slots; int gn_nslab; const float* gn_gamma; const float* gn_beta; float gn_eps;
+    const float* gn_R; int gn_ldr; const float* gn_rowmask; float* gn_H;
 };
 
 template <int MODE, int WPC>
@@ -4483,6 +4526,32 @@
     sk_arrive(mp.sk, tag, tid);
 }
 
+__device__ __forceinline__ void ev_gn_merge(const float* slots, int nslab, int b, int g, int S, int P, int T, int nrows, int lane, float eps,
+                                            float& mean_out, float& rstd_out) {
+    const int s0 = (b * S) >> 5;
+    const int vlo = b * S + P, vhi = (vlo + T < nrows) ? vlo + T : nrows;
+    float na = 0.f, mean = 0.f, m2 = 0.f;
+    for (int j0 = 0; j0 < nslab; j0 += 8) {
+        const int j = j0 + (lane >> 3);
+        const int r0 = (s0 + j) * 32;
+        const int lo = r0 > vlo ? r0 : vlo, hi = r0 + 32 < vhi ? r0 + 32 : vhi;
+        f32x4 sv = {0.f, 0.f, 0.f, 0.f};
+        if (j < nslab && lo < hi) sv = *(const f32x4*)(slots + ((size_t)(b * nslab + j) * 8 + (lane & 7)) * 4);
+        const int nj = nslab - j0 < 8 ? nslab - j0 : 8;
+        for (int k = 0; k < nj; ++k) {
+            const float nb = __shfl(sv[0], k * 8 + g, 64), mb = __shfl(sv[1], k * 8 + g, 64), qb = __shfl(sv[2], k * 8 + g, 64);
+            if (nb > 0.f) {
+                const float nn = na + nb, d = mb - mean, w = nb / nn;
+                mean += d * w;
+                m2 += qb + d * d * na * w;
+                na = nn;
+            }
+        }
+    }
+    mean_out = mean;
+    rstd_out = 1.0f / sqrtf(m2 / na + eps);
+}
+
 template <int UNUSED = 0>
 __global__ __launch_bounds__(256, 2) void ln_qkv_h16_kernel(const MlpParams mp) {
     constexpr int NT = 64, C = 256, TM = 3;
@@ -4513,12 +4582,6 @@
             for (int pc = 0; pc < 2; ++pc) dst[i][pc] = ev_bload4(rW1, wlane, (unsigned)((((wave * TM + i) * (C / 16) + sl) * 2 + pc) * 1024));
     };
     ldA(A[0], 0); ldA(A[1], 1); ldA(A[2], 2);
-    f32x4 bq[TM][4];
-    const unsigned coff = (unsigned)(4 * lh) * 4u;
-#pragma unroll
-    for (int i = 0; i < TM; ++i)
-#pragma unroll
-        for (int q = 0; q < 4; ++q) bq[i][q] = ev_bload4(rB1, coff + (unsigned)((wave * TM + i) * 32 + 8 * q) * 4u, 0);
     float sx;
     {
         const f32x4 gm = *(const f32x4*)(mp.ln_g + lane * 4), be = *(const f32x4*)(mp.ln_b + lane * 4);
@@ -4527,6 +4590,46 @@
         for (int r = 0; r < 16; ++r) {
             const int gr = n0 + wave * 16 + r;
             xv[r] = ev_bload4(rX, ((unsigned)(gr < p.nrows ? gr : 0) * mp.ldx + lane * 4) * 4u, 0);
+        }
+        if (mp.gn_slots) {
+            const int gr0 = n0 + wave * 16;
+            const int b0 = gr0 / p.S, rem = gr0 - b0 * p.S;
+            const int g = lane >> 3;
+            float mean0, rstd0, mean1 = 0.f, rstd1 = 0.f;
+            ev_gn_merge(mp.gn_slots, mp.gn_nslab, b0, g, p.S, p.P, p.T, p.nrows, lane, mp.gn_eps, mean0, rstd0);
+            if (rem + 15 >= p.S && (b0 + 1) * p.S < p.nrows)
+                ev_gn_merge(mp.gn_slots, mp.gn_nslab, b0 + 1, g, p.S, p.P, p.T, p.nrows, lane, mp.gn_eps, mean1, rstd1);
+            const f32x4 ga = *(const f32x4*)(mp.gn_gamma + lane * 4), gb = *(const f32x4*)(mp.gn_beta + lane * 4);
+            const __amdgpu_buffer_rsrc_t rR = ev_rsrc(mp.gn_R), rH = ev_rsrc(mp.gn_H);
+#pragma unroll
+            for (int r8 = 0; r8 < 16; r8 += 8) {
+                f32x4 rv[8];
+                float mk[8];
+#pragma unroll
+                for (int r = 0; r < 8; ++r) {
+                    const int gr = gr0 + r8 + r;
+                    const int gs = gr < p.nrows ? gr : 0;
+                    rv[r] = ev_bload4(rR, ((unsigned)gs * mp.gn_ldr + lane * 4) * 4u, 0);
+                    mk[r] = mp.gn_rowmask[gs];
+                }
+#pragma unroll
+                for (int r = 0; r < 8; ++r) {
+                    const int gr = gr0 + r8 + r;
+                    const bool nxt = rem + r8 + r >= p.S;
+                    const int t = rem + r8 + r - (nxt ? p.S : 0) - p.P;
+                    const bool live = t >= 0 && t < p.T && gr < p.nrows;
+                    const float mean = nxt ? mean1 : mean0, rstd = nxt ? rstd1 : rstd0;
+                    f32x4 o;
+#pragma unroll
+                    for (int e = 0; e < 4; ++e) {
+                        const float y = (xv[r8 + r][e] - mean) * rstd * ga[e] + gb[e];
+                        o[e] = ev_mish(y) * mk[r] + rv[r][e];
+                    }
+                    const f32x4 z = {0.f, 0.f, 0.f, 0.f};
+                    xv[r8 + r] = live ? o : z;
+                    if (live) ev_bstore4(rH, ((unsigned)gr * 256u + lane * 4) * 4u, o);
+                }
+            }
         }
         float mx = 0.f;
 #pragma unroll
@@ -4558,6 +4661,12 @@
             *(uint2*)(dst) = q0v; *(uint2*)(dst + 2 * C) = q1v;
         }
     }
+    f32x4 bq[TM][4];
+    const unsigned coff = (unsigned)(4 * lh) * 4u;
+#pragma unroll
+    for (int i = 0; i < TM; ++i)
+#pragma unroll
+        for (int q = 0; q < 4; ++q) bq[i][q] = ev_bload4(rB1, coff + (unsigned)((wave * TM + i) * 32 + 8 * q) * 4u, 0);
     ev_lds_barrier();
     const float u1 = mp.w1_scale * sx, inv1 = 1.0f / u1;
     f32x16 acc[TM][2];
diff --git a/include/emojivoice.h b/include/emojivoice.h
--- a/include/emojivoice.h
+++ b/include/emojivoice.h
@@ -111,6 +111,7 @@
 
 int ev_dbg_sk_stats(ev_handle *h, uint32_t *out3);
 int64_t ev_dbg_sk_taken(ev_handle *h);
+int ev_dbg_gn_fused(ev_handle *h, uint32_t *out2);
 
 int ev_op_conv1d(ev_handle *h, const float *d_x , const float *w ,
                  const float *bias , int B, int Cin, int T, int Cout, int K, int dilation,
```

Result: no change. 4782 audio_s/s (-0.2%).
